# DecodeGenetics/Ratatosk

Hardware: AMD Instinct MI355X
Metric: corrected long-read bases/sec (higher is better)
Workload: dtype u64

## Files before the change

### include/ratatosk_hip.h

```cpp
#ifndef RATATOSK_HIP_H
#define RATATOSK_HIP_H

#include <stdint.h>

#ifdef __cplusplus
extern "C" {
#endif

#define RTK_OK 0
#define RTK_ERR_IO (-1)
#define RTK_ERR_FORMAT (-2)
#define RTK_ERR_ARG (-3)
#define RTK_ERR_NO_DEVICE (-4)
#define RTK_ERR_DEVICE (-5)
#define RTK_ERR_UNSUPPORTED (-6)

typedef struct rtk_graph rtk_graph;
typedef struct rtk_batch rtk_batch;

typedef struct rtk_opts {
    uint64_t insert_sz;
    uint64_t min_cov_vertices;
    uint64_t max_len_weak_region1;
    uint64_t max_km_cov;
    double weak_region_len_factor;
    double large_k_factor;
    double min_score;
    int32_t max_qual;
    int32_t out_qual;
    double min_confidence_snp_corr;
    int32_t long_read_correct;
    int32_t force_unres_snp_corr;
    uint64_t max_len_weak_region2;
    int32_t a2_exclusive;
    int32_t a3_strand_order;
    int32_t d1_desc;
    uint32_t struct_size;
} rtk_opts;

typedef struct rtk_graph_info {
    uint64_t n_unitigs, n_kmers, n_bases, n_colour_ids, n_global_sets;
    uint64_t table_slots, hbm_bytes;
    uint64_t max_km_cov_top;
    int32_t k, device;
} rtk_graph_info;

typedef struct rtk_stats {
    double ms_total, ms_lookup_exact, ms_mask, ms_lookup_inexact, ms_seeds, ms_regions, ms_correct, ms_stitch;
    uint64_t n_windows, n_probes_exact, n_probes_inexact, n_hits_inexact, n_regions, n_region_items, n_arena_overflow;
    uint64_t n_expand, n_colour_elem, n_path_base, n_align, n_align_cells;
    uint64_t in_bases, out_bases;
    uint64_t cyc_colour, cyc_paths, cyc_consensus, cyc_total, cyc_myers, cyc_sets , cyc_tostring, cyc_pathqual;
    uint64_t n_slots_exact, n_slots_inexact;
    uint64_t cyc_walk, n_moves;
    double ms_lanes;
    uint64_t n_lane_regions, n_lane_handed;
    double ms_phase;
    uint64_t n_phase_skipped;
    uint64_t n_trim_stored, n_trim_column, n_trim_fallback, n_consensus_resumed, n_consensus_swept;
    uint64_t n_fa_linked_run, n_fa_linked_skipped, n_fa_linked_entries;
    uint64_t n_strand2_run, n_strand2_skipped, n_strand2_audit_mismatch;
    uint64_t n_park_walked, n_park_deferred;
    uint64_t n_colours_small, n_colours_wide, n_colours_bits, n_colours_general, n_colours_audit_mismatch;
    uint64_t n_colours_declined_fit;
    uint64_t n_park_resweeps;
} rtk_stats;

int rtk_graph_load(const char* unitig_fasta_gz, const char* rtsk, int k, int n_threads, rtk_graph** out);
#define RTK_LOAD_DEVICE_TABLES 1u
int rtk_graph_load2(const char* unitig_fasta_gz, const char* rtsk, int k, int n_threads, uint32_t flags, rtk_graph** out);

int rtk_graph_upload(rtk_graph* g, int device);

int rtk_graph_shell(int k, rtk_graph** out);
int rtk_graph_n_buffers(const rtk_graph* g);
int rtk_graph_buffer(rtk_graph* g, int idx, void** dev_ptr, uint64_t* bytes);
int rtk_graph_alloc_buffers(rtk_graph* g, int device, const uint64_t* bytes, int n, const rtk_graph_info* info);
int rtk_graph_adopt_device(rtk_graph* g);
int rtk_graph_attach_buffers(rtk_graph* g, int device, void* const* dev_ptrs, const uint64_t* bytes, int n, const rtk_graph_info* info);
int rtk_graph_buffer_bytes(const rtk_graph* g, uint64_t* bytes, int n);
int rtk_graph_move_buffer(rtk_graph* g, int idx, void* dev_ptr, uint64_t bytes);
int rtk_graph_host_buffer(const rtk_graph* g, int idx, const void** p, uint64_t* bytes);
int rtk_graph_download_buffer(const rtk_graph* g, int idx, void* host_dst, uint64_t bytes);

int rtk_n_devices(void);
int rtk_device_memory(int device, uint64_t* free_bytes, uint64_t* total_bytes);
int rtk_graph_clone_to_device(const rtk_graph* src, int device, rtk_graph** out);

int rtk_graph_get_info(const rtk_graph* g, rtk_graph_info* info);
void rtk_graph_free(rtk_graph* g);
long long rtk_graph_strip_annotations(rtk_graph* g);

int rtk_reserve_scratch(int device, uint32_t max_read_len);
int rtk_reserve_second_pass(int device, uint32_t n_tickets, uint64_t phase_bytes, uint64_t region_bytes);
int rtk_graph_reserve_batches(rtk_graph* g, uint32_t n_batches, uint64_t bases_per_batch, uint32_t reads_per_batch, int with_qualities, uint64_t raw_bases_per_batch);

int rtk_opts_default(const rtk_graph* g, rtk_opts* opts);

int rtk_correct_batch(rtk_graph* g, const rtk_opts* opts, uint32_t n, const char* const* seq, const char* const* qual,
                      const uint32_t* len, char** out_seq, char** out_qual, uint32_t* out_len);
int rtk_coalesce_stats(rtk_graph* g, uint64_t* n_groups, uint64_t* n_tickets);

int rtk_batch_create(rtk_graph* g, uint32_t n, const char* const* seq, const char* const* qual, const uint32_t* len, rtk_batch** out);
int rtk_batch_create2(rtk_graph* g, uint32_t n, const char* const* seq, const char* const* qual, const uint32_t* len,
                      const char* const* raw, const uint32_t* raw_len, rtk_batch** out);
int rtk_batch_run(rtk_batch* b, const rtk_opts* opts);
int rtk_batch_run_seeds(rtk_batch* b, const rtk_opts* opts);
int rtk_batch_run_regions(rtk_batch* b, const rtk_opts* opts);
int rtk_batch_fetch(rtk_batch* b, char** out_seq, char** out_qual, uint32_t* out_len);
int rtk_batch_fetch_view(rtk_batch* b, const char** pool, const uint64_t** off, const uint32_t** len);
int rtk_batch_get_stats(const rtk_batch* b, rtk_stats* stats);
void rtk_batch_free(rtk_batch* b);


int rtk_lookup_exact(rtk_graph* g, const char* seq, uint32_t len, int64_t* hits);

int rtk_fix_snps(rtk_graph* g, const char* seq, uint32_t len, char* out);

int rtk_seeds(rtk_graph* g, const rtk_opts* opts, const char* seq, uint32_t len,
              uint64_t* n_solid, int64_t* solid, uint64_t* n_weak, int64_t* weak, uint64_t cap);

int rtk_batch_fetch_seeds(rtk_batch* b, uint32_t read, uint64_t* n_solid, int64_t* solid, uint64_t* n_weak, int64_t* weak, uint64_t cap);

int rtk_myers_batch(uint32_t n, const char* const* query, const uint32_t* qlen, const char* const* target, const uint32_t* tlen,
                    const int32_t* k, const int32_t* mode, int want_path, int use_iupac,
                    int32_t* dist, int32_t* n_loc, int32_t* end_locs, uint32_t cap_locs, char* cigar, uint32_t cap_cigar);

int rtk_myers_batch_waves(uint32_t n, const char* const* query, const uint32_t* qlen, const char* const* target, const uint32_t* tlen,
                          const int32_t* k, const int32_t* mode, int want_path, int use_iupac,
                          int32_t* dist, int32_t* n_loc, int32_t* end_locs, uint32_t cap_locs, char* cigar, uint32_t cap_cigar, int waves);

#define RTK_MYERS_MODE_SHW_BY_COLUMN 3
#define RTK_MYERS_MODE_NW_PREFIX 4
#define RTK_MYERS_MODE_NW_PREFIX_LAST 5
#define RTK_MYERS_MODE_NW_PREFIX_LAST_COLUMN 6
void rtk_myers_column_last_routes(uint64_t* column_route, uint64_t* fallback);

int rtk_myers_batch_lanes(uint32_t n, const char* const* query, const uint32_t* qlen, const char* const* target, const uint32_t* tlen,
                          const int32_t* k, const int32_t* mode, int want_path, int use_iupac,
                          int32_t* dist, int32_t* n_loc, int32_t* end_locs, uint32_t cap_locs, char* cigar, uint32_t cap_cigar);
void rtk_myers_lanes_last_routes(uint64_t* lane_route, uint64_t* wave_route);

int rtk_index_count_kmers(int device, int k, const char* const* files, int n_files, uint32_t min_count, int n_threads, uint64_t** solid, uint64_t* n_solid);
int rtk_index_unitigs(int device, int k, const uint64_t* solid, uint64_t n_solid, char** seq_pool, uint64_t** seq_off, uint64_t** seeds, uint64_t* n_unitigs,
                      uint64_t** left, uint64_t* n_left);

int rtk_index_colour_begin(int device, int k, const char* seq_pool, const uint64_t* seq_off, uint64_t n_unitigs, void** job);
int rtk_index_colour_chunk(void* job, const char* chars, uint64_t n_chars, const uint64_t* starts, const uint32_t* ids, uint32_t n_reads);
int rtk_index_colour_end(void* job, uint64_t** events, uint64_t* n_events, uint64_t** cov);
int rtk_index_colour_chunk_q(void* job, const char* chars, const unsigned char* quals, unsigned char q_min, uint64_t n_chars, const uint64_t* starts, const uint32_t* ids,
                             uint32_t n_reads);
int rtk_index_colour_cov(void* job, uint64_t** cov);
int rtk_index_colour_end_subsampled(void* job, const uint8_t* bin_of_unitig, const uint8_t* forced_candidate, const uint8_t* bin_is_sampled, uint32_t n_bins, uint32_t mcv,
                                    double rate, uint64_t seed, uint64_t** events, uint64_t* n_events, uint64_t* n_events_before, uint64_t* n_ids_before, uint64_t* n_ids_after);
int rtk_index_subsample_events(int device, const uint64_t* events, uint64_t n_events, uint32_t n_unitigs, const uint8_t* bin_of_unitig, const uint8_t* forced_candidate,
                               const uint8_t* bin_is_sampled, uint32_t n_bins, uint32_t mcv, double rate, uint64_t seed, uint64_t* events_out, uint64_t* n_out,
                               uint64_t* n_ids_before, uint64_t* n_ids_after);
int rtk_index_colour_merge(void* job, uint64_t* n_events_before, uint64_t* n_events_after, uint64_t* n_ids_before, uint64_t* n_ids_after);
int rtk_index_colour_merge_classes(void* job, uint64_t* classes_above_one, uint64_t* largest);
int rtk_index_merge_events(int device, const uint64_t* events, uint64_t n_events, uint32_t n_unitigs, uint64_t* events_out, uint64_t* n_out, uint64_t* n_ids_before,
                           uint64_t* n_ids_after);

#define RTK_SNP_FIRST_PER_SITE 1u
int rtk_index_snp_candidates(int device, int k, const char* seq_pool, const uint64_t* seq_off, uint64_t n_unitigs, const uint8_t* searched, uint32_t flags,
                             uint64_t** cand, uint64_t* n_cand);
int rtk_index_snp_plan(int device, int k, const uint64_t* seq_off, uint64_t n_unitigs, const uint8_t* searched, uint64_t room, uint32_t* passes,
                       uint64_t* need_one_pass, uint64_t* need_min);

int rtk_index_cover_begin(int device, int k, const char* seq_pool, const uint64_t* seq_off, uint64_t n_unitigs, const uint8_t* low_bits, void** job);
int rtk_index_cover_chunk(void* job, const char* chars, uint64_t n_chars, const uint64_t* starts, const uint32_t* seq_numbers, const uint64_t* first_positions, uint32_t n_seqs);
int rtk_index_cover_end(void* job, uint64_t** crossings, uint64_t* n);

int rtk_rescue_begin(int device, int k, const uint64_t* lr, uint64_t n_lr, const uint64_t* sr, uint64_t n_sr, uint32_t min_positions, void** job);
int rtk_rescue_chunk(void* job, const char* chars, uint64_t n_chars, const uint64_t* starts, uint32_t n_reads, unsigned char* keep);
int rtk_rescue_end(void* job, uint64_t* n_positions_probed, uint64_t* n_hits);

int rtk_qv_begin(int device, int k, const uint64_t* solid, uint64_t n_solid, void** job);
int rtk_qv_chunk(void* job, const char* chars, uint64_t n_chars, const uint64_t* starts, uint32_t n_pieces, uint32_t* windows, uint32_t* found);
int rtk_qv_end(void* job, uint64_t* n_windows, uint64_t* n_found);
uint32_t rtk_qv_span(void);

#define RTK_SETS_UNION 0
#define RTK_SETS_INTER 1
#define RTK_SETS_DIFF 2
#define RTK_SETS_INTER_COUNT 3
#define RTK_SETS_SORT_PAIRS 4
#define RTK_SETS_RADIX_U32 5
#define RTK_SETS_RADIX_PAIRS_U32 6
#define RTK_SETS_BM_LOWEST 7
#define RTK_SETS_BM8_LOWEST 8
#define RTK_SETS_RADIX_TAGGED 9
#define RTK_SETS_COLOUR_UNIVERSE 10
#define RTK_SETS_OK 0
#define RTK_SETS_NOT_IN_BUILD 1
#define RTK_SETS_DECLINED 2
int rtk_sets_batch(uint32_t n, const uint32_t* op, const uint32_t* const* a, const uint32_t* na, const uint32_t* const* b, const uint32_t* nb, const uint32_t* scalar,
                   uint32_t* out_pool, const uint64_t* out_off, uint32_t* out_n, uint32_t* result, uint32_t* status);

void rtk_free(void* p);
void rtk_free_many(void** p, uint32_t n);
const char* rtk_last_error(void);
const char* rtk_version(void);
#define RTK_API_REVISION 10
int rtk_api_revision(void);

#ifdef __cplusplus
}
#endif

#endif
```

### ratatosk_amd/api.py

```python
import ctypes as C
import os

_HERE = os.path.dirname(os.path.abspath(__file__))
LIB_PATH = os.environ.get("RTK_LIB_OVERRIDE") or os.path.join(_HERE, "libratatosk_hip.so")


class RtkError(RuntimeError):
    pass


class RtkOpts(C.Structure):
    _fields_ = [("insert_sz", C.c_uint64), ("min_cov_vertices", C.c_uint64), ("max_len_weak_region1", C.c_uint64),
                ("max_km_cov", C.c_uint64), ("weak_region_len_factor", C.c_double), ("large_k_factor", C.c_double),
                ("min_score", C.c_double), ("max_qual", C.c_int32), ("out_qual", C.c_int32), ("min_confidence_snp_corr", C.c_double),
                ("long_read_correct", C.c_int32), ("force_unres_snp_corr", C.c_int32), ("max_len_weak_region2", C.c_uint64),
                ("a2_exclusive", C.c_int32), ("a3_strand_order", C.c_int32), ("d1_desc", C.c_int32), ("struct_size", C.c_uint32)]


class RtkGraphInfo(C.Structure):
    _fields_ = [("n_unitigs", C.c_uint64), ("n_kmers", C.c_uint64), ("n_bases", C.c_uint64), ("n_colour_ids", C.c_uint64),
                ("n_global_sets", C.c_uint64), ("table_slots", C.c_uint64), ("hbm_bytes", C.c_uint64), ("max_km_cov_top", C.c_uint64),
                ("k", C.c_int32), ("device", C.c_int32)]


class RtkStats(C.Structure):
    _fields_ = [(n, C.c_double) for n in ("ms_total", "ms_lookup_exact", "ms_mask", "ms_lookup_inexact", "ms_seeds", "ms_regions", "ms_correct", "ms_stitch")] + \
               [(n, C.c_uint64) for n in ("n_windows", "n_probes_exact", "n_probes_inexact", "n_hits_inexact", "n_regions", "n_region_items", "n_arena_overflow",
                                         "n_expand", "n_colour_elem", "n_path_base", "n_align", "n_align_cells", "in_bases", "out_bases",
                                         "cyc_colour", "cyc_paths", "cyc_consensus", "cyc_total", "cyc_myers", "cyc_sets", "cyc_tostring", "cyc_pathqual", "n_slots_exact", "n_slots_inexact", "cyc_walk", "n_moves")] + \
               [("ms_lanes", C.c_double), ("n_lane_regions", C.c_uint64), ("n_lane_handed", C.c_uint64), ("ms_phase", C.c_double), ("n_phase_skipped", C.c_uint64)] + \
               [(n, C.c_uint64) for n in ("n_trim_stored", "n_trim_column", "n_trim_fallback", "n_consensus_resumed", "n_consensus_swept",
                                         "n_fa_linked_run", "n_fa_linked_skipped", "n_fa_linked_entries",
                                         "n_strand2_run", "n_strand2_skipped", "n_strand2_audit_mismatch",
                                         "n_park_walked", "n_park_deferred",
                                         "n_colours_small", "n_colours_wide", "n_colours_bits", "n_colours_general", "n_colours_audit_mismatch", "n_colours_declined_fit",
                                         "n_park_resweeps")]

    def as_dict(self):
        return {n: getattr(self, n) for n, _ in self._fields_}


_libs = {}


os.environ.setdefault("GPU_MAX_HW_QUEUES", "16")


def load_library(path=None):
    path = path or LIB_PATH
    if path in _libs:
        return _libs[path]
    if not os.path.exists(path):
        raise RtkError("%s is missing: build it with `python -c 'import __graft_entry__ as g; g.build()'` (make -C ratatosk_amd/csrc)" % path)
    L = C.CDLL(path)
    L.rtk_last_error.restype = C.c_char_p
    L.rtk_version.restype = C.c_char_p
    L.rtk_graph_load.argtypes = [C.c_char_p, C.c_char_p, C.c_int, C.c_int, C.POINTER(C.c_void_p)]
    L.rtk_graph_load2.argtypes = [C.c_char_p, C.c_char_p, C.c_int, C.c_int, C.c_uint32, C.POINTER(C.c_void_p)]
    L.rtk_graph_move_buffer.argtypes = [C.c_void_p, C.c_int, C.c_void_p, C.c_uint64]
    L.rtk_graph_host_buffer.argtypes = [C.c_void_p, C.c_int, C.POINTER(C.c_void_p), C.POINTER(C.c_uint64)]
    L.rtk_graph_download_buffer.argtypes = [C.c_void_p, C.c_int, C.c_void_p, C.c_uint64]
    L.rtk_graph_upload.argtypes = [C.c_void_p, C.c_int]
    L.rtk_graph_shell.argtypes = [C.c_int, C.POINTER(C.c_void_p)]
    L.rtk_graph_n_buffers.argtypes = [C.c_void_p]
    L.rtk_graph_buffer.argtypes = [C.c_void_p, C.c_int, C.POINTER(C.c_void_p), C.POINTER(C.c_uint64)]
    L.rtk_graph_alloc_buffers.argtypes = [C.c_void_p, C.c_int, C.POINTER(C.c_uint64), C.c_int, C.POINTER(RtkGraphInfo)]
    L.rtk_graph_adopt_device.argtypes = [C.c_void_p]
    L.rtk_graph_buffer_bytes.argtypes = [C.c_void_p, C.POINTER(C.c_uint64), C.c_int]
    L.rtk_graph_get_info.argtypes = [C.c_void_p, C.POINTER(RtkGraphInfo)]
    L.rtk_graph_free.argtypes = [C.c_void_p]
    L.rtk_opts_default.argtypes = [C.c_void_p, C.POINTER(RtkOpts)]
    L.rtk_correct_batch.argtypes = [C.c_void_p, C.POINTER(RtkOpts), C.c_uint32, C.POINTER(C.c_char_p), C.POINTER(C.c_char_p), C.POINTER(C.c_uint32),
                                    C.POINTER(C.c_void_p), C.POINTER(C.c_void_p), C.POINTER(C.c_uint32)]
    L.rtk_batch_create.argtypes = [C.c_void_p, C.c_uint32, C.POINTER(C.c_char_p), C.POINTER(C.c_char_p), C.POINTER(C.c_uint32), C.POINTER(C.c_void_p)]
    L.rtk_batch_create2.argtypes = [C.c_void_p, C.c_uint32, C.POINTER(C.c_char_p), C.POINTER(C.c_char_p), C.POINTER(C.c_uint32),
                                    C.POINTER(C.c_char_p), C.POINTER(C.c_uint32), C.POINTER(C.c_void_p)]
    L.rtk_batch_run.argtypes = [C.c_void_p, C.POINTER(RtkOpts)]
    L.rtk_graph_strip_annotations.restype = C.c_longlong
    L.rtk_graph_strip_annotations.argtypes = [C.c_void_p]
    L.rtk_batch_run_seeds.argtypes = [C.c_void_p, C.POINTER(RtkOpts)]
    L.rtk_batch_run_regions.argtypes = [C.c_void_p, C.POINTER(RtkOpts)]
    L.rtk_batch_fetch.argtypes = [C.c_void_p, C.POINTER(C.c_void_p), C.POINTER(C.c_void_p), C.POINTER(C.c_uint32)]
    L.rtk_batch_fetch_view.argtypes = [C.c_void_p, C.POINTER(C.c_char_p), C.POINTER(C.POINTER(C.c_uint64)), C.POINTER(C.POINTER(C.c_uint32))]
    L.rtk_n_devices.restype = C.c_int
    L.rtk_device_memory.argtypes = [C.c_int, C.POINTER(C.c_uint64), C.POINTER(C.c_uint64)]
    L.rtk_graph_clone_to_device.argtypes = [C.c_void_p, C.c_int, C.POINTER(C.c_void_p)]
    L.rtk_batch_get_stats.argtypes = [C.c_void_p, C.POINTER(RtkStats)]
    L.rtk_batch_free.argtypes = [C.c_void_p]
    L.rtk_lookup_exact.argtypes = [C.c_void_p, C.c_char_p, C.c_uint32, C.POINTER(C.c_int64)]
    L.rtk_fix_snps.argtypes = [C.c_void_p, C.c_char_p, C.c_uint32, C.c_char_p]
    L.rtk_seeds.argtypes = [C.c_void_p, C.POINTER(RtkOpts), C.c_char_p, C.c_uint32, C.POINTER(C.c_uint64), C.POINTER(C.c_int64),
                            C.POINTER(C.c_uint64), C.POINTER(C.c_int64), C.c_uint64]
    L.rtk_myers_batch.argtypes = [C.c_uint32, C.POINTER(C.c_char_p), C.POINTER(C.c_uint32), C.POINTER(C.c_char_p), C.POINTER(C.c_uint32),
                                  C.POINTER(C.c_int32), C.POINTER(C.c_int32), C.c_int, C.c_int,
                                  C.POINTER(C.c_int32), C.POINTER(C.c_int32), C.POINTER(C.c_int32), C.c_uint32, C.c_char_p, C.c_uint32]
    L.rtk_myers_batch_waves.argtypes = L.rtk_myers_batch.argtypes + [C.c_int]
    L.rtk_myers_batch_lanes.argtypes = L.rtk_myers_batch.argtypes
    L.rtk_myers_batch_lanes.restype = C.c_int
    L.rtk_coalesce_stats.argtypes = [C.c_void_p, C.POINTER(C.c_uint64), C.POINTER(C.c_uint64)]
    L.rtk_graph_reserve_batches.argtypes = [C.c_void_p, C.c_uint32, C.c_uint64, C.c_uint32, C.c_int, C.c_uint64]
    L.rtk_free_many.argtypes = [C.POINTER(C.c_void_p), C.c_uint32]; L.rtk_free_many.restype = None
    if L.rtk_api_revision() >= 9:
        L.rtk_rescue_begin.argtypes = [C.c_int, C.c_int, C.POINTER(C.c_uint64), C.c_uint64, C.POINTER(C.c_uint64), C.c_uint64, C.c_uint32, C.POINTER(C.c_void_p)]
        L.rtk_rescue_chunk.argtypes = [C.c_void_p, C.c_char_p, C.c_uint64, C.POINTER(C.c_uint64), C.c_uint32, C.POINTER(C.c_ubyte)]
        L.rtk_rescue_end.argtypes = [C.c_void_p, C.POINTER(C.c_uint64), C.POINTER(C.c_uint64)]
    if L.rtk_api_revision() >= 10:
        L.rtk_sets_batch.argtypes = [C.c_uint32, C.POINTER(C.c_uint32), C.POINTER(C.POINTER(C.c_uint32)), C.POINTER(C.c_uint32), C.POINTER(C.POINTER(C.c_uint32)), C.POINTER(C.c_uint32),
                                     C.POINTER(C.c_uint32), C.POINTER(C.c_uint32), C.POINTER(C.c_uint64), C.POINTER(C.c_uint32), C.POINTER(C.c_uint32), C.POINTER(C.c_uint32)]
    if hasattr(L, "rtk_index_subsample_events"):
        L.rtk_index_colour_cov.argtypes = [C.c_void_p, C.POINTER(C.POINTER(C.c_uint64))]
        L.rtk_index_colour_end_subsampled.argtypes = [C.c_void_p, C.POINTER(C.c_ubyte), C.POINTER(C.c_ubyte), C.POINTER(C.c_ubyte), C.c_uint32, C.c_uint32, C.c_double, C.c_uint64,
                                                      C.POINTER(C.POINTER(C.c_uint64)), C.POINTER(C.c_uint64), C.POINTER(C.c_uint64), C.POINTER(C.c_uint64), C.POINTER(C.c_uint64)]
        L.rtk_index_subsample_events.argtypes = [C.c_int, C.POINTER(C.c_uint64), C.c_uint64, C.c_uint32, C.POINTER(C.c_ubyte), C.POINTER(C.c_ubyte), C.POINTER(C.c_ubyte), C.c_uint32, C.c_uint32,
                                                 C.c_double, C.c_uint64, C.POINTER(C.c_uint64), C.POINTER(C.c_uint64), C.POINTER(C.c_uint64), C.POINTER(C.c_uint64)]
    if hasattr(L, "rtk_index_merge_events"):
        L.rtk_index_colour_merge.argtypes = [C.c_void_p, C.POINTER(C.c_uint64), C.POINTER(C.c_uint64), C.POINTER(C.c_uint64), C.POINTER(C.c_uint64)]
        L.rtk_index_colour_merge_classes.argtypes = [C.c_void_p, C.POINTER(C.c_uint64), C.POINTER(C.c_uint64)]
        L.rtk_index_merge_events.argtypes = [C.c_int, C.POINTER(C.c_uint64), C.c_uint64, C.c_uint32, C.POINTER(C.c_uint64), C.POINTER(C.c_uint64), C.POINTER(C.c_uint64), C.POINTER(C.c_uint64)]
    if hasattr(L, "rtk_index_colour_chunk_q"):
        L.rtk_index_colour_chunk_q.argtypes = [C.c_void_p, C.c_char_p, C.c_char_p, C.c_ubyte, C.c_uint64, C.POINTER(C.c_uint64), C.POINTER(C.c_uint32), C.c_uint32]
    if hasattr(L, "rtk_batch_fetch_seeds"):
        L.rtk_batch_fetch_seeds.argtypes = [C.c_void_p, C.c_uint32, C.POINTER(C.c_uint64), C.POINTER(C.c_int64), C.POINTER(C.c_uint64), C.POINTER(C.c_int64), C.c_uint64]
    if hasattr(L, "rtk_index_snp_candidates"):
        L.rtk_index_snp_candidates.argtypes = [C.c_int, C.c_int, C.c_char_p, C.POINTER(C.c_uint64), C.c_uint64, C.POINTER(C.c_ubyte), C.c_uint32,
                                               C.POINTER(C.POINTER(C.c_uint64)), C.POINTER(C.c_uint64)]
    if hasattr(L, "rtk_index_snp_plan"):
        L.rtk_index_snp_plan.argtypes = [C.c_int, C.c_int, C.POINTER(C.c_uint64), C.c_uint64, C.POINTER(C.c_ubyte), C.c_uint64, C.POINTER(C.c_uint32), C.POINTER(C.c_uint64),
                                         C.POINTER(C.c_uint64)]
    if hasattr(L, "rtk_index_cover_begin"):
        L.rtk_index_cover_begin.argtypes = [C.c_int, C.c_int, C.c_char_p, C.POINTER(C.c_uint64), C.c_uint64, C.POINTER(C.c_ubyte), C.POINTER(C.c_void_p)]
        L.rtk_index_cover_chunk.argtypes = [C.c_void_p, C.c_char_p, C.c_uint64, C.POINTER(C.c_uint64), C.POINTER(C.c_uint32), C.POINTER(C.c_uint64), C.c_uint32]
        L.rtk_index_cover_end.argtypes = [C.c_void_p, C.POINTER(C.POINTER(C.c_uint64)), C.POINTER(C.c_uint64)]
    if hasattr(L, "rtk_qv_begin"):
        L.rtk_qv_begin.argtypes = [C.c_int, C.c_int, C.POINTER(C.c_uint64), C.c_uint64, C.POINTER(C.c_void_p)]
        L.rtk_qv_chunk.argtypes = [C.c_void_p, C.c_char_p, C.c_uint64, C.POINTER(C.c_uint64), C.c_uint32, C.POINTER(C.c_uint32), C.POINTER(C.c_uint32)]
        L.rtk_qv_end.argtypes = [C.c_void_p, C.POINTER(C.c_uint64), C.POINTER(C.c_uint64)]
        L.rtk_qv_span.argtypes = []; L.rtk_qv_span.restype = C.c_uint32
    L.rtk_free.argtypes = [C.c_void_p]
    _libs[path] = L
    return L


RTK_LOAD_DEVICE_TABLES = 1


def _b(s):
    return s.encode() if isinstance(s, str) else s


class Graph:

    def __init__(self, fasta_gz, rtsk, k=31, device=0, lib_path=None, upload=True, n_threads=None, host_tables=None):
        self.L = load_library(lib_path)
        self.h = C.c_void_p()
        if n_threads is None:
            n_threads = max(1, min(32, os.cpu_count() or 1))
        if host_tables is None:
            host_tables = not upload or os.environ.get("RTK_HOST_TABLES") == "1"
        self._check(self.L.rtk_graph_load2(_b(fasta_gz), _b(rtsk), k, n_threads, 0 if host_tables else RTK_LOAD_DEVICE_TABLES, C.byref(self.h)))
        self.k = k
        if upload:
            self._check(self.L.rtk_graph_upload(self.h, device))

    def _check(self, rc):
        if rc != 0:
            raise RtkError("rtk error %d: %s" % (rc, self.L.rtk_last_error().decode()))

    def close(self):
        if getattr(self, "h", None):
            self.L.rtk_graph_free(self.h)
            self.h = None

    def __del__(self):
        try:
            self.close()
        except Exception:
            pass

    def info(self):
        i = RtkGraphInfo()
        self._check(self.L.rtk_graph_get_info(self.h, C.byref(i)))
        return i

    def opts(self, **kw):
        o = RtkOpts()
        self._check(self.L.rtk_opts_default(self.h, C.byref(o)))
        for k_, v in kw.items():
            setattr(o, k_, v)
        return o

    def lookup_exact(self, seq):
        s = _b(seq)
        nw = max(0, len(s) - self.k + 1)
        out = (C.c_int64 * max(1, nw))()
        self._check(self.L.rtk_lookup_exact(self.h, s, len(s), out))
        return [out[i] for i in range(nw)]

    def fix_snps(self, seq):
        s = _b(seq)
        out = C.create_string_buffer(len(s) + 1)
        self._check(self.L.rtk_fix_snps(self.h, s, len(s), out))
        return out.raw[:len(s)]

    def seeds(self, seq, opts=None):
        s = _b(seq)
        o = opts or self.opts()
        cap = 64 * len(s) + 64
        ns, nw = C.c_uint64(), C.c_uint64()
        so, we = (C.c_int64 * (4 * cap))(), (C.c_int64 * (4 * cap))()
        self._check(self.L.rtk_seeds(self.h, C.byref(o), s, len(s), C.byref(ns), so, C.byref(nw), we, cap))
        f = lambda a, n: [(a[4 * i], a[4 * i + 1], a[4 * i + 2], a[4 * i + 3]) for i in range(n)]
        return f(so, ns.value), f(we, nw.value)

    def correct_batch(self, seqs, quals=None, opts=None, raw=None):
        b = Batch(self, seqs, quals, raw)
        try:
            b.run(opts)
            return b.fetch()
        finally:
            b.close()


class Batch:

    def __init__(self, graph, seqs, quals=None, raw=None):
        self.g = graph
        self.L = graph.L
        n = len(seqs)
        bs = [_b(s) for s in seqs]
        seq_arr = (C.c_char_p * n)(*bs)
        qual_arr = None
        if quals is not None:
            bq = [_b(q) for q in quals]
            qual_arr = (C.c_char_p * n)(*bq)
        lens = (C.c_uint32 * n)(*[len(b) for b in bs])
        self.n = n
        self.lens = [len(b) for b in bs]
        self.in_bases = sum(self.lens)
        self.h = C.c_void_p()
        if raw is not None:
            br = [_b(s) for s in raw]
            raw_arr = (C.c_char_p * n)(*br)
            raw_lens = (C.c_uint32 * n)(*[len(b) for b in br])
            graph._check(self.L.rtk_batch_create2(graph.h, n, seq_arr, qual_arr, lens, raw_arr, raw_lens, C.byref(self.h)))
        else:
            graph._check(self.L.rtk_batch_create(graph.h, n, seq_arr, qual_arr, lens, C.byref(self.h)))

    def run(self, opts=None):
        o = opts or self.g.opts()
        self.g._check(self.L.rtk_batch_run(self.h, C.byref(o)))

    def run_seeds(self, opts=None):
        o = opts or self.g.opts()
        self.g._check(self.L.rtk_batch_run_seeds(self.h, C.byref(o)))

    def run_regions(self, opts=None):
        o = opts or self.g.opts()
        self.g._check(self.L.rtk_batch_run_regions(self.h, C.byref(o)))

    def seeds(self, i, cap=None):
        if not hasattr(self.L, "rtk_batch_fetch_seeds"):
            raise RtkError("%s lacks rtk_batch_fetch_seeds (anchors of one read of a batch: appended at interface revision 10)" % self.L._name)
        ns, nw = C.c_uint64(), C.c_uint64()
        if cap is None:
            one = (C.c_int64 * 4)()
            rc = self.L.rtk_batch_fetch_seeds(self.h, i, C.byref(ns), one, C.byref(nw), one, 0)
            if rc != 0 and b"capacity" not in self.L.rtk_last_error():
                self.g._check(rc)
            cap = max(ns.value, nw.value)
        so, we = (C.c_int64 * (4 * max(1, cap)))(), (C.c_int64 * (4 * max(1, cap)))()
        self.g._check(self.L.rtk_batch_fetch_seeds(self.h, i, C.byref(ns), so, C.byref(nw), we, cap))
        f = lambda a, n: [(a[4 * j], a[4 * j + 1], a[4 * j + 2], a[4 * j + 3]) for j in range(n)]
        return f(so, ns.value), f(we, nw.value)

    def fetch(self):
        n = self.n
        os_, oq = (C.c_void_p * n)(), (C.c_void_p * n)()
        ol = (C.c_uint32 * n)()
        self.g._check(self.L.rtk_batch_fetch(self.h, os_, oq, ol))
        out = []
        for i in range(n):
            out.append((C.string_at(os_[i], ol[i]).decode(), C.string_at(oq[i], ol[i]).decode()))
            self.L.rtk_free(os_[i]); self.L.rtk_free(oq[i])
        return out

    def stats(self):
        s = RtkStats()
        self.g._check(self.L.rtk_batch_get_stats(self.h, C.byref(s)))
        return s.as_dict()

    def close(self):
        if getattr(self, "h", None):
            self.L.rtk_batch_free(self.h)
            self.h = None

    def __del__(self):
        try:
            self.close()
        except Exception:
            pass


def myers_batch(queries, targets, ks=None, modes=None, want_path=False, use_iupac=True, lib_path=None, waves=0, lanes=False):
    L = load_library(lib_path)
    n = len(queries)
    bq = [_b(q) for q in queries]; bt = [_b(t) for t in targets]
    ks = ks if ks is not None else [-1] * n
    modes = modes if modes is not None else [0] * n
    qa = (C.c_char_p * n)(*bq); ta = (C.c_char_p * n)(*bt)
    ql = (C.c_uint32 * n)(*[len(x) for x in bq]); tl = (C.c_uint32 * n)(*[len(x) for x in bt])
    ka = (C.c_int32 * n)(*ks); ma = (C.c_int32 * n)(*modes)
    cap_locs = max(len(x) for x in bt) + 2 if n else 2
    cap_cig = 4 * (max((len(x) for x in bq), default=0) + max((len(x) for x in bt), default=0)) + 16
    dist = (C.c_int32 * n)(); nloc = (C.c_int32 * n)(); locs = (C.c_int32 * (n * cap_locs))()
    cig = C.create_string_buffer(n * cap_cig) if want_path else None
    if lanes:
        rc = L.rtk_myers_batch_lanes(n, qa, ql, ta, tl, ka, ma, 1 if want_path else 0, 1 if use_iupac else 0, dist, nloc, locs, cap_locs, cig, cap_cig)
    elif waves > 1:
        rc = L.rtk_myers_batch_waves(n, qa, ql, ta, tl, ka, ma, 1 if want_path else 0, 1 if use_iupac else 0, dist, nloc, locs, cap_locs, cig, cap_cig, waves)
    else:
        rc = L.rtk_myers_batch(n, qa, ql, ta, tl, ka, ma, 1 if want_path else 0, 1 if use_iupac else 0, dist, nloc, locs, cap_locs, cig, cap_cig)
    if rc != 0:
        raise RtkError("rtk error %d: %s" % (rc, L.rtk_last_error().decode()))
    out = []
    for i in range(n):
        el = [locs[i * cap_locs + j] for j in range(min(nloc[i], cap_locs))] if dist[i] >= 0 else []
        c = ""
        if want_path:
            c = cig.raw[i * cap_cig:(i + 1) * cap_cig].split(b"\0", 1)[0].decode()
        out.append((dist[i], el, c))
    return out


def _u64_array(a):
    if hasattr(a, "ctypes"):
        import numpy as np
        arr = np.ascontiguousarray(a, dtype=np.uint64)
        return arr, arr.ctypes.data_as(C.POINTER(C.c_uint64)), int(arr.size)
    arr = (C.c_uint64 * max(1, len(a)))(*[int(x) for x in a])
    return arr, arr, len(a)


def rescue_reads(lr_kmers, sr_kmers, seqs, k=31, min_positions=31, device=0, stats=None, lib_path=None):
    L = load_library(lib_path)
    if L.rtk_api_revision() < 9:
        raise RtkError("%s is of interface revision %d: the rescue entries came with revision 9" % (L._name, L.rtk_api_revision()))
    keep_lr, p_lr, n_lr = _u64_array(lr_kmers)
    keep_sr, p_sr, n_sr = _u64_array(sr_kmers)
    job = C.c_void_p()

    def check(rc):
        if rc != 0:
            raise RtkError("rtk error %d: %s" % (rc, L.rtk_last_error().decode()))

    check(L.rtk_rescue_begin(device, k, p_lr, n_lr, p_sr, n_sr, min_positions, C.byref(job)))
    out = []
    try:
        bs = [_b(s) for s in seqs]
        i = 0
        while i < len(bs):
            j, size = i, 0
            while j < len(bs) and (j == i or (size + len(bs[j]) + 1 <= (48 << 20) and j - i < (2 << 20))):
                size += len(bs[j]) + 1; j += 1
            starts, at = (C.c_uint64 * (j - i))(), 0
            for r in range(i, j):
                starts[r - i] = at; at += len(bs[r]) + 1
            chars = b"\n".join(bs[i:j]) + b"\n"
            keep = (C.c_ubyte * (j - i))()
            check(L.rtk_rescue_chunk(job, chars, len(chars), starts, j - i, keep))
            out.extend(bool(x) for x in keep)
            i = j
    except Exception:
        L.rtk_rescue_end(job, None, None)
        raise
    probed, hits = C.c_uint64(), C.c_uint64()
    check(L.rtk_rescue_end(job, C.byref(probed), C.byref(hits)))
    if stats is not None:
        stats["n_positions_probed"], stats["n_hits"] = probed.value, hits.value
    return out


QV_CHUNK_CHARS = 48 << 20


def qv_span(lib_path=None):
    L = load_library(lib_path)
    if not hasattr(L, "rtk_qv_begin"):
        raise RtkError("%s has no rtk_qv entries" % L._name)
    return int(L.rtk_qv_span())


def qv_reads(solid_kmers, seqs, k=31, device=0, max_piece=None, lib_path=None, threads=1, stats=None):
    L = load_library(lib_path)
    if not hasattr(L, "rtk_qv_begin"):
        raise RtkError("%s has no rtk_qv entries" % L._name)
    if max_piece is None:
        max_piece = QV_CHUNK_CHARS - 1
    if max_piece < k or max_piece > QV_CHUNK_CHARS - 1:
        raise ValueError("max_piece must lie in k .. %d" % (QV_CHUNK_CHARS - 1))
    keep_solid, p_solid, n_solid = _u64_array(solid_kmers)
    bs = [_b(s) for s in seqs]
    pieces = []
    for r, s in enumerate(bs):
        a = 0
        while True:
            pieces.append((r, s[a:a + max_piece]))
            if a + max_piece >= len(s):
                break
            a += max_piece - (k - 1)
    chunks, i = [], 0
    while i < len(pieces):
        j, size = i, 0
        while j < len(pieces) and size + len(pieces[j][1]) + 1 <= max_piece + 1 and j - i < (2 << 20):
            size += len(pieces[j][1]) + 1; j += 1
        chunks.append((i, j)); i = j
    job = C.c_void_p()

    def check(rc):
        if rc != 0:
            raise RtkError("rtk error %d: %s" % (rc, L.rtk_last_error().decode()))

    check(L.rtk_qv_begin(device, k, p_solid, n_solid, C.byref(job)))
    windows, found = [0] * len(bs), [0] * len(bs)
    results = [None] * len(chunks)

    def run(c):
        i, j = chunks[c]
        starts, at = (C.c_uint64 * (j - i))(), 0
        for p in range(i, j):
            starts[p - i] = at; at += len(pieces[p][1]) + 1
        chars = b"\n".join(t for _, t in pieces[i:j]) + b"\n"
        w, f = (C.c_uint32 * (j - i))(), (C.c_uint32 * (j - i))()
        check(L.rtk_qv_chunk(job, chars, len(chars), starts, j - i, w, f))
        results[c] = (list(w), list(f))

    try:
        if threads <= 1:
            for c in range(len(chunks)):
                run(c)
        else:
            import threading
            errors = []

            def feed(t):
                try:
                    for c in range(t, len(chunks), threads):
                        run(c)
                except Exception as e:
                    errors.append(e)

            th = [threading.Thread(target=feed, args=(t,)) for t in range(threads)]
            for t in th:
                t.start()
            for t in th:
                t.join()
            if errors:
                raise errors[0]
    except Exception:
        L.rtk_qv_end(job, None, None)
        raise
    n_windows, n_found = C.c_uint64(), C.c_uint64()
    check(L.rtk_qv_end(job, C.byref(n_windows), C.byref(n_found)))
    for c, (i, j) in enumerate(chunks):
        w, f = results[c]
        for p in range(i, j):
            windows[pieces[p][0]] += w[p - i]; found[pieces[p][0]] += f[p - i]
    if (sum(windows), sum(found)) != (n_windows.value, n_found.value):
        raise RtkError("rtk_qv: the pieces add up to %d windows / %d found, the device counted %d / %d" % (sum(windows), sum(found), n_windows.value, n_found.value))
    if stats is not None:
        stats["n_chunks"], stats["n_windows"], stats["n_found"] = len(chunks), n_windows.value, n_found.value
    return windows, found


MODE_SHW_BY_COLUMN, MODE_NW_PREFIX, MODE_NW_PREFIX_LAST, MODE_NW_PREFIX_LAST_COLUMN = 3, 4, 5, 6


def myers_column_last_routes(lib_path=None):
    L = load_library(lib_path)
    a, b = C.c_uint64(), C.c_uint64()
    L.rtk_myers_column_last_routes.argtypes = [C.POINTER(C.c_uint64), C.POINTER(C.c_uint64)]; L.rtk_myers_column_last_routes.restype = None
    L.rtk_myers_column_last_routes(C.byref(a), C.byref(b))
    return a.value, b.value


def myers_lanes_last_routes(lib_path=None):
    L = load_library(lib_path)
    a, b = C.c_uint64(), C.c_uint64()
    L.rtk_myers_lanes_last_routes.argtypes = [C.POINTER(C.c_uint64), C.POINTER(C.c_uint64)]; L.rtk_myers_lanes_last_routes.restype = None
    L.rtk_myers_lanes_last_routes(C.byref(a), C.byref(b))
    return a.value, b.value


SETS_UNION, SETS_INTER, SETS_DIFF, SETS_INTER_COUNT, SETS_SORT_PAIRS, SETS_RADIX_U32, SETS_RADIX_PAIRS_U32, SETS_BM_LOWEST, SETS_BM8_LOWEST, SETS_RADIX_TAGGED, SETS_COLOUR_UNIVERSE = range(11)
SETS_OK, SETS_NOT_IN_BUILD, SETS_DECLINED = 0, 1, 2


def sets_batch(problems, lib_path=None):
    import numpy as np
    L = load_library(lib_path)
    if L.rtk_api_revision() < 10:
        raise RtkError("%s is of interface revision %d: rtk_sets_batch came with revision 10" % (L._name, L.rtk_api_revision()))
    n = len(problems)
    keep, off = [], [0]
    ops = (C.c_uint32 * max(1, n))(); na = (C.c_uint32 * max(1, n))(); nb = (C.c_uint32 * max(1, n))(); sc = (C.c_uint32 * max(1, n))()
    pa = (C.POINTER(C.c_uint32) * max(1, n))(); pb = (C.POINTER(C.c_uint32) * max(1, n))()
    for i, (op, a, b, scalar) in enumerate(problems):
        if op == SETS_SORT_PAIRS:
            a = np.ascontiguousarray(a, dtype="<u8"); b = np.ascontiguousarray(b, dtype="<u8")
            count_a, count_b, a, b = int(a.size), int(b.size), a.view("<u4"), b.view("<u4")
        else:
            a = np.ascontiguousarray(a, dtype=np.uint32); b = np.ascontiguousarray(b, dtype=np.uint32)
            count_a, count_b = int(a.size), int(b.size)
        keep.append((a, b))
        ops[i], na[i], nb[i], sc[i] = op, count_a, count_b, scalar
        pa[i] = a.ctypes.data_as(C.POINTER(C.c_uint32)); pb[i] = b.ctypes.data_as(C.POINTER(C.c_uint32))
        need = {SETS_UNION: count_a + count_b, SETS_INTER: count_a, SETS_DIFF: count_a, SETS_INTER_COUNT: 0, SETS_SORT_PAIRS: 4 * count_a, SETS_RADIX_U32: count_a,
                SETS_RADIX_PAIRS_U32: 2 * count_a, SETS_BM_LOWEST: min(scalar, count_b), SETS_BM8_LOWEST: min(scalar, count_b),
                SETS_RADIX_TAGGED: 2 * count_a, SETS_COLOUR_UNIVERSE: 2 + count_a + 2 * count_b * max(1, (count_a + 63) // 64)}.get(op, 0)
        off.append(off[-1] + need)
    out = np.zeros(max(1, off[-1]), dtype=np.uint32)
    offs = (C.c_uint64 * (n + 1))(*off)
    out_n = (C.c_uint32 * max(1, n))(); res = (C.c_uint32 * max(1, n))(); st = (C.c_uint32 * max(1, n))()
    rc = L.rtk_sets_batch(n, ops, pa, na, pb, nb, sc, out.ctypes.data_as(C.POINTER(C.c_uint32)), offs, out_n, res, st)
    if rc != 0:
        raise RtkError("rtk error %d: %s" % (rc, L.rtk_last_error().decode()))
    ret = []
    for i, (op, _, _, _) in enumerate(problems):
        if out_n[i] > off[i + 1] - off[i]:
            raise RtkError("rtk_sets_batch: problem %d reports %d output words for a slice of %d" % (i, out_n[i], off[i + 1] - off[i]))
        w = out[off[i]:off[i] + out_n[i]]
        if op == SETS_SORT_PAIRS and st[i] == SETS_OK:
            h = len(w) // 2
            words = (w[:h].copy().view("<u8").tolist(), w[h:].copy().view("<u8").tolist())
        else:
            words = w.tolist()
        ret.append((words, int(res[i]), int(st[i])))
    return ret


def index_subsample_events(events, n_unitigs, bin_of_unitig, forced_candidate, bin_is_sampled, mcv, rate, seed=1, device=0, lib_path=None):
    import numpy as np
    L = load_library(lib_path)
    missing = [s for s in ("rtk_index_colour_cov", "rtk_index_colour_end_subsampled", "rtk_index_subsample_events") if not hasattr(L, s)]
    if missing:
        raise RtkError("%s lacks %s (colour subsampling: appended at interface revision 10)" % (L._name, ", ".join(missing)))
    ev = np.ascontiguousarray(events, dtype=np.uint64)
    bins = np.ascontiguousarray(bin_of_unitig, dtype=np.uint8); forced = np.ascontiguousarray(forced_candidate, dtype=np.uint8); sampled = np.ascontiguousarray(bin_is_sampled, dtype=np.uint8)
    if bins.size != n_unitigs or forced.size != n_unitigs:
        raise RtkError("index_subsample_events: bin_of_unitig and forced_candidate hold one entry per unitig")
    out = np.zeros(max(1, ev.size), dtype=np.uint64)
    n_out, before, after = C.c_uint64(0), C.c_uint64(0), C.c_uint64(0)
    u8, u64 = C.POINTER(C.c_ubyte), C.POINTER(C.c_uint64)
    rc = L.rtk_index_subsample_events(device, ev.ctypes.data_as(u64), ev.size, n_unitigs, bins.ctypes.data_as(u8), forced.ctypes.data_as(u8), sampled.ctypes.data_as(u8), sampled.size, mcv,
                                      float(rate), seed, out.ctypes.data_as(u64), C.byref(n_out), C.byref(before), C.byref(after))
    if rc != 0:
        raise RtkError("rtk error %d: %s" % (rc, L.rtk_last_error().decode()))
    return out[:n_out.value].copy(), before.value, after.value


def index_merge_events(events, n_unitigs, device=0, lib_path=None):
    import numpy as np
    L = load_library(lib_path)
    missing = [s for s in ("rtk_index_colour_merge", "rtk_index_colour_merge_classes", "rtk_index_merge_events") if not hasattr(L, s)]
    if missing:
        raise RtkError("%s lacks %s (merged ids: appended at interface revision 10)" % (L._name, ", ".join(missing)))
    ev = np.ascontiguousarray(events, dtype=np.uint64)
    out = np.zeros(max(1, ev.size), dtype=np.uint64)
    n_out, before, after = C.c_uint64(0), C.c_uint64(0), C.c_uint64(0)
    u64 = C.POINTER(C.c_uint64)
    rc = L.rtk_index_merge_events(device, ev.ctypes.data_as(u64), ev.size, n_unitigs, out.ctypes.data_as(u64), C.byref(n_out), C.byref(before), C.byref(after))
    if rc != 0:
        raise RtkError("rtk error %d: %s" % (rc, L.rtk_last_error().decode()))
    return out[:n_out.value].copy(), before.value, after.value


def index_colour_reads(unitigs, k, reads, ids=None, quals=None, q_min=0, device=0, lib_path=None, chunks=None):
    import numpy as np
    L = load_library(lib_path)
    u64p, u32p = C.POINTER(C.c_uint64), C.POINTER(C.c_uint32)
    L.rtk_index_colour_begin.argtypes = [C.c_int, C.c_int, C.c_char_p, u64p, C.c_uint64, C.POINTER(C.c_void_p)]
    L.rtk_index_colour_chunk.argtypes = [C.c_void_p, C.c_char_p, C.c_uint64, u64p, u32p, C.c_uint32]
    L.rtk_index_colour_end.argtypes = [C.c_void_p, C.POINTER(u64p), u64p, C.POINTER(u64p)]

    def as_bytes(x):
        return x if isinstance(x, bytes) else x.encode()

    reads = [as_bytes(r) for r in reads]
    ids = list(range(len(reads))) if ids is None else list(ids)
    quals = [None] * len(reads) if quals is None else [None if q is None else as_bytes(q) for q in quals]
    if len(ids) != len(reads) or len(quals) != len(reads):
        raise ValueError("index_colour_reads: ids and quals need one entry per read")
    for r, q in zip(reads, quals):
        if q is not None and len(q) != len(r):
            raise ValueError("index_colour_reads: a quality string is as long as its read")
    cuts = [0] + sorted(chunks or []) + [len(reads)]
    parts = [(a, b) for a, b in zip(cuts[:-1], cuts[1:]) if a < b]
    for a, b in parts:
        n_q = sum(q is not None for q in quals[a:b])
        if n_q not in (0, b - a):
            raise ValueError("index_colour_reads: reads %d .. %d: a chunk holds reads with qualities or reads without, not both" % (a, b))
        if n_q and not hasattr(L, "rtk_index_colour_chunk_q"):
            raise RtkError("%s lacks rtk_index_colour_chunk_q (colouring by base confidence: appended at interface revision 10)" % L._name)

    def ok(rc):
        if rc != 0:
            raise RtkError("rtk error %d: %s" % (rc, L.rtk_last_error().decode()))

    seqs = [as_bytes(u) for u in unitigs]
    off = np.zeros(len(seqs) + 1, dtype=np.uint64)
    off[1:] = np.cumsum([len(u) for u in seqs], dtype=np.uint64)
    job = C.c_void_p()
    ok(L.rtk_index_colour_begin(device, k, b"".join(seqs), off.ctypes.data_as(u64p), len(seqs), C.byref(job)))
    try:
        for a, b in parts:
            chars = b"".join(r + b"\n" for r in reads[a:b])
            starts = np.zeros(b - a, dtype=np.uint64)
            starts[1:] = np.cumsum([len(r) + 1 for r in reads[a:b - 1]], dtype=np.uint64)
            cid = np.ascontiguousarray(ids[a:b], dtype=np.uint32)
            if quals[a] is None:
                ok(L.rtk_index_colour_chunk(job, chars, len(chars), starts.ctypes.data_as(u64p), cid.ctypes.data_as(u32p), b - a))
            else:
                qs = b"".join(q + b"\0" for q in quals[a:b])
                ok(L.rtk_index_colour_chunk_q(job, chars, qs, q_min, len(chars), starts.ctypes.data_as(u64p), cid.ctypes.data_as(u32p), b - a))
    except BaseException:
        L.rtk_index_colour_end(job, None, None, None)
        raise
    ev_p, cov_p, n_ev = u64p(), u64p(), C.c_uint64(0)
    ok(L.rtk_index_colour_end(job, C.byref(ev_p), C.byref(n_ev), C.byref(cov_p)))
    try:
        events = np.ctypeslib.as_array(ev_p, shape=(max(1, n_ev.value),))[:n_ev.value].copy()
        cov = np.ctypeslib.as_array(cov_p, shape=(len(seqs),)).copy()
    finally:
        L.rtk_free(ev_p); L.rtk_free(cov_p)
    return events, cov


SNP_FIRST_PER_SITE = 1


def index_snp_candidates(unitigs, k, searched=None, first_per_site=False, device=0, lib_path=None):
    import numpy as np
    L = load_library(lib_path)
    if not hasattr(L, "rtk_index_snp_candidates"):
        raise RtkError("%s lacks rtk_index_snp_candidates (SNP candidates: appended at interface revision 10)" % L._name)
    seqs = [_b(u) for u in unitigs]
    off = np.zeros(len(seqs) + 1, dtype=np.uint64)
    off[1:] = np.cumsum([len(u) for u in seqs], dtype=np.uint64)
    flags = None
    if searched is not None:
        flags = np.ascontiguousarray([1 if f else 0 for f in searched], dtype=np.uint8)
        if flags.size != len(seqs):
            raise ValueError("index_snp_candidates: searched holds one flag per unitig")
    u64p = C.POINTER(C.c_uint64)
    cand, n = u64p(), C.c_uint64(0)
    rc = L.rtk_index_snp_candidates(device, k, b"".join(seqs), off.ctypes.data_as(u64p), len(seqs), None if flags is None else flags.ctypes.data_as(C.POINTER(C.c_ubyte)),
                                    SNP_FIRST_PER_SITE if first_per_site else 0, C.byref(cand), C.byref(n))
    if rc != 0:
        raise RtkError("rtk error %d: %s" % (rc, L.rtk_last_error().decode()))
    try:
        w = np.ctypeslib.as_array(cand, shape=(max(1, 2 * n.value),))[:2 * n.value].copy() if n.value else np.zeros(0, dtype=np.uint64)
    finally:
        L.rtk_free(cand)
    w0, w1 = w[0::2], w[1::2]
    return list(zip((w0 >> np.uint64(32)).tolist(), (w0 & np.uint64(0xFFFFFFFF)).tolist(), (w1 >> np.uint64(40)).tolist(), ((w1 >> np.uint64(32)) & np.uint64(3)).tolist(), (w1 & np.uint64(0xFFFFFFFF)).tolist()))


def index_snp_plan(unitigs, k, searched=None, room=0, device=0, lib_path=None):
    import numpy as np
    L = load_library(lib_path)
    if not hasattr(L, "rtk_index_snp_plan"):
        raise RtkError("%s lacks rtk_index_snp_plan (SNP candidates in passes: appended at interface revision 10)" % L._name)
    off = np.zeros(len(unitigs) + 1, dtype=np.uint64)
    off[1:] = np.cumsum([len(u) for u in unitigs], dtype=np.uint64)
    flags = None
    if searched is not None:
        flags = np.ascontiguousarray([1 if f else 0 for f in searched], dtype=np.uint8)
        if flags.size != len(unitigs):
            raise ValueError("index_snp_plan: searched holds one flag per unitig")
    passes, one, least = C.c_uint32(0), C.c_uint64(0), C.c_uint64(0)
    rc = L.rtk_index_snp_plan(device, k, off.ctypes.data_as(C.POINTER(C.c_uint64)), len(unitigs), None if flags is None else flags.ctypes.data_as(C.POINTER(C.c_ubyte)), room,
                              C.byref(passes), C.byref(one), C.byref(least))
    if rc != 0:
        raise RtkError("rtk error %d: %s" % (rc, L.rtk_last_error().decode()))
    return passes.value, one.value, least.value


def index_cover_layout(sequences, k, chunks=None):
    import numpy as np
    if chunks is not None and chunks < k + 3:
        raise ValueError("index_cover_crossings: a chunk holds at least k + 2 characters and a separator")
    pieces = []
    for n, s in enumerate(_b(x) for x in sequences):
        if len(s) < k + 1:
            continue
        a, room = 0, len(s) if chunks is None else chunks - 1
        while True:
            e = min(len(s), a + room)
            pieces.append((n, a, s[a:e]))
            if e == len(s):
                break
            a = e - k
    parts, cur, size = [], [], 0
    for pc in pieces:
        if cur and chunks is not None and size + len(pc[2]) + 1 > chunks:
            parts.append(cur); cur, size = [], 0
        cur.append(pc); size += len(pc[2]) + 1
    if cur:
        parts.append(cur)
    out = []
    for part in parts:
        starts = np.zeros(len(part), dtype=np.uint64)
        starts[1:] = np.cumsum([len(c) + 1 for _, _, c in part[:-1]], dtype=np.uint64)
        out.append((b"".join(c + b"\n" for _, _, c in part), starts, np.ascontiguousarray([n for n, _, _ in part], dtype=np.uint32),
                    np.ascontiguousarray([a for _, a, _ in part], dtype=np.uint64)))
    return out


def index_cover_crossings(unitigs, k, low_bits, sequences, device=0, lib_path=None, chunks=None):
    import numpy as np
    L = load_library(lib_path)
    if not hasattr(L, "rtk_index_cover_begin"):
        raise RtkError("%s lacks rtk_index_cover_begin / _chunk / _end (low-coverage edges covered: appended at interface revision 10)" % L._name)
    u64p, u32p = C.POINTER(C.c_uint64), C.POINTER(C.c_uint32)
    seqs = [_b(u) for u in unitigs]
    off = np.zeros(len(seqs) + 1, dtype=np.uint64)
    off[1:] = np.cumsum([len(u) for u in seqs], dtype=np.uint64)
    low = np.ascontiguousarray(low_bits, dtype=np.uint8)
    if low.size != len(seqs):
        raise ValueError("index_cover_crossings: low_bits holds one byte per unitig")
    parts = index_cover_layout(sequences, k, chunks)

    def ok(rc):
        if rc != 0:
            raise RtkError("rtk error %d: %s" % (rc, L.rtk_last_error().decode()))

    job = C.c_void_p()
    ok(L.rtk_index_cover_begin(device, k, b"".join(seqs), off.ctypes.data_as(u64p), len(seqs), low.ctypes.data_as(C.POINTER(C.c_ubyte)), C.byref(job)))
    try:
        for chars, starts, numbers, first in parts:
            ok(L.rtk_index_cover_chunk(job, chars, len(chars), starts.ctypes.data_as(u64p), numbers.ctypes.data_as(u32p), first.ctypes.data_as(u64p), len(numbers)))
    except BaseException:
        L.rtk_index_cover_end(job, None, None)
        raise
    out, n = u64p(), C.c_uint64(0)
    ok(L.rtk_index_cover_end(job, C.byref(out), C.byref(n)))
    try:
        w = np.ctypeslib.as_array(out, shape=(max(1, 2 * n.value),))[:2 * n.value].copy() if n.value else np.zeros(0, dtype=np.uint64)
    finally:
        L.rtk_free(out)
    w0, w1 = w[0::2], w[1::2]
    one = np.uint64(1)
    return list(zip((w0 >> np.uint64(32)).tolist(), (w0 & np.uint64(0xFFFFFFFF)).tolist(), (w1 >> np.uint64(33)).tolist(), ((w1 >> np.uint64(3)) & np.uint64(0x3FFFFFFF)).tolist(),
                    ((w1 >> np.uint64(2)) & one).tolist(), (w1 & np.uint64(3)).tolist()))


def run_pipelined(batches, opts=None):
    import threading
    prev, err = None, []

    def seeds(b):
        try:
            b.run_seeds(opts)
        except Exception as e:
            err.append(e)

    for b in batches:
        t = threading.Thread(target=seeds, args=(b,))
        t.start()
        if prev is not None:
            prev.run_regions(opts)
        t.join()
        if err:
            raise err[0]
        prev = b
    if prev is not None:
        prev.run_regions(opts)
```

### ratatosk_amd/csrc/hip/rtk_knobs.h

```cpp
#ifndef RTK_KNOBS_H
#define RTK_KNOBS_H

#include <stdint.h>
#include <stdlib.h>
#include <string.h>
#include <algorithm>

inline bool rtk_env_set(const char* name) { return getenv(name) != nullptr; }
inline bool rtk_env_is1(const char* name) { const char* e = getenv(name); return e && e[0] == '1'; }
inline int rtk_env_int(const char* name, int dflt) { const char* e = getenv(name); return e ? atoi(e) : dflt; }
inline int rtk_env_pos_int(const char* name, int dflt) { const int v = rtk_env_int(name, 0); return v > 0 ? v : dflt; }
inline uint64_t rtk_env_u64(const char* name, uint64_t dflt) { const char* e = getenv(name); return e ? strtoull(e, nullptr, 10) : dflt; }
inline bool rtk_env_eq(const char* name, const char* value) { const char* e = getenv(name); return e && !strcmp(e, value); }

inline bool rtk_knob_trace() { return rtk_env_set("RTK_TRACE"); }
inline int rtk_knob_trace_class(int dflt) { return rtk_env_int("RTK_TRACE_CLASS", dflt); }
inline bool rtk_knob_lane_cost() { return rtk_env_set("RTK_LANE_COST"); }
inline bool rtk_knob_myers_prof() { return rtk_env_set("RTK_MYERS_PROF"); }
inline bool rtk_knob_myers_time() { return rtk_env_set("RTK_MYERS_TIME"); }
inline bool rtk_knob_index_trace() { return rtk_env_set("RTK_INDEX_TRACE"); }
inline bool rtk_knob_load_trace() { return rtk_env_set("RTK_LOAD_TRACE"); }

inline uint32_t rtk_knob_mask_seg() { return static_cast<uint32_t>(rtk_env_u64("RTK_MASK_SEG", 8192)); }
inline int rtk_knob_seed_waves() { return rtk_env_pos_int("RTK_SEED_WAVES", 4096); }
inline bool rtk_knob_inexact_enum() { return rtk_env_is1("RTK_INEXACT_ENUM"); }
inline bool rtk_knob_test_tiny_scratch() { return rtk_env_set("RTK_TEST_TINY_SCRATCH"); }
inline int rtk_knob_a2_exclusive() { return rtk_env_eq("RTK_A2_XOR", "union") ? 0 : (rtk_env_eq("RTK_A2_XOR", "exclusive-ids") ? 2 : 1); }
inline int rtk_knob_a3_strand_order() { return rtk_env_eq("RTK_A3_ORDER", "strand") ? 1 : 0; }
inline int rtk_knob_d1_desc() { return rtk_env_eq("RTK_D1_ORDER", "desc") ? 1 : 0; }

inline bool rtk_knob_phase_align_all() { return rtk_env_is1("RTK_PHASE_ALIGN_ALL"); }
inline uint32_t rtk_knob_phase_long() { return static_cast<uint32_t>(rtk_env_u64("RTK_PHASE_LONG", 24576)); }
inline int rtk_knob_phase_lwaves() { return std::max(1, std::min(16, rtk_env_int("RTK_PHASE_LWAVES", 4))); }
inline int rtk_knob_phase_pgrid() { return rtk_env_int("RTK_PHASE_PGRID", 1024); }
inline int rtk_knob_phase_lgrid() { return rtk_env_int("RTK_PHASE_LGRID", 192); }
inline int rtk_knob_phase_mgrid() { return rtk_env_int("RTK_PHASE_MGRID", 768); }

inline bool rtk_knob_lane_max_gap_set() { return rtk_env_set("RTK_LANE_MAX_GAP"); }
inline uint32_t rtk_knob_lane_max_gap() { return static_cast<uint32_t>(rtk_env_u64("RTK_LANE_MAX_GAP", 0)); }
inline int rtk_knob_lane_waves() { return rtk_env_pos_int("RTK_LANE_WAVES", 1024); }
inline bool rtk_knob_lane_serial() { return rtk_env_is1("RTK_LANE_SERIAL"); }
inline int rtk_knob_lane_round() { return rtk_env_int("RTK_LANE_ROUND", 64); }
inline bool rtk_knob_compact() { return rtk_env_is1("RTK_COMPACT"); }
inline int rtk_knob_region_waves() { return rtk_env_pos_int("RTK_REGION_WAVES", 4096); }
inline int rtk_knob_p2_rgrid() { return rtk_env_int("RTK_P2_RGRID", 512); }
inline bool rtk_knob_fa_linked_always() { return rtk_env_is1("RTK_FA_LINKED_ALWAYS"); }
inline bool rtk_knob_strand2_always() { return rtk_env_is1("RTK_STRAND2_ALWAYS"); }
inline bool rtk_knob_strand2_audit() { return rtk_env_is1("RTK_STRAND2_AUDIT"); }
inline uint32_t rtk_knob_colours_route() { return rtk_env_eq("RTK_COLOURS_ROUTE", "bits") ? 1u : (rtk_env_eq("RTK_COLOURS_ROUTE", "general") ? 2u : 0u); }
inline uint32_t rtk_knob_colours_audit() { return rtk_env_is1("RTK_COLOURS_AUDIT") ? (rtk_env_is1("RTK_TEST_COLOURS_FAULT") ? 3u : 1u) : 0u; }
inline bool rtk_knob_park_eager() { return rtk_env_is1("RTK_PARK_EAGER"); }
inline bool rtk_knob_trim_store() { return rtk_env_is1("RTK_TRIM_STORE"); }
inline bool rtk_knob_test_coalesce_fail() { return rtk_env_set("RTK_TEST_COALESCE_FAIL"); }

inline uint64_t rtk_knob_lane_auto_bases() { static const uint64_t v = rtk_env_u64("RTK_LANE_AUTO_BASES", 512ull << 20); return v; }
inline uint64_t rtk_knob_half_slab_bases() { static const uint64_t v = rtk_env_u64("RTK_HALF_SLAB_BASES", 8ull << 20); return v; }
inline int rtk_knob_half_waves() { static const int v = std::min(rtk_env_pos_int("RTK_HALF_WAVES", 2048), 2048); return v; }
inline uint64_t rtk_knob_coalesce_bases() { static const uint64_t v = rtk_env_u64("RTK_COALESCE_BASES", 16ull << 20); return v; }
inline long rtk_knob_coalesce_wait_us() { static const long v = [] { const char* e = getenv("RTK_COALESCE_WAIT_US"); return e ? atol(e) : 1500L; }(); return v; }
inline uint32_t rtk_knob_coalesce_split() { static const uint32_t v = static_cast<uint32_t>(rtk_env_pos_int("RTK_COALESCE_SPLIT", 2)); return v; }

inline uint64_t rtk_knob_index_cap(uint64_t dflt) { return rtk_env_u64("RTK_INDEX_CAP", dflt); }
inline uint64_t rtk_knob_index_chunk(uint64_t dflt) { const uint64_t v = rtk_env_u64("RTK_INDEX_CHUNK", 0); return v >= 1024 ? v : dflt; }
inline int rtk_knob_index_keep_text() { return rtk_env_int("RTK_INDEX_KEEP_TEXT", -1); }
inline uint64_t rtk_knob_index_events(uint64_t dflt) { return rtk_env_u64("RTK_INDEX_EVENTS", dflt); }
inline uint64_t rtk_knob_index_cover_cap(uint64_t dflt) { return rtk_env_u64("RTK_INDEX_COVER_CAP", dflt); }
inline uint64_t rtk_knob_index_snp_mem(uint64_t dflt) { return std::min(dflt, rtk_env_u64("RTK_INDEX_SNP_MEM", dflt)); }
inline uint32_t rtk_knob_index_snp_passes() { return static_cast<uint32_t>(std::min<uint64_t>(rtk_env_u64("RTK_INDEX_SNP_PASSES", 0), 0xFFFFFFFFull)); }
inline uint64_t rtk_knob_hx_part_keys(uint64_t dflt) { return rtk_env_u64("RTK_HX_PART_KEYS", dflt); }

inline int rtk_knob_sim_devices() { return std::max(1, rtk_env_int("RTK_SIM_DEVICES", 1)); }


#endif
```

### ratatosk_amd/csrc/hip/rtk_pipeline_run.inc

```

RTK_GLOBAL void k_enum(const LaunchCtx* L, BatchView bv, int grid) {
#ifdef RTK_SIM
    unsigned char comp_tab[256];
#else
    __shared__ unsigned char comp_tab[256];
#endif
    for (uint32_t c = static_cast<uint32_t>(rtk_lane()); c < 256u; c += RTK_WAVE) comp_tab[c] = static_cast<unsigned char>(rtk_comp(static_cast<char>(c)));
    rtk_sync();
    for (uint32_t ri = static_cast<uint32_t>(RTK_BLOCK_ID); ri < bv.n_reads; ri += static_cast<uint32_t>(grid)) rtk_enum_regions(L->g, L->bv, L->rb, bv.order[ri], comp_tab);
}

RTK_DEV bool rtk_region_is_heavy(const BatchView& bv, const RegionDesc& rd) {
    if (rd.kind == RTK_RG_GAP) { const uint32_t* sp = bv.s_pos + bv.roff[rd.read]; return (sp[rd.i_solid + 1] - sp[rd.i_solid]) >= 160u; }
    return rd.kind == RTK_RG_HEAD || rd.kind == RTK_RG_TAIL;
}
RTK_DEV bool rtk_gap_is_easy(const GraphView& g, const OptsView& o, const BatchView& bv, const RegionDesc& rd, bool* shortcut, UMap* ua_out, uint32_t* len_unitig_km_out, uint32_t* min_pos_out) {
    const uint64_t base = bv.roff[rd.read]; const uint32_t* sp = bv.s_pos + base; const uint32_t k = static_cast<uint32_t>(g.k);
    const uint32_t pa = sp[rd.i_solid], pb = sp[rd.i_solid + 1];
    const UMap ua = rtk_unpack_hit(bv.hits[base + pa]), ub = rtk_unpack_hit(bv.hits[base + pb]);
    *shortcut = false;
    bool same = (ua.unitig == ub.unitig) && (ua.strand == ub.strand);
    if (same && !(g.flags[ua.unitig] & RTK_F_SHORT_CYCLE)) {
        const uint32_t min_pos = ua.dist < ub.dist ? ua.dist : ub.dist, max_pos = ua.dist < ub.dist ? ub.dist : ua.dist;
        const uint32_t len_query_km = pb - pa, len_unitig_km = max_pos - min_pos;
        uint64_t mn, mx; rtk_min_max_len(len_unitig_km, o.weak_region_len_factor, &mn, &mx);
        same = same && ((ua.strand && (ua.dist < ub.dist)) || (!ua.strand && (ua.dist > ub.dist)));
        same = same && (len_query_km >= mn) && (len_query_km <= mx);
        *shortcut = same; *ua_out = ua; *len_unitig_km_out = len_unitig_km; *min_pos_out = min_pos;
        return true;
    }
    return pb < pa + k;
}
#define RTK_OQ 4
RTK_GLOBAL void k_region_order(const LaunchCtx* L, uint64_t n_regions, int grid) {
    const BatchView& bv = L->bv; const RegionBatch& rb = L->rb;
    const bool first_pass = L->o.long_read_correct == 0;
    const uint32_t lane_max_gap = rb.lane_max_gap;
    for (uint64_t i0 = static_cast<uint64_t>(RTK_BLOCK_ID) * RTK_OQ * RTK_WAVE; i0 < n_regions; i0 += static_cast<uint64_t>(grid) * RTK_OQ * RTK_WAVE) {
        uint64_t mh[RTK_OQ], ml[RTK_OQ], me[RTK_OQ], mn[RTK_OQ][4]; uint32_t th = 0, tl = 0, te = 0, tn[4] = {0, 0, 0, 0};
#pragma unroll
        for (int q = 0; q < RTK_OQ; ++q) {
            const uint64_t i = i0 + static_cast<uint64_t>(q) * RTK_WAVE + static_cast<uint64_t>(rtk_lane());
            const bool in = i < n_regions;
            bool easy = false, heavy = false, lane_cls = false; uint32_t lane_sub = 0;
            if (in) {
                const RegionDesc rd = rb.regions[i];
                if (first_pass) {
                    if (rd.kind == RTK_RG_GAP) { bool sc_; UMap ua_; uint32_t a_, b_; easy = rtk_gap_is_easy(L->g, L->o, bv, rd, &sc_, &ua_, &a_, &b_); }
                    else easy = rd.kind == RTK_RG_WHOLE_MAX || rd.kind == RTK_RG_WHOLE_MIN || rd.kind == RTK_RG_TAIL_COPY;
                }
                if (first_pass && !easy && lane_max_gap != 0 && rd.kind == RTK_RG_GAP) { const uint32_t* sp = bv.s_pos + bv.roff[rd.read]; const uint32_t gl = sp[rd.i_solid + 1] - sp[rd.i_solid]; lane_cls = gl < lane_max_gap; lane_sub = lane_cls ? (4u * gl) / lane_max_gap : 0u; }
                heavy = !easy && !lane_cls && rtk_region_is_heavy(bv, rd);
            }
            mh[q] = rtk_ballot(heavy); ml[q] = rtk_ballot(in && !heavy && !easy && !lane_cls); me[q] = rtk_ballot(easy);
            for (uint32_t sb = 0; sb < 4; ++sb) { mn[q][sb] = rtk_ballot(lane_cls && lane_sub == sb); tn[sb] += static_cast<uint32_t>(rtk_popc(mn[q][sb])); }
            th += static_cast<uint32_t>(rtk_popc(mh[q])); tl += static_cast<uint32_t>(rtk_popc(ml[q])); te += static_cast<uint32_t>(rtk_popc(me[q]));
        }
        unsigned long long bh = 0, bl = 0, be = 0, bn[4] = {0, 0, 0, 0};
        if (rtk_lane() == 0) {
            if (th) bh = rtk_atomic_add(rb.n_heavy.get(), static_cast<unsigned long long>(th));
            if (tl) bl = rtk_atomic_add(rb.n_heavy.get() + 1, static_cast<unsigned long long>(tl));
            if (te) be = rtk_atomic_add(rb.n_heavy.get() + 2, static_cast<unsigned long long>(te));
            for (uint32_t sb = 0; sb < 4; ++sb) if (tn[sb]) bn[sb] = rtk_atomic_add(rb.n_heavy.get() + 8 + sb, static_cast<unsigned long long>(tn[sb]));
        }
        bh = rtk_shfl(bh, 0); bl = rtk_shfl(bl, 0); be = rtk_shfl(be, 0); for (uint32_t sb = 0; sb < 4; ++sb) bn[sb] = rtk_shfl(bn[sb], 0);
        const uint64_t below = (1ull << rtk_lane()) - 1ull;
#pragma unroll
        for (int q = 0; q < RTK_OQ; ++q) {
            const uint64_t i = i0 + static_cast<uint64_t>(q) * RTK_WAVE + static_cast<uint64_t>(rtk_lane());
            const uint64_t mine = 1ull << rtk_lane();
            if (mh[q] & mine) rb.rorder[bh + static_cast<unsigned long long>(rtk_popc(mh[q] & below))] = static_cast<uint32_t>(i);
            else if (me[q] & mine) rb.eorder[be + static_cast<unsigned long long>(rtk_popc(me[q] & below))] = static_cast<uint32_t>(i);
            else if (ml[q] & mine) rb.rorder[n_regions - 1ull - (bl + static_cast<unsigned long long>(rtk_popc(ml[q] & below)))] = static_cast<uint32_t>(i);
            else for (uint32_t sb = 0; sb < 4; ++sb) if (mn[q][sb] & mine) rb.lorder[sb * rb.regions_cap + bn[sb] + static_cast<unsigned long long>(rtk_popc(mn[q][sb] & below))] = static_cast<uint32_t>(i);
            bh += static_cast<unsigned long long>(rtk_popc(mh[q])); bl += static_cast<unsigned long long>(rtk_popc(ml[q])); be += static_cast<unsigned long long>(rtk_popc(me[q])); for (uint32_t sb = 0; sb < 4; ++sb) bn[sb] += static_cast<unsigned long long>(rtk_popc(mn[q][sb]));
        }
    }
}

struct RtkEasy { uint64_t src; uint64_t b0; uint32_t len_a, len_b, n_max, n_min, n_dec, strand; };
RTK_GLOBAL void k_regions_easy(const LaunchCtx* L, int grid) {
    const GraphView& g = L->g; const OptsView& o = L->o; const BatchView& bv = L->bv; const RegionBatch& rb = L->rb;
    const unsigned long long n_easy = rtk_u(rb.n_heavy[2]);
    const uint32_t k = static_cast<uint32_t>(g.k);
    const char q_min = rtk_get_qual(0.0, 0, static_cast<uint64_t>(o.max_qual)), q_max = rtk_get_qual(1.0, 0, static_cast<uint64_t>(o.max_qual));
    const char* const seq = bv.seq.get(); const uint64_t* const useq = g.useq.get(); char* const pool = rb.seg_pool.get();
    unsigned long long npb = 0;
    for (unsigned long long i0 = static_cast<unsigned long long>(RTK_BLOCK_ID) * RTK_WAVE; i0 < n_easy; i0 += static_cast<unsigned long long>(grid) * RTK_WAVE) {
        const unsigned long long i = i0 + static_cast<unsigned long long>(rtk_lane());
        const bool in = i < n_easy;
        RtkEasy e; e.src = 0; e.b0 = 0; e.len_a = 0; e.len_b = 0; e.n_max = 0; e.n_min = 0; e.n_dec = 0; e.strand = 1;
        RegionDesc* rd = nullptr;
        if (in) {
            rd = rb.regions.get() + rb.eorder[i];
            const uint32_t r = rd->read, kind = rd->kind;
            const uint64_t base = bv.roff[r]; const uint32_t Lr = static_cast<uint32_t>(bv.roff[r + 1] - base);
            if (kind == RTK_RG_WHOLE_MAX || kind == RTK_RG_WHOLE_MIN) { e.src = base; e.len_a = Lr; if (kind == RTK_RG_WHOLE_MAX) e.n_max = Lr; else e.n_min = Lr; }
            else if (kind == RTK_RG_TAIL_COPY) { const uint32_t prev_pos = rd->prev_pos, pa = bv.s_pos[base + rd->i_solid]; e.src = base + prev_pos; e.len_a = Lr - prev_pos; e.n_max = pa - prev_pos + k; e.n_min = Lr - pa - k; }
            else {
                const uint32_t prev_pos = rd->prev_pos, pa = bv.s_pos[base + rd->i_solid], pb = bv.s_pos[base + rd->i_solid + 1];
                bool shortcut = false; UMap ua = rtk_um_empty(); uint32_t len_unitig_km = 0, min_pos = 0;
                (void)rtk_gap_is_easy(g, o, bv, *rd, &shortcut, &ua, &len_unitig_km, &min_pos);
                e.src = base + prev_pos;
                if (shortcut) {
                    e.len_a = pa - prev_pos; e.len_b = len_unitig_km; e.n_dec = len_unitig_km + k; e.n_max = e.len_a + e.len_b;
                    e.b0 = g.uoff[ua.unitig] + min_pos; e.strand = ua.strand;
                } else {
                    e.len_a = pb - prev_pos;
                    if (pb < pa + k) e.n_max = (pa - prev_pos) + (pb - pa); else { e.n_max = (pa - prev_pos) + k; e.n_min = pb - pa - k; }
                }
            }
        }
        const uint32_t sl = e.len_a + e.len_b, ql = e.n_max + e.n_min;
        int total = 0; const int mine = rtk_wave_excl_scan(static_cast<int>(in ? sl + ql : 0u), &total);
        unsigned long long off0 = 0;
        if (rtk_lane() == 0 && total) off0 = rtk_atomic_add(rb.seg_top, static_cast<unsigned long long>(total));
        off0 = rtk_u(rtk_shfl(off0, 0));
        const unsigned long long off = off0 + static_cast<unsigned long long>(mine);
        if (in) { rd->seg_off = off; rd->seq_len = sl; rd->qual_len = ql; rd->status = 0; }
        if (off0 + static_cast<unsigned long long>(rtk_u(total)) > rb.seg_cap) continue;
        const int cnt = static_cast<int>((n_easy - i0) < static_cast<unsigned long long>(RTK_WAVE) ? (n_easy - i0) : static_cast<unsigned long long>(RTK_WAVE));
        for (int j = 0; j < cnt; ++j) {
            const uint64_t src = rtk_u(rtk_shfl(e.src, j)), b0 = rtk_u(rtk_shfl(e.b0, j)); const unsigned long long o_j = rtk_u(rtk_shfl(off, j));
            const uint32_t len_a = rtk_u(rtk_shfl(e.len_a, j)), len_b = rtk_u(rtk_shfl(e.len_b, j)), n_max = rtk_u(rtk_shfl(e.n_max, j)), n_min = rtk_u(rtk_shfl(e.n_min, j)), n_dec = rtk_u(rtk_shfl(e.n_dec, j)), strand = rtk_u(rtk_shfl(e.strand, j));
            char* out = pool + o_j;
            for (uint32_t x = static_cast<uint32_t>(rtk_lane()); x < len_a; x += RTK_WAVE) out[x] = seq[src + x];
            for (uint32_t x = static_cast<uint32_t>(rtk_lane()); x < len_b; x += RTK_WAVE) {
                const uint64_t pos = strand ? (b0 + x) : (b0 + (n_dec - 1 - x));
                const uint32_t bb = static_cast<uint32_t>((useq[pos >> 5] >> (2 * (pos & 31))) & 3ull);
                out[len_a + x] = static_cast<char>((0x54474341u >> (8 * (strand ? bb : (3u - bb)))) & 0xFFu);
            }
            const uint32_t sl_j = len_a + len_b, ql_j = n_max + n_min;
            for (uint32_t x = static_cast<uint32_t>(rtk_lane()); x < ql_j; x += RTK_WAVE) out[sl_j + x] = x < n_max ? q_max : q_min;
            npb += n_dec;
        }
    }
    if (rtk_lane() == 0 && npb) rtk_atomic_add(L->bv.counters + RTK_CNT_PATHBASE, npb);
}

struct RlLimits { uint32_t str, um, list, arena0, arena1, arena2, tb; };
RTK_GLOBAL void k_regions_lanes(const LaunchCtx* L, uint32_t* area, uint64_t* table, uint64_t n_regions, RlLimits lim, int grid, int round_lanes) {
    const RegionBatch& rb = L->rb; const BatchView& bv = L->bv;
    (void)grid;
    const uint32_t lane = static_cast<uint32_t>(rtk_lane());
#ifndef RTK_SIM
    __builtin_amdgcn_s_setprio(3);
    const unsigned long long round = static_cast<unsigned long long>(round_lanes < 1 ? 1 : (round_lanes > RTK_WAVE ? RTK_WAVE : round_lanes));
#else
    const unsigned long long round = RTK_WAVE; (void)round_lanes;
#endif
    if (lane == 0) {
        RlEnv e;
        e.g = &L->g; e.o = &L->o; e.bv = &L->bv; e.rb = &L->rb;
        e.m = area + static_cast<uint64_t>(RTK_BLOCK_ID) * (static_cast<uint64_t>(RL_WORDS) * RL_STRIDE);
        e.tb = table + static_cast<uint64_t>(RTK_BLOCK_ID) * (static_cast<uint64_t>(RL_TB_WORDCOLS) * 2ull * RL_STRIDE);
        e.k = static_cast<uint32_t>(static_cast<int32_t>(L->g.k));
        e.lim_str = lim.str; e.lim_um = lim.um; e.lim_list = lim.list; e.lim_arena[0] = lim.arena0; e.lim_arena[1] = lim.arena1; e.lim_arena[2] = lim.arena2; e.lim_tb = lim.tb;
        rl_env = e;
    }
    rtk_sync();
    RlCtx c;
    c.c_expand = 0; c.c_colour = 0; c.c_pathbase = 0; c.c_align = 0; c.c_cells = 0;
    unsigned long long n_handed = 0, n_done = 0;
#ifdef RTK_LANE_PROF
    for (int x = 0; x < RL_NPROF; ++x) { c.prof[x] = 0; c.prof2[x] = 0; } c.prof_t = rtk_clock(); c.prof_cur = RL_P_DRIVER;
#endif
    for (int sub = 3; sub >= 0; --sub) {
    const unsigned long long n_lane = rtk_u(rb.n_heavy[8 + sub]);
    const uint32_t* const lorder = rb.lorder.get() + static_cast<uint64_t>(sub) * rb.regions_cap;
    while (true) {
        unsigned long long i0 = 0;
        if (lane == 0) i0 = rtk_atomic_add(rb.next_lane.get() + sub, round);
        i0 = rtk_u(rtk_shfl(i0, 0));
        if (i0 >= n_lane) break;
        const unsigned long long idx = i0 + lane;
        const bool in = idx < n_lane && lane < round;
        uint32_t osl = 0, oql = 0; RegionDesc* rd = nullptr;
        c.fail() = 0;
        if (in) {
            rd = rb.regions.get() + lorder[idx];
            c.top(0) = 0; c.top(1) = 0; c.top(2) = 0; c.memo_n() = 0; c.n_all() = 0; c.sv_valid = 0;
            const uint32_t e0 = c.c_expand, e1 = c.c_colour, e2 = c.c_pathbase, e3 = c.c_align; const unsigned long long e4 = c.c_cells;
#if defined(RTK_SIM) && defined(RTK_LANE_PROF)
            const unsigned long long tr0_ = rtk_clock();
#endif
            rl_region_program(c, rd, &osl, &oql);
#if defined(RTK_SIM) && defined(RTK_LANE_PROF)
            if (rtk_knob_lane_cost()) { const uint32_t* sp_ = bv.s_pos + bv.roff[rd->read]; fprintf(stderr, "LANECOST gap %u cycles %llu expand %u align %u cells %llu fail %u\n", sp_[rd->i_solid + 1] - sp_[rd->i_solid], rtk_clock() - tr0_, c.c_expand - e0, c.c_align - e3, c.c_cells - e4, c.fail()); }
#endif
            if (c.fail()) { osl = 0; oql = 0; c.c_expand = e0; c.c_colour = e1; c.c_pathbase = e2; c.c_align = e3; c.c_cells = e4; }
        }
        RL_LAP(c, RL_P_DRIVER);
        int total = 0; const int mine = rtk_wave_excl_scan(static_cast<int>(osl + oql), &total);
        RL_LAP(c, RL_P_IDLE);
        unsigned long long off0 = 0;
        if (lane == 0 && total) off0 = rtk_atomic_add(rb.seg_top, static_cast<unsigned long long>(total));
        off0 = rtk_u(rtk_shfl(off0, 0));
        if (in) {
            if (c.fail()) {
                rd->status = c.fail(); ++n_handed;
                const unsigned long long at = rtk_atomic_add(rb.n_heavy.get() + 4, 1ull);
                rb.horder[at] = lorder[idx];
            } else {
                const unsigned long long off = off0 + static_cast<unsigned long long>(mine);
                rd->seg_off = off; rd->seq_len = osl; rd->qual_len = oql; rd->status = 0; ++n_done;
                if (off + osl + oql <= rb.seg_cap) {
                    char* out = rb.seg_pool.get() + off;
                    for (uint32_t x = 0; x < osl; ++x) out[x] = static_cast<char>(rl_ldb(c, rl_sb(RL_SB_OUTS) + x));
                    for (uint32_t x = 0; x < oql; ++x) out[osl + x] = static_cast<char>(rl_ldb(c, rl_sb(RL_SB_OUTQ) + x));
                }
            }
        }
        RL_LAP(c, RL_P_EMIT);
    }
    }
#ifdef RTK_LANE_PROF
    { for (int x = 0; x < RL_NPROF; ++x) { unsigned long long v_ = c.prof[x], w_ = c.prof2[x];
#ifndef RTK_SIM
      for (int o = 32; o > 0; o >>= 1) { v_ += __shfl_xor(v_, o, 64); w_ += __shfl_xor(w_, o, 64); }
#endif
      if (lane == 0 && v_) { rtk_atomic_add(bv.counters + RTK_CNT_LANE_PROF + x, v_); rtk_atomic_add(bv.counters + RTK_CNT_LANE_PROF2 + x, w_); } } }
#endif
    {
    unsigned long long v[7] = { c.c_expand, c.c_colour, c.c_pathbase, c.c_align, c.c_cells, n_handed, n_done };
#ifndef RTK_SIM
    for (int x = 0; x < 7; ++x) for (int o = 32; o > 0; o >>= 1) v[x] += __shfl_xor(v[x], o, 64);
#endif
    if (lane == 0) {
        if (v[0]) rtk_atomic_add(bv.counters + RTK_CNT_EXPAND, v[0]); if (v[1]) rtk_atomic_add(bv.counters + RTK_CNT_COLOUR, v[1]); if (v[2]) rtk_atomic_add(bv.counters + RTK_CNT_PATHBASE, v[2]);
        if (v[3]) rtk_atomic_add(bv.counters + RTK_CNT_ALIGN, v[3]); if (v[4]) rtk_atomic_add(bv.counters + RTK_CNT_CELLS, v[4]);
        if (v[5]) rtk_atomic_add(bv.counters + RTK_CNT_LANE_HANDED, v[5]); if (v[6]) rtk_atomic_add(bv.counters + RTK_CNT_LANE_DONE, v[6]);
    }
    }
}

#if defined(RTK_REGION_WPE) && !defined(RTK_SIM)
__attribute__((amdgpu_waves_per_eu(RTK_REGION_WPE, RTK_REGION_WPE)))
#endif
RTK_GLOBAL void k_regions(const LaunchCtx* L, GraphView g, OptsView o, BatchView bv, RegionBatch rb, char* scratch, uint64_t stride, RegionScratchCfg cfg, uint64_t n_regions, int only_flagged, int trace_class, int which) {
#ifdef RTK_SIM
    RegionScratch hdr;
#else
    __shared__ RegionScratch hdr;
#endif
    RegionScratch* sc = region_scratch_carve(scratch + static_cast<uint64_t>(RTK_BLOCK_ID) * stride, cfg, &hdr);
    rtk_sync();
    (void)o;
    RCtx c = {L->g, L->o, L->bv, L->rb, {rtk_opaque(sc)}, {g.k}};
    const unsigned long long n_hv = (which & 1) ? rtk_u(rb.n_heavy[0]) : 0ull, n_lt = (which & 1) ? rtk_u(rb.n_heavy[1]) : 0ull;
    const unsigned long long n_ho = (which & 2) ? rtk_u(rb.n_heavy[4]) : 0ull;
    unsigned long long nxt = 0;
    if (rtk_lane() == 0) nxt = rtk_atomic_add(rb.next_region, 1ull);
#if !defined(RTK_SIM)
    const unsigned long long wall0 = trace_class >= -1 ? 0ull : wall_clock64(); unsigned long long dt_max = 0, n_mine = 0, idx_of_max = 0;
#endif
    int steal_sub = 0;
    while (true) {
        const unsigned long long idx = rtk_u(rtk_shfl(nxt, 0));
        uint32_t ri; bool stolen = false;
        if (idx < n_hv + n_lt + n_ho) {
            ri = rtk_u(idx < n_hv + n_lt ? rb.rorder[idx < n_hv ? idx : (n_regions - n_lt) + (idx - n_hv)] : rb.horder[idx - n_hv - n_lt]);
            if (rtk_lane() == 0) nxt = rtk_atomic_add(rb.next_region, 1ull);
        } else if ((which & 4) && steal_sub < 4) {
            ri = RTK_NONE32;
            while (steal_sub < 4) {
                unsigned long long at = 0;
                if (rtk_lane() == 0) at = rtk_atomic_add(rb.next_lane.get() + steal_sub, 1ull);
                at = rtk_u(rtk_shfl(at, 0));
                if (at < rtk_u(rb.n_heavy[8 + steal_sub])) { ri = rtk_u(rb.lorder[static_cast<uint64_t>(steal_sub) * rb.regions_cap + at]); stolen = true; break; }
                ++steal_sub;
            }
            if (ri == RTK_NONE32) break;
        } else break;
        RegionDesc* rd = rb.regions + ri;
        if (only_flagged && rd->status == 0) continue;
        if (trace_class >= 0) {
            int hb = RTK_GAP_CLASS_HEAD_TAIL;
            if (rd->kind == RTK_RG_GAP) { const uint32_t* sp = bv.s_pos + bv.roff[rd->read]; const uint32_t gl = sp[rd->i_solid + 1] - sp[rd->i_solid]; hb = rtk_gap_class(gl); }
            if (hb != trace_class) continue;
        }
        *sc->overflow = 0; sc->top[RTK_ARENA_REGION] = 0; sc->top[RTK_ARENA_BFS] = 0; sc->top[RTK_ARENA_DFS] = 0; sc->memo_n = 0;
        RTK_PAIR_REGION();
#ifdef RTK_PROF
        {
            const uint64_t* ht = reinterpret_cast<const uint64_t*>(g.ht.get()); const uint64_t nsl = g.ht_slots ? g.ht_slots : 1;
            uint64_t x = (idx * 0x9E3779B97F4A7C15ull) ^ (static_cast<uint64_t>(RTK_BLOCK_ID) << 20);
            unsigned long long t0_ = rtk_clock();
            for (int q = 0; q < 4; ++q) { x = rtk_u(ht[2ull * ((x >> 7) % nsl)]) + x * 0x9E3779B97F4A7C15ull + q; }
            unsigned long long t1_ = rtk_clock();
            uint64_t y = x & 7ull;
            for (int q = 0; q < 4; ++q) { y = (rtk_u(g.uoff[y & 63ull]) + y) & 63ull; }
            unsigned long long t2_ = rtk_clock();
            volatile uint64_t* slab = reinterpret_cast<volatile uint64_t*>(sc->str[RTK_STR_PROBE].get());
            slab[rtk_lane()] = y + x; const uint64_t z = slab[(rtk_lane() + 1) & 63];
            unsigned long long t3_ = rtk_clock() + (z & 1ull);
            sc->prof[RTK_LAP_PROBE_COLD] += t1_ - t0_; sc->prof[RTK_LAP_PROBE_WARM] += t2_ - t1_; sc->prof[RTK_LAP_PROBE_SLAB] += t3_ - t2_; sc->prof[RTK_LAP_PROBE_SAMPLES] += 1; sc->prof_t = rtk_clock();
        }
#endif
        const unsigned long long t0 = rtk_clock();
        const unsigned long long exp0 = RTK_HIST_GET(*sc, RTK_H_DFS_RUNNING);
        rtk_region_program(c, rd);
        { const unsigned long long dt = rtk_clock() - t0; sc->cnt[RTK_RC_CYC_TOTAL] += dt;
#if !defined(RTK_SIM)
          if (trace_class < -1) { ++n_mine; if (dt > dt_max) { dt_max = dt; idx_of_max = idx; } }
#endif
          int hb = RTK_GAP_CLASS_HEAD_TAIL;
          if (rd->kind == RTK_RG_GAP) { const uint32_t* sp = bv.s_pos + bv.roff[rd->read]; const uint32_t gl = sp[rd->i_solid + 1] - sp[rd->i_solid]; hb = rtk_gap_class(gl); }
          else if (rd->kind != RTK_RG_HEAD && rd->kind != RTK_RG_TAIL) hb = -1;
          if (hb >= 0) { RTK_HIST_ADD(*sc, RTK_H_CYCLES + hb, dt); RTK_HIST_ADD(*sc, RTK_H_REGIONS + hb, 1); RTK_HIST_ADD(*sc, RTK_H_DFS + hb, RTK_HIST_GET(*sc, RTK_H_DFS_RUNNING) - exp0); } }
        rd->status = *sc->overflow;
        if (*sc->overflow && rtk_lane() == 0) {
            rtk_atomic_add(rb.n_overflow, 1ull);
            if (stolen) { const unsigned long long at = rtk_atomic_add(rb.n_heavy.get() + 4, 1ull); rb.horder[at] = ri; }
        }
    }
#if !defined(RTK_SIM)
    if (trace_class < -1 && rtk_lane() == 0) {
        const unsigned long long wall1 = wall_clock64();
        atomicMax(reinterpret_cast<unsigned long long*>(bv.counters + RTK_CNT_WAVE_TRACE + 0), dt_max); atomicMax(reinterpret_cast<unsigned long long*>(bv.counters + RTK_CNT_WAVE_TRACE + 1), ~wall0); atomicMax(reinterpret_cast<unsigned long long*>(bv.counters + RTK_CNT_WAVE_TRACE + 2), wall1);
        rtk_atomic_add(bv.counters + RTK_CNT_WAVE_TRACE + 3, wall1 - wall0); rtk_atomic_add(bv.counters + RTK_CNT_WAVE_TRACE + 4, 1ull);
        if (dt_max > 0 && atomicMax(reinterpret_cast<unsigned long long*>(bv.counters + RTK_CNT_WAVE_TRACE + 5), dt_max) < dt_max) bv.counters[RTK_CNT_WAVE_TRACE + 6] = idx_of_max;
        atomicMax(reinterpret_cast<unsigned long long*>(bv.counters + RTK_CNT_WAVE_TRACE + 7), n_mine);
    }
#endif
    if (rtk_lane() == 0) {
        rtk_atomic_add(bv.counters + RTK_CNT_EXPAND, sc->cnt[RTK_RC_EXPAND]); rtk_atomic_add(bv.counters + RTK_CNT_COLOUR, sc->cnt[RTK_RC_COLOUR]); rtk_atomic_add(bv.counters + RTK_CNT_PATHBASE, sc->cnt[RTK_RC_PATHBASE]);
        rtk_atomic_add(bv.counters + RTK_CNT_ALIGN, sc->cnt[RTK_RC_ALIGN]); rtk_atomic_add(bv.counters + RTK_CNT_CELLS, sc->cnt[RTK_RC_CELLS]);
        for (int i = 0; i < 6; ++i) rtk_atomic_add(bv.counters + RTK_CNT_CYC + i, sc->cnt[RTK_RC_CYC_COLOUR + i]);
        rtk_atomic_add(bv.counters + RTK_CNT_CYC_SETS, sc->cnt[RTK_RC_CYC_PATHREC]); rtk_atomic_add(bv.counters + RTK_CNT_CYC_TOSTRING, sc->cnt[RTK_RC_CYC_TOSTRING]); rtk_atomic_add(bv.counters + RTK_CNT_CYC_PATHQUAL, sc->cnt[RTK_RC_CYC_PATHQUAL]); rtk_atomic_add(bv.counters + RTK_CNT_WALK_CYCLES, sc->my.walk_cycles); rtk_atomic_add(bv.counters + RTK_CNT_WALK_MOVES, sc->my.walk_moves); rtk_atomic_add(bv.counters + RTK_CNT_WALK_RELOADS, sc->my.walk_reloads); rtk_atomic_add(bv.counters + RTK_CNT_WALK_SCALAR, sc->my.walk_scalar); rtk_atomic_add(bv.counters + RTK_CNT_WALK_CALLS, sc->my.walk_calls); rtk_atomic_add(bv.counters + RTK_CNT_WALK_TAIL, sc->my.walk_tail_cycles); rtk_atomic_add(bv.counters + RTK_CNT_CYC_DFS, sc->cnt[RTK_RC_CYC_DFS]); rtk_atomic_add(bv.counters + RTK_CNT_CYC_COLOUR_OK, sc->cnt[RTK_RC_CYC_COLOUR_OK]);
        for (int i = 0; i < RTK_FINE_N; ++i) rtk_atomic_add(bv.counters + RTK_CNT_FINE + i, sc->fine[i]);
        for (int i = RTK_RC_TRIM_STORED; i < RTK_RC_FA_LINKED_RUN; ++i) rtk_atomic_add(bv.counters + RTK_CNT_ROUTES + (i - RTK_RC_TRIM_STORED), sc->cnt[i]);
        for (int i = RTK_RC_FA_LINKED_RUN; i < RTK_RC_STRAND2_RUN; ++i) rtk_atomic_add(bv.counters + RTK_CNT_FA_LINKED + (i - RTK_RC_FA_LINKED_RUN), sc->cnt[i]);
        for (int i = RTK_RC_STRAND2_RUN; i < RTK_RC_PARK_WALKED; ++i) rtk_atomic_add(bv.counters + RTK_CNT_STRAND2 + (i - RTK_RC_STRAND2_RUN), sc->cnt[i]);
        for (int i = RTK_RC_PARK_WALKED; i < RTK_RC_COLOURS_SMALL; ++i) rtk_atomic_add(bv.counters + RTK_CNT_PARK + (i - RTK_RC_PARK_WALKED), sc->cnt[i]);
        for (int i = RTK_RC_COLOURS_SMALL; i < RTK_RC_PARK_RESWEEPS; ++i) rtk_atomic_add(bv.counters + RTK_CNT_COLOURS + (i - RTK_RC_COLOURS_SMALL), sc->cnt[i]);
        rtk_atomic_add(bv.counters + RTK_CNT_PARK_RESWEEPS, sc->cnt[RTK_RC_PARK_RESWEEPS]);
        for (int i = 0; i < RTK_H_N; ++i) rtk_atomic_add(bv.counters + RTK_CNT_HIST + i, static_cast<unsigned long long>(RTK_HIST_GET(*sc, i)));
#ifdef RTK_PROF
        for (int i = 0; i < RTK_LAP_N; ++i) rtk_atomic_add(bv.counters + RTK_CNT_PROF + i, static_cast<unsigned long long>(sc->prof[i]));
#endif
    }
}

RTK_GLOBAL void k_stitch(const LaunchCtx* L, BatchView bv, int grid) {
    for (uint32_t ri = static_cast<uint32_t>(RTK_BLOCK_ID); ri < bv.n_reads; ri += static_cast<uint32_t>(grid)) rtk_stitch_offsets(L->bv, L->rb, bv.order[ri]);
}
RTK_GLOBAL void k_stitch_copy(const LaunchCtx* L, uint64_t n_regions, int grid) {
    for (uint64_t c0 = static_cast<uint64_t>(RTK_BLOCK_ID) * RTK_WAVE; c0 < n_regions; c0 += static_cast<uint64_t>(grid) * RTK_WAVE) rtk_stitch_copy(L->rb, c0, n_regions);
}

static bool region_compact() { return rtk_knob_compact(); }
static int region_waves_that_fit(uint64_t stride, uint64_t held, bool trace) {
    int w = rtk_knob_region_waves();
#ifndef RTK_SIM
    size_t fr = 0, tot = 0;
    if (hipMemGetInfo(&fr, &tot) == hipSuccess && stride) {
        const uint64_t room = (static_cast<uint64_t>(fr) + held) / 10 * 7;
        if (trace) fprintf(stderr, "[rtk trace] region work areas: %.1f GB free + %.1f GB held of %.1f GB, %d waves x %.1f MB wanted\n", fr / 1073741824.0, held / 1073741824.0, tot / 1073741824.0, w, stride / 1048576.0);
        if (static_cast<uint64_t>(w) * stride > room) { uint64_t f = room / stride / 256 * 256; if (f < 512) f = 512; if (f < static_cast<uint64_t>(w)) w = static_cast<int>(f); }
    }
#else
    (void)stride; (void)held; (void)trace;
#endif
    return w;
}

static RegionScratchCfg region_cfg(uint32_t max_len_exact, int attempt) {
    RegionScratchCfg c;
    uint32_t max_len = 131072u; while (max_len < max_len_exact) max_len <<= 1;
    if (attempt == 0 && rtk_knob_test_tiny_scratch()) {
        c.str_cap = 2048; c.my.w_cap = c.str_cap / 64 + 2; c.my.t_cap = c.str_cap; c.my.r_cap = c.str_cap; c.my.mv_cap = 2 * c.str_cap;
        c.my.tb_cap_words = 4ull * 52429 + 64; c.set_cap = 64; c.um_cap = 8; c.list_cap = 64; c.memo_cap = 16; c.bm_words = max_len / 64 + 8; c.arena_cap = 8192;
        return c;
    }
    if (region_compact()) {
        if (attempt == 0) {
            c.str_cap = 65536; c.my.w_cap = c.str_cap / 64 + 2; c.my.t_cap = c.str_cap; c.my.r_cap = c.str_cap; c.my.mv_cap = 2 * c.str_cap;
            c.my.tb_cap_words = 4ull * 8192 + 64; c.set_cap = 4096; c.um_cap = 512; c.list_cap = 1024; c.memo_cap = 512; c.bm_words = c.str_cap / 64 + 8; c.arena_cap = 128u << 10;
            return c;
        }
        attempt -= 1;
    }
    const uint32_t scale = 1u << (3 * attempt);
    c.str_cap = std::max<uint32_t>(65536u, (5u * max_len) / 2u + 1024u) * scale;
    c.my.w_cap = c.str_cap / 64 + 2; c.my.t_cap = c.str_cap; c.my.r_cap = c.str_cap; c.my.mv_cap = 2 * c.str_cap;
    c.my.tb_cap_words = std::max<uint64_t>(4ull * 52429 + 64, 4ull * c.my.w_cap + 64);
    c.set_cap = 16384u * scale; c.um_cap = 2048u * scale; c.list_cap = 4096u * scale; c.memo_cap = 2048u * scale;
    c.bm_words = max_len / 64 + 8; c.arena_cap = (1ull << 20) * scale;
    return c;
}

static int batch_precheck(rtk_batch* b, const rtk_opts* opts, const char* who) {
    if (!b || !opts) return rtk_fail(RTK_ERR_ARG, std::string(who) + ": null argument");
    if (!opts_ok(opts)) return rtk_fail(RTK_ERR_ARG, std::string(who) + ": rtk_opts was not filled by this library's rtk_opts_default (struct_size does not match: older header, or a zero-filled struct)");
    if (!b->g->on_device) return rtk_fail(RTK_ERR_NO_DEVICE, std::string(who) + ": graph is not resident on a device");
    return RTK_OK;
}

extern "C" int rtk_batch_run_seeds(rtk_batch* b, const rtk_opts* opts) {
    int rc = batch_precheck(b, opts, "rtk_batch_run_seeds");
    if (rc) return rc;
    if (b->g->info.k > 31 && !opts->long_read_correct) return rtk_fail(RTK_ERR_ARG, "rtk_batch_run_seeds: graphs with k > 31 serve the second pass only (long_read_correct = 1): the 1-edit anchor search of the first pass is built for one-word k-mers");
    try {
        rtk_set_device(b->g->device);
        b->seeded = false; b->ran = false;
        b->t_all.start(b->stream);
        if (opts->long_read_correct && opts->force_unres_snp_corr && !b->snps_fixed) fix_snps_step(b);
        if (opts->long_read_correct && b->has_raw && !b->phased) { rc = phase_step(b, opts_view(opts)); if (rc) return rc; }
        rc = seed_stage_checked(b, opts_view(opts));
        if (rc == RTK_OK) b->seeded = true;
    } catch (const std::exception& e) { return rtk_fail(RTK_ERR_DEVICE, e.what()); }
    return rc;
}

struct SlabHold {
    rtk_graph* g; int what;
    void take(bool half_ok) { what = g->region_slab_take(half_ok); }
    void release() { if (what >= 0) { g->region_slab_give(what); what = -1; } }
    ~SlabHold() { release(); }
};
struct OwnSlab {
    rtk_graph* g; void* p; uint64_t n;
    char* at_least(uint64_t bytes) { if (n < bytes) { if (p) { g->phase_give(p, n); p = nullptr; n = 0; } p = g->phase_take(bytes, &n); } return static_cast<char*>(p); }
    ~OwnSlab() { if (p) g->phase_give(p, n); }
};
struct RegionRun {
    rtk_batch* b; rtk_graph* g; OptsView ov; rtk_stream_t sm;
    bool trace;
    bool own_slab;
    std::chrono::steady_clock::time_point w0;
    int grid; uint32_t max_len; unsigned long long n_regions, n_ovf_total, out_top;
    bool lane_auto, lanes_on, lanes_beside; int lane_waves_used;
    RtkTimer t_enum, t_easy, t_lanes, t_reg, t_st; double ms_reg;
    SlabHold hold; OwnSlab slab;
    const LaunchCtx* ctx() const { return static_cast<const LaunchCtx*>(b->ctx()); }
    void set_ctx() { rtk_launch(k_set_ctx, 1, sm, b->ctx(), g->dview, ov, b->bv, b->rb); }
    void lap(const char* what) const {
        if (trace) fprintf(stderr, "[rtk trace] regions %-10s +%.2f ms\n", what, std::chrono::duration<double, std::milli>(std::chrono::steady_clock::now() - w0).count());
    }
};

static void region_alloc_lists(rtk_batch* b, uint64_t cap) {
    RegionBatch& rb = b->rb;
    rb.regions_cap = cap;
    rb.regions = b->alloc<RegionDesc>(cap); rb.rorder = b->alloc<uint32_t>(cap); rb.eorder = b->alloc<uint32_t>(cap);
    rb.lorder = b->alloc<uint32_t>(4 * cap); rb.horder = b->alloc<uint32_t>(cap); rb.st_off = b->alloc<uint64_t>(cap);
}

static void region_alloc(RegionRun& R) {
    rtk_batch* b = R.b; RegionBatch& rb = b->rb;
    if (rb.seq_rc) return;
    rb.seq_rc = b->alloc<char>(b->n_bases + 64);
    rb.qual_rev = b->bv.qual.get() ? b->alloc<char>(b->n_bases + 64) : nullptr;
    rb.r_first = b->alloc<uint64_t>(b->n); rb.r_count = b->alloc<uint32_t>(b->n);
    rb.n_regions = b->alloc<unsigned long long>(1); rb.n_heavy = b->alloc<unsigned long long>(16); rb.seg_top = b->alloc<unsigned long long>(1);
    rb.next_region = b->alloc<unsigned long long>(1); rb.n_overflow = b->alloc<unsigned long long>(1); rb.out_top = b->alloc<unsigned long long>(1);
    rb.out_off = b->alloc<uint64_t>(b->n); rb.out_seq_len = b->alloc<uint32_t>(b->n); rb.out_qual_len = b->alloc<uint32_t>(b->n);
    region_alloc_lists(b, std::max<uint64_t>(1024, b->n_bases / 8 + 4ull * b->n));
    rb.next_lane = b->alloc<unsigned long long>(4);
    rb.seg_cap = 6 * b->n_bases + (1ull << 20); rb.seg_pool = b->alloc<char>(rb.seg_cap);
    rb.out_cap = 6 * b->n_bases + (1ull << 20); rb.out_pool = b->alloc<char>(rb.out_cap);
}

static void region_lane_class(RegionRun& R) {
    const uint64_t auto_bases = rtk_knob_lane_auto_bases();
    R.lane_auto = !R.own_slab && !rtk_knob_lane_max_gap_set() && auto_bases != 0 && R.b->n_bases >= auto_bases;
    R.b->rb.lane_max_gap = R.own_slab ? 0u : (R.lane_auto ? 128u : rtk_knob_lane_max_gap());
}

static void region_enumerate(RegionRun& R) {
    rtk_batch* b = R.b; RegionBatch& rb = b->rb; const rtk_stream_t sm = R.sm;
    const int eg = std::min<int>(R.grid, static_cast<int>(b->n) > 0 ? static_cast<int>(b->n) : 1);
    for (int tries = 0; tries < 2; ++tries) {
        rtk_dzero_s(rb.n_regions, 8, sm);
        R.set_ctx();
        R.t_enum.start(sm);
        rtk_launch(k_enum, eg, sm, R.ctx(), b->bv, eg);
        R.t_enum.stop(sm);
        rtk_ssync(sm);
        rtk_d2h_s(&R.n_regions, rb.n_regions, 8, sm);
        if (R.n_regions <= rb.regions_cap) break;
        region_alloc_lists(b, R.n_regions + 1024);
    }
    if (R.n_regions) {
        rtk_dzero_s(rb.n_heavy, 128, sm);
        R.set_ctx();
        const unsigned long long per_wave = RTK_OQ * RTK_WAVE;
        const int og = static_cast<int>(std::min<unsigned long long>(static_cast<unsigned long long>(R.grid), (R.n_regions + per_wave - 1ull) / per_wave));
        rtk_launch(k_region_order, og, sm, R.ctx(), static_cast<uint64_t>(R.n_regions), og);
    }
}

static void region_easy(RegionRun& R) {
    rtk_dzero_s(R.b->rb.seg_top, 8, R.sm); rtk_dzero_s(R.b->rb.out_top, 8, R.sm);
    if (!R.n_regions) return;
    const int eg = static_cast<int>(std::min<unsigned long long>(static_cast<unsigned long long>(2 * R.grid), R.n_regions));
    R.t_easy.start(R.sm);
    rtk_launch(k_regions_easy, eg, R.sm, R.ctx(), eg);
    R.t_easy.stop(R.sm);
}

static void region_lanes(RegionRun& R) {
    rtk_batch* b = R.b; RegionBatch& rb = b->rb; const rtk_stream_t sm = R.sm;
    R.lane_waves_used = 0;
    R.lanes_on = R.n_regions && rb.lane_max_gap;
    R.lanes_beside = R.lanes_on && !R.lane_auto && !rtk_knob_lane_serial();
    if (!R.lanes_on) return;
    R.hold.take(false);
#ifdef RTK_SIM
    const int lgrid = 16;
#else
    const int lgrid = R.lane_auto ? 4096 : rtk_knob_lane_waves();
#endif
    R.lane_waves_used = lgrid;
    const uint64_t a_bytes = rl_area_bytes(), t_bytes = rl_table_bytes();
    char* ls = graph_scratch(R.g, 2, (a_bytes + t_bytes) * static_cast<uint64_t>(lgrid));
    RlLimits lim;
    lim.str = RL_STR_BYTES; lim.um = RL_UM_CAP; lim.list = RL_LIST_CAP; lim.arena0 = RL_A0_W; lim.arena1 = RL_A1_W; lim.arena2 = RL_A2_W; lim.tb = RL_TB_WORDCOLS;
    if (rtk_knob_test_tiny_scratch()) { lim.str = 200; lim.um = 6; lim.list = 3; lim.arena0 = 160; lim.arena1 = 400; lim.arena2 = 400; lim.tb = 400; }
    rtk_dzero_s(rb.next_lane, 32, sm);
    rtk_stream_t sl = sm;
    if (R.lanes_beside) { sl = b->lane_stream(); rtk_event_record(b->ev[0], sm); rtk_stream_wait(sl, b->ev[0]); }
    R.t_lanes.start(sl);
    rtk_launch(k_regions_lanes, lgrid, sl, R.ctx(), reinterpret_cast<uint32_t*>(ls), reinterpret_cast<uint64_t*>(ls + a_bytes * static_cast<uint64_t>(lgrid)),
               static_cast<uint64_t>(R.n_regions), lim, lgrid, rtk_knob_lane_round());
    R.t_lanes.stop(sl);
    if (R.lanes_beside) rtk_event_record(b->ev[1], sl);
}

static void region_take_areas(RegionRun& R) {
    rtk_batch* b = R.b; rtk_graph* g = R.g;
    if (!R.own_slab && R.hold.what < 0) {
        const uint64_t half_max_bases = rtk_knob_half_slab_bases();
        R.hold.take(half_max_bases != 0 && b->n_bases <= half_max_bases && !region_compact());
        if (R.hold.what != 2) {
            const uint64_t st0 = region_scratch_bytes(region_cfg(R.max_len, 0)), half_bytes = (g->scratch_bytes_[1] / 2) & ~255ull;
            if (!g->scratch[1] || half_bytes / st0 < 512) { R.hold.release(); R.hold.take(false); }
        }
    }
    if (b->on_region_slab) { b->on_region_slab(b->on_region_slab_arg); b->on_region_slab = nullptr; }
}

struct RegionGridIn {
    int attempt; bool compact;
    int waves_that_fit;
    bool own_slab; int p2_cap;
    bool lanes_beside; int lane_waves;
    bool on_half; int half_waves; uint64_t half_fit;
    unsigned long long n_regions;
};
static int region_grid(const RegionGridIn& in) {
#ifdef RTK_SIM
    int rgrid = 16;
#else
    const int big = in.attempt - (in.compact ? 1 : 0);
    int rgrid = in.attempt == 0 ? in.waves_that_fit : (big == 0 ? 1024 : (big == 1 ? 256 : 8));
#endif
    if (in.own_slab && in.attempt == 0)
        rgrid = static_cast<int>(std::min<unsigned long long>(static_cast<unsigned long long>(in.p2_cap), std::max<unsigned long long>(128ull, in.n_regions / 4ull)));
    if (in.attempt == 0 && in.lanes_beside) rgrid = std::max(1024, rgrid - in.lane_waves);
    rgrid = static_cast<int>(std::min<unsigned long long>(static_cast<unsigned long long>(rgrid), in.n_regions ? in.n_regions : 1ull));
    if (in.on_half) rgrid = static_cast<int>(std::min<uint64_t>(static_cast<uint64_t>(std::min(rgrid, in.half_waves)), in.half_fit));
    return rgrid;
}

static void region_attempt_trace(RegionRun& R, int attempt, int rgrid, uint64_t stride) {
    const BatchView& bv = R.b->bv; const rtk_stream_t sm = R.sm;
    std::vector<RegionDesc> rds(R.n_regions); rtk_d2h_s(rds.data(), R.b->rb.regions, sizeof(RegionDesc) * R.n_regions, sm);
    unsigned long long hist[16] = {0}; for (size_t i = 0; i < rds.size(); ++i) hist[rds[i].status & 15u]++;
    fprintf(stderr, "[rtk trace] k_regions attempt %d: %.2f ms, %d waves, stride %.2f MB; status codes:", attempt, R.t_reg.elapsed(), rgrid, stride / 1048576.0);
    for (int i = 1; i < 16; ++i) if (hist[i]) fprintf(stderr, " %d:%llu", i, hist[i]);
    fprintf(stderr, "\n");
    unsigned long long tc[RTK_CNT_WAVE_TRACE_END - RTK_CNT_WAVE_TRACE] = {0}; rtk_d2h_s(tc, bv.counters + RTK_CNT_WAVE_TRACE, sizeof(tc), sm);
    const double span = static_cast<double>(tc[2] - ~tc[1]) / 100e6 * 1e3, avg_life = tc[4] ? static_cast<double>(tc[3]) / static_cast<double>(tc[4]) / 100e6 * 1e3 : 0.0;
    fprintf(stderr, "[rtk trace] k_regions waves: first start to last end %.2f ms, average lifetime of a wave %.2f ms (%.0f %% of it), longest single region %.3g cycles "
                    "(taken off the queue at place %llu of %llu), most regions on one wave %llu\n",
            span, avg_life, span > 0 ? 100.0 * avg_life / span : 0.0, static_cast<double>(tc[0]), tc[6], static_cast<unsigned long long>(R.n_regions), tc[7]);
}

static int region_attempts(RegionRun& R) {
    rtk_batch* b = R.b; rtk_graph* g = R.g; RegionBatch& rb = b->rb; const rtk_stream_t sm = R.sm;
    const int n_attempts = region_compact() ? 4 : 3;
    R.ms_reg = 0; R.n_ovf_total = 0;
    for (int attempt = 0; attempt < n_attempts; ++attempt) {
        if (attempt != 0 && !R.own_slab && R.hold.what != 2) { R.hold.release(); R.hold.take(false); }
        const RegionScratchCfg cfg = region_cfg(R.max_len, attempt);
        const uint64_t stride = region_scratch_bytes(cfg);
        if (R.trace) fprintf(stderr, "[rtk trace] region work area: %llu bytes per wave\n", static_cast<unsigned long long>(stride));
        const bool on_half = !R.own_slab && R.hold.what != 2;
        const uint64_t half_bytes = (g->scratch_bytes_[1] / 2) & ~255ull;
        RegionGridIn gi;
        gi.attempt = attempt; gi.compact = region_compact(); gi.n_regions = R.n_regions;
#ifdef RTK_SIM
        gi.waves_that_fit = 0;
#else
        gi.waves_that_fit = attempt == 0 ? region_waves_that_fit(stride, R.own_slab ? 0 : g->scratch_bytes_[1], R.trace) : 0;
#endif
        gi.own_slab = R.own_slab; gi.p2_cap = rtk_knob_p2_rgrid();
        gi.lanes_beside = R.lanes_beside; gi.lane_waves = R.lane_waves_used;
        gi.on_half = on_half; gi.half_waves = on_half ? rtk_knob_half_waves() : 0; gi.half_fit = on_half ? half_bytes / stride : 0;
        const int rgrid = region_grid(gi);
        char* scratch;
        if (R.own_slab) scratch = R.slab.at_least(stride * rgrid);
        else if (!on_half) scratch = graph_scratch(g, 1, stride * rgrid);
        else scratch = static_cast<char*>(g->scratch[1]) + static_cast<uint64_t>(R.hold.what) * half_bytes;
        rtk_dzero_s(rb.next_region, 8, sm); rtk_dzero_s(rb.n_overflow, 8, sm);
        if (attempt != 0) R.set_ctx();
        const int tcls = rtk_knob_trace_class(R.trace ? -2 : -1);
        R.t_reg.start(sm);
        rtk_launch(k_regions, rgrid, sm, R.ctx(), g->dview, R.ov, b->bv, rb, scratch, stride, cfg, static_cast<uint64_t>(R.n_regions), attempt == 0 ? 0 : 1, tcls,
                   attempt == 0 ? (R.lanes_beside ? 5 : 1) : 3);
        if (attempt == 0 && R.lanes_on) {
            if (R.lanes_beside) rtk_stream_wait(sm, b->ev[1]);
            rtk_dzero_s(rb.next_region, 8, sm);
            rtk_launch(k_regions, std::min(rgrid, 1024), sm, R.ctx(), g->dview, R.ov, b->bv, rb, scratch, stride, cfg, static_cast<uint64_t>(R.n_regions), 0, tcls, 2);
        }
        R.t_reg.stop(sm);
        rtk_ssync(sm);
        R.ms_reg += R.t_reg.elapsed();
        if (R.trace) region_attempt_trace(R, attempt, rgrid, stride);
        unsigned long long n_ovf = 0; rtk_d2h_s(&n_ovf, rb.n_overflow, 8, sm);
        if (attempt == 0) R.n_ovf_total = n_ovf;
        unsigned long long seg_top = 0; rtk_d2h_s(&seg_top, rb.seg_top, 8, sm);
        if (seg_top > rb.seg_cap) return rtk_fail(RTK_ERR_DEVICE, "region stage: segment pool exhausted");
        if (n_ovf == 0) return RTK_OK;
    }
    return rtk_fail(RTK_ERR_DEVICE, "region stage: scratch capacity exceeded after " + std::to_string(n_attempts) + " attempts");
}

static int region_stitch(RegionRun& R) {
    rtk_batch* b = R.b; const rtk_stream_t sm = R.sm;
    R.t_st.start(sm);
    const int sg = std::min<int>(R.grid, static_cast<int>(b->n) > 0 ? static_cast<int>(b->n) : 1);
    rtk_launch(k_stitch, sg, sm, R.ctx(), b->bv, sg);
    if (R.n_regions) {
        const int cg = static_cast<int>(std::min<unsigned long long>(static_cast<unsigned long long>(2 * R.grid), (R.n_regions + RTK_WAVE - 1ull) / RTK_WAVE));
        rtk_launch(k_stitch_copy, cg, sm, R.ctx(), static_cast<uint64_t>(R.n_regions), cg);
    }
    R.t_st.stop(sm);
    b->t_all.stop(sm);
    rtk_ssync(sm);
    R.out_top = 0; rtk_d2h_s(&R.out_top, b->rb.out_top, 8, sm);
    if (R.out_top > b->rb.out_cap) return rtk_fail(RTK_ERR_DEVICE, "stitch: output pool exhausted");
    return RTK_OK;
}

static void region_trace_report(const unsigned long long* cnt) {
    const double total = double(cnt[RTK_CNT_CYC_TOTAL] ? cnt[RTK_CNT_CYC_TOTAL] : 1);
    auto share = [&](int slot) { return double(cnt[slot]) / total; };
#ifdef RTK_PROF
    {
        static const char* const pn[RTK_LAP_N] = {
            "driver: dispatch + anchors", "driver: same-unitig shortcut", "region: prologue", "region: side lists", "region: chooseColors",
            "semiweak: glue", "paths: prologue", "explore: prefix", "dfs: pop + adj", "dfs: nkm + colour_ok", "dfs T: load/extend",
            "dfs T: to_string", "dfs T: NW sweep", "dfs T: commit", "dfs NT: load/extend", "dfs NT: commit/rest", "dfs post: nt scoring",
            "dfs post: load + to_string", "dfs post: path qual", "dfs post: commit", "paths: after explore", "paths: final select",
            "semiweak: merge", "region: restart/select", "region: assemble", "region: fixAmbiguity", "region: corrected? + trim",
            "driver: between fw/bw", "consensus: rc + card", "consensus: fw NW path", "consensus: bw path / checks", "consensus: merge",
            "consensus: final", "driver: emit prep", "dequeue", "emit", 0, 0, 0, 0, "probe: 4 dependent cold loads", "probe: 4 dependent warm loads",
            "probe: slab store + load", 0};
        const unsigned long long* pr = cnt + RTK_CNT_PROF; const int n = RTK_LAP_N;
        if (pr[RTK_LAP_PROBE_SAMPLES]) fprintf(stderr, "[rtk trace] in-situ probes: cold load %.0f cycles, warm load %.0f cycles, slab store + load %.0f cycles "
                                    "(per round trip, %llu samples)\n",
                            double(pr[RTK_LAP_PROBE_COLD]) / 4.0 / double(pr[RTK_LAP_PROBE_SAMPLES]), double(pr[RTK_LAP_PROBE_WARM]) / 4.0 / double(pr[RTK_LAP_PROBE_SAMPLES]), double(pr[RTK_LAP_PROBE_SLAB]) / double(pr[RTK_LAP_PROBE_SAMPLES]), pr[RTK_LAP_PROBE_SAMPLES]);
        unsigned long long tot = 0; for (int i = 0; i < n; ++i) tot += pr[i];
        fprintf(stderr, "[rtk trace] k_regions lap profile (%.3g cycles):", double(tot));
        for (int i = 0; i < n; ++i) if (pr[i] && pn[i]) fprintf(stderr, " [%d %s %.4f]", i, pn[i], double(pr[i]) / double(tot ? tot : 1));
        fprintf(stderr, "\n");
    }
#endif
    {
        static const char* const hn[RTK_GAP_CLASSES] = {"gap<40", "gap<64", "gap<128", "gap<256", "gap<512", "gap<1024", "gap>=1024", "head/tail"};
        const unsigned long long* h = cnt + RTK_CNT_HIST;
        fprintf(stderr, "[rtk trace] k_regions by size class (share of region time, regions, avg kcycles, second-strand share, DFS calls per region):");
        for (int i = 0; i < RTK_GAP_CLASSES; ++i) {
            const unsigned long long cyc = h[RTK_H_CYCLES + i], n = h[RTK_H_REGIONS + i];
            if (n) fprintf(stderr, " [%s %.3f n=%llu %.0fk bw=%.2f dfs=%.1f]", hn[i], double(cyc) / total, n, 1e-3 * double(cyc) / double(n), double(h[RTK_H_STRAND2 + i]) / double(n),
                           double(h[RTK_H_DFS + i]) / double(n));
        }
        fprintf(stderr, "\n");
    }
    {
        static const char* const fine_names[RTK_FINE_N] = {
            "colour: class unions", "fixAmbiguity: path alignment", "fixAmbiguity: walk of the moves",
            "fixAmbiguity: linked alleles (k-mer lookups)", "fixAmbiguity: apply", "colour small: bit vectors (or array: shared_with(all))",
            "colour small: classes + selection (or array: set ops)", "region: side lists", "region: trim alignment", "region: fixAmbiguity",
            "consensus: merge logic", "paths: explore_paths outside DFS", "colour: small path (cycles)", "colour: 4096-bit path (cycles)",
            "colour: small path calls / total cycles", "colour: 4096-bit path calls / total cycles"};
        const unsigned long long* f = cnt + RTK_CNT_FINE;
        fprintf(stderr, "[rtk trace] chooseColors calls: small path %llu, 4096-bit path %llu; fixAmbiguity calls %llu, of which left by the all-confident way out %llu\n",
                f[RTK_FINE_COL_S_CALLS], f[RTK_FINE_COL_B_CALLS], f[RTK_FINE_FA_CALLS], f[RTK_FINE_FA_ALL_CONFIDENT]);
        fprintf(stderr, "[rtk trace] k_regions fine shares:");
        for (int i = 0; i < RTK_FINE_N; ++i) if (f[i]) fprintf(stderr, " [%s %.3f]", fine_names[i], double(f[i]) / total);
        fprintf(stderr, "\n");
    }
#ifdef RTK_LANE_PROF
    {
        static const char* const ln[RL_NPROF] = {
            "driver", "side lists", "chooseColors", "search glue", "dfs walk", "colour_ok", "to_string", "peq build", "sweep", "walk",
            "path records", "path qual", "select", "amb collect", "fixAmbiguity", "assemble", "trim", "revcomp", "consensus", "emit",
            "idle at round end", "colours: universe", "colours: rows", 0};
        static_assert(RL_NPROF == RTK_CNT_LANE_PROF2 - RTK_CNT_LANE_PROF, "counter map: the lane profile has RL_NPROF slots");
        const unsigned long long* p1 = cnt + RTK_CNT_LANE_PROF; const unsigned long long* p2 = cnt + RTK_CNT_LANE_PROF2;
        unsigned long long tot = 0; for (int i = 0; i < RL_NPROF; ++i) tot += p1[i];
        fprintf(stderr, "[rtk trace] k_regions_lanes lap profile (%.3g lane cycles):", double(tot));
        for (int i = 0; i < RL_NPROF; ++i) if (p1[i] && ln[i]) fprintf(stderr, " [%s %.4f]", ln[i], double(p1[i]) / double(tot ? tot : 1));
        fprintf(stderr, "\n");
        unsigned long long tw = 0; for (int i = 0; i < RL_NPROF; ++i) tw += p2[i];
        fprintf(stderr, "[rtk trace] k_regions_lanes wave-time estimate by slot (share of %.3g, lanes together):", double(tw) / 64.0);
        for (int i = 0; i < RL_NPROF; ++i)
            if (p2[i] && ln[i]) fprintf(stderr, " [%s %.4f x%.1f]", ln[i], double(p2[i]) / double(tw ? tw : 1), 64.0 * double(p1[i]) / double(p2[i]));
        fprintf(stderr, "\n");
    }
#endif
    fprintf(stderr, "[rtk trace] k_regions shares of %.3g wave cycles: colour %.3f paths %.3f consensus %.3f myers %.3f sets %.3f tostring %.3f pathqual %.3f "
                    "walk %.3f\n",
            double(cnt[RTK_CNT_CYC_TOTAL]), share(RTK_CNT_CYC_COLOUR), share(RTK_CNT_CYC_PATHS), share(RTK_CNT_CYC_CONSENSUS), share(RTK_CNT_CYC_MYERS),
            share(RTK_CNT_CYC_SETS),
            share(RTK_CNT_CYC_TOSTRING), share(RTK_CNT_CYC_PATHQUAL), share(RTK_CNT_WALK_CYCLES));
    fprintf(stderr, "[rtk trace] k_regions cycle shares: DFS bookkeeping %.3f (of which colour checks %.3f)\n", share(RTK_CNT_CYC_DFS), share(RTK_CNT_CYC_COLOUR_OK));
    fprintf(stderr, "[rtk trace] trims: by column %llu (of which stored %llu), by the distance call %llu, cycles %.3g; consensus calls: forward alignment resumed %llu, swept %llu\n",
            cnt[RTK_CNT_ROUTES + 0] + cnt[RTK_CNT_ROUTES + 1], cnt[RTK_CNT_ROUTES + 0], cnt[RTK_CNT_ROUTES + 2], double(cnt[RTK_CNT_FINE + RTK_FINE_TRIM]), cnt[RTK_CNT_ROUTES + 3], cnt[RTK_CNT_ROUTES + 4]);
    fprintf(stderr, "[rtk trace] fixAmbiguity linked-allele searches: run %llu, skipped %llu, entries produced %llu, cycles %.3g\n", cnt[RTK_CNT_FA_LINKED + 0], cnt[RTK_CNT_FA_LINKED + 1],
            cnt[RTK_CNT_FA_LINKED + 2], double(cnt[RTK_CNT_FINE + RTK_FINE_FA_LINKED]));
    fprintf(stderr, "[rtk trace] second strand of gap regions: run %llu, skipped %llu (the forward result decides), audit mismatches %llu\n", cnt[RTK_CNT_STRAND2 + 0], cnt[RTK_CNT_STRAND2 + 1], cnt[RTK_CNT_STRAND2 + 2]);
    fprintf(stderr, "[rtk trace] stored sweeps of the forward trims: walked for a consensus %llu (from a second sweep %llu), never walked %llu\n", cnt[RTK_CNT_PARK + 0], cnt[RTK_CNT_PARK_RESWEEPS], cnt[RTK_CNT_PARK + 1]);
    fprintf(stderr, "[rtk trace] colour selections answered by: small %llu, wide %llu, bits %llu, general %llu; audit mismatches %llu; handed on by the register program for room %llu\n", cnt[RTK_CNT_COLOURS + 0], cnt[RTK_CNT_COLOURS + 1], cnt[RTK_CNT_COLOURS + 2],
            cnt[RTK_CNT_COLOURS + 3], cnt[RTK_CNT_COLOURS + 4], cnt[RTK_CNT_COLOURS + 5]);
    fprintf(stderr, "[rtk trace] walks %llu moves %llu reloads %llu scalar steps %llu cycles %.3g tail cycles %.3g\n", cnt[RTK_CNT_WALK_CALLS], cnt[RTK_CNT_WALK_MOVES],
            cnt[RTK_CNT_WALK_RELOADS], cnt[RTK_CNT_WALK_SCALAR], double(cnt[RTK_CNT_WALK_CYCLES]), double(cnt[RTK_CNT_WALK_TAIL]));
}

static void region_stats(RegionRun& R, const unsigned long long* cnt) {
    rtk_batch* b = R.b; rtk_stats& st = b->stats;
    st.cyc_colour = cnt[RTK_CNT_CYC_COLOUR]; st.cyc_paths = cnt[RTK_CNT_CYC_PATHS]; st.cyc_consensus = cnt[RTK_CNT_CYC_CONSENSUS]; st.cyc_total = cnt[RTK_CNT_CYC_TOTAL];
    st.cyc_myers = cnt[RTK_CNT_CYC_MYERS]; st.cyc_sets = cnt[RTK_CNT_CYC_SETS]; st.cyc_tostring = cnt[RTK_CNT_CYC_TOSTRING]; st.cyc_pathqual = cnt[RTK_CNT_CYC_PATHQUAL];
    st.cyc_walk = cnt[RTK_CNT_WALK_CYCLES]; st.n_moves = cnt[RTK_CNT_WALK_MOVES];
    st.n_slots_exact = cnt[RTK_CNT_SLOTS_EXACT]; st.n_slots_inexact = cnt[RTK_CNT_SLOTS_INEXACT];
    st.ms_regions = R.t_enum.elapsed() + (R.n_regions ? R.t_easy.elapsed() : 0.0);
    st.ms_lanes = R.lanes_on ? R.t_lanes.elapsed() : 0.0;
    st.ms_correct = R.ms_reg + ((R.lanes_on && !R.lanes_beside) ? st.ms_lanes : 0.0);
    st.n_lane_handed = cnt[RTK_CNT_LANE_HANDED]; st.n_lane_regions = cnt[RTK_CNT_LANE_HANDED] + cnt[RTK_CNT_LANE_DONE];
    st.n_trim_stored = cnt[RTK_CNT_ROUTES + 0]; st.n_trim_column = cnt[RTK_CNT_ROUTES + 1]; st.n_trim_fallback = cnt[RTK_CNT_ROUTES + 2];
    st.n_consensus_resumed = cnt[RTK_CNT_ROUTES + 3]; st.n_consensus_swept = cnt[RTK_CNT_ROUTES + 4];
    st.n_fa_linked_run = cnt[RTK_CNT_FA_LINKED + 0]; st.n_fa_linked_skipped = cnt[RTK_CNT_FA_LINKED + 1]; st.n_fa_linked_entries = cnt[RTK_CNT_FA_LINKED + 2];
    st.n_strand2_run = cnt[RTK_CNT_STRAND2 + 0]; st.n_strand2_skipped = cnt[RTK_CNT_STRAND2 + 1]; st.n_strand2_audit_mismatch = cnt[RTK_CNT_STRAND2 + 2];
    st.n_park_walked = cnt[RTK_CNT_PARK + 0]; st.n_park_deferred = cnt[RTK_CNT_PARK + 1]; st.n_park_resweeps = cnt[RTK_CNT_PARK_RESWEEPS];
    st.n_colours_small = cnt[RTK_CNT_COLOURS + 0]; st.n_colours_wide = cnt[RTK_CNT_COLOURS + 1]; st.n_colours_bits = cnt[RTK_CNT_COLOURS + 2]; st.n_colours_general = cnt[RTK_CNT_COLOURS + 3];
    st.n_colours_audit_mismatch = cnt[RTK_CNT_COLOURS + 4]; st.n_colours_declined_fit = cnt[RTK_CNT_COLOURS + 5];
    st.ms_stitch = R.t_st.elapsed(); st.ms_total = b->t_all.elapsed();
    st.n_windows = b->n_bases;
    st.n_probes_exact = cnt[RTK_CNT_PROBES_EXACT]; st.n_probes_inexact = cnt[RTK_CNT_PROBES_INEXACT]; st.n_hits_inexact = cnt[RTK_CNT_HITS_INEXACT];
    st.n_regions = R.n_regions; st.n_region_items = R.n_regions; st.n_arena_overflow = R.n_ovf_total;
    st.n_expand = cnt[RTK_CNT_EXPAND]; st.n_colour_elem = cnt[RTK_CNT_COLOUR]; st.n_path_base = cnt[RTK_CNT_PATHBASE];
    st.n_align = cnt[RTK_CNT_ALIGN]; st.n_align_cells = cnt[RTK_CNT_CELLS];
    st.in_bases = b->n_bases; st.out_bases = R.out_top / 2;
}

extern "C" int rtk_batch_run_regions(rtk_batch* b, const rtk_opts* opts) {
    int rc = batch_precheck(b, opts, "rtk_batch_run_regions");
    if (rc) return rc;
    if (!b->seeded) return rtk_fail(RTK_ERR_ARG, "rtk_batch_run_regions: rtk_batch_run_seeds has not completed for this batch");
    if (opts->long_read_correct && !b->bv.qual.get())
        return rtk_fail(RTK_ERR_ARG, "rtk_batch_run_regions: the second pass (long_read_correct) needs a batch created with quality strings");
    rtk_graph* g = b->g;
    try {
        rtk_set_device(g->device);
        RegionRun R = {};
        R.b = b; R.g = g; R.ov = opts_view(opts); R.sm = b->stream; R.own_slab = opts->long_read_correct != 0;
        R.hold.g = g; R.hold.what = -1; R.slab.g = g;
        R.trace = rtk_knob_trace(); R.w0 = std::chrono::steady_clock::now();
        for (uint32_t i = 0; i < b->n; ++i) R.max_len = std::max<uint32_t>(R.max_len, static_cast<uint32_t>(b->roff[i + 1] - b->roff[i]));
        R.grid = default_grid();
        region_alloc(R);
        region_lane_class(R);
        R.lap("alloc");
        region_enumerate(R);
        R.lap("enum");
        region_easy(R);
        region_lanes(R);
        region_take_areas(R);
        rc = region_attempts(R);
        if (rc) return rc;
        R.hold.release();
        R.lap("regions");
        rc = region_stitch(R);
        if (rc) return rc;
        unsigned long long cnt[RTK_CNT_TOTAL]; rtk_d2h_s(cnt, b->bv.counters, sizeof(cnt), R.sm);
        if (R.trace) region_trace_report(cnt);
        region_stats(R, cnt);
        R.lap("done");
        if (b->h_out) { g->stage_give(b->h_out, b->h_out_bytes); b->h_out = nullptr; }
        b->ran = true; b->seeded = false;
    } catch (const std::exception& e) { return rtk_fail(RTK_ERR_DEVICE, e.what()); }
    return RTK_OK;
}

extern "C" int rtk_batch_run(rtk_batch* b, const rtk_opts* opts) {
    const int rc = rtk_batch_run_seeds(b, opts);
    return rc ? rc : rtk_batch_run_regions(b, opts);
}

static int batch_fetch_host(rtk_batch* b) {
    if (b->h_out) return RTK_OK;
    rtk_set_device(b->g->device);
    const auto tf0 = std::chrono::steady_clock::now();
    unsigned long long out_top = 0; rtk_d2h_s(&out_top, b->rb.out_top, 8, b->stream);
    const auto tf1 = std::chrono::steady_clock::now();
    b->h_out = b->g->stage_take(out_top + 8, &b->h_out_bytes);
    const auto tf2 = std::chrono::steady_clock::now();
    b->h_off.resize(b->n); b->h_sl.resize(b->n); b->h_ql.resize(b->n);
    if (out_top) rtk_check_async_d2h(b->h_out, b->rb.out_pool, out_top, b->stream);
    rtk_d2h_s(b->h_off.data(), b->rb.out_off, 8ull * b->n, b->stream); rtk_d2h_s(b->h_sl.data(), b->rb.out_seq_len, 4ull * b->n, b->stream); rtk_d2h_s(b->h_ql.data(), b->rb.out_qual_len, 4ull * b->n, b->stream);
    if (rtk_knob_trace()) { auto ms = [](std::chrono::steady_clock::time_point a, std::chrono::steady_clock::time_point b_) { return std::chrono::duration<double, std::milli>(b_ - a).count(); }; fprintf(stderr, "[rtk trace] fetch: wait for the stream %.2f ms, staging buffer %.2f ms, %.1f MB to the host %.2f ms\n", ms(tf0, tf1), ms(tf1, tf2), out_top / 1048576.0, ms(tf2, std::chrono::steady_clock::now())); }
    for (uint32_t i = 0; i < b->n; ++i) {
        const char* bad = nullptr;
        if (b->h_sl[i] != b->h_ql[i]) bad = "rtk_batch_fetch: sequence and quality lengths differ for a read";
        else if (b->h_off[i] + 2ull * b->h_sl[i] > out_top) bad = "rtk_batch_fetch: record outside the output pool";
        if (bad) { rtk_ssync(b->stream); b->g->stage_give(b->h_out, b->h_out_bytes); b->h_out = nullptr; return rtk_fail(RTK_ERR_DEVICE, bad); }
    }
    return RTK_OK;
}

extern "C" int rtk_batch_fetch_view(rtk_batch* b, const char** pool, const uint64_t** off, const uint32_t** len) {
    if (!b || !pool || !off || !len) return rtk_fail(RTK_ERR_ARG, "rtk_batch_fetch_view: null argument");
    if (!b->ran) return rtk_fail(RTK_ERR_ARG, "rtk_batch_fetch_view: rtk_batch_run has not completed");
    try { const int rc = batch_fetch_host(b); if (rc) return rc; }
    catch (const std::exception& e) { return rtk_fail(RTK_ERR_DEVICE, e.what()); }
    *pool = static_cast<const char*>(b->h_out); *off = b->h_off.data(); *len = b->h_sl.data();
    return RTK_OK;
}

extern "C" int rtk_batch_fetch(rtk_batch* b, char** out_seq, char** out_qual, uint32_t* out_len) {
    if (!b || !out_seq || !out_qual || !out_len) return rtk_fail(RTK_ERR_ARG, "rtk_batch_fetch: null argument");
    if (!b->ran) return rtk_fail(RTK_ERR_ARG, "rtk_batch_fetch: rtk_batch_run has not completed");
    try {
        const int rc = batch_fetch_host(b); if (rc) return rc;
        const char* pool = static_cast<const char*>(b->h_out);
        for (uint32_t i = 0; i < b->n; ++i) { out_seq[i] = nullptr; out_qual[i] = nullptr; }
        std::atomic<bool> oom(false);
        auto copy_range = [&](uint32_t lo, uint32_t hi) {
            for (uint32_t i = lo; i < hi && !oom.load(std::memory_order_relaxed); ++i) {
                const uint32_t sl = b->h_sl[i];
                out_seq[i] = static_cast<char*>(malloc(sl + 1)); out_qual[i] = static_cast<char*>(malloc(sl + 1));
                if (!out_seq[i] || !out_qual[i]) { oom.store(true); return; }
                memcpy(out_seq[i], pool + b->h_off[i], sl); out_seq[i][sl] = 0;
                memcpy(out_qual[i], pool + b->h_off[i] + sl, sl); out_qual[i][sl] = 0;
                out_len[i] = sl;
            }
        };
        {
            const uint32_t n_thr = (b->n_bases >= (4u << 20) && b->n >= 8) ? 4u : 1u;
            std::vector<uint32_t> cut(n_thr + 1, b->n); cut[0] = 0;
            for (uint32_t t = 1, i = 0; t < n_thr; ++t) { const uint64_t want = b->n_bases / n_thr * t; while (i < b->n && b->roff[i] < want) ++i; cut[t] = i; }
            std::vector<std::thread> thr;
            for (uint32_t t = 1; t < n_thr; ++t) thr.emplace_back(copy_range, cut[t], cut[t + 1]);
            copy_range(cut[0], cut[1]);
            for (size_t t = 0; t < thr.size(); ++t) thr[t].join();
        }
        if (oom.load()) { for (uint32_t j = 0; j < b->n; ++j) { free(out_seq[j]); free(out_qual[j]); out_seq[j] = nullptr; out_qual[j] = nullptr; } return rtk_fail(RTK_ERR_DEVICE, "rtk_batch_fetch: out of host memory"); }
    } catch (const std::exception& e) { return rtk_fail(RTK_ERR_DEVICE, e.what()); }
    return RTK_OK;
}

extern "C" int rtk_batch_get_stats(const rtk_batch* b, rtk_stats* stats) { if (!b || !stats) return rtk_fail(RTK_ERR_ARG, "rtk_batch_get_stats: null"); *stats = b->stats; return RTK_OK; }

struct CoGroup { rtk_batch* b = nullptr; const char* pool = nullptr; const uint64_t* off = nullptr; const uint32_t* len = nullptr; std::atomic<int> left{0}; };
struct CoTicket {
    const rtk_opts* opts; uint32_t n; const char* const* seq; const char* const* qual; const uint32_t* len; uint64_t bases;
    bool taken = false, done = false, alone_after_all = false; int rc = 0; std::string err; CoGroup* grp = nullptr; uint32_t first = 0;
};
static bool co_compatible(const CoTicket& a, const CoTicket& b) { return (a.qual == nullptr) == (b.qual == nullptr) && memcmp(a.opts, b.opts, sizeof(rtk_opts)) == 0; }

extern "C" int rtk_coalesce_stats(rtk_graph* g, uint64_t* n_groups, uint64_t* n_tickets) {
    if (!g || !n_groups || !n_tickets) return rtk_fail(RTK_ERR_ARG, "rtk_coalesce_stats: null argument");
    std::lock_guard<std::mutex> lk(g->co_m); *n_groups = g->co_groups; *n_tickets = g->co_tickets; return RTK_OK;
}

static int correct_batch_alone(rtk_graph* g, const rtk_opts* opts, uint32_t n, const char* const* seq, const char* const* qual, const uint32_t* len, char** out_seq, char** out_qual, uint32_t* out_len) {
    rtk_batch* b = nullptr;
    const bool trace = rtk_knob_trace();
    const auto t0 = std::chrono::steady_clock::now();
    auto ms = [&](std::chrono::steady_clock::time_point a) { return std::chrono::duration<double, std::milli>(std::chrono::steady_clock::now() - a).count(); };
    int rc = rtk_batch_create(g, n, seq, qual, len, &b);
    if (rc) return rc;
    const double t_create = ms(t0); const auto t1 = std::chrono::steady_clock::now();
    rc = rtk_batch_run(b, opts);
    const double t_run = ms(t1); const auto t2 = std::chrono::steady_clock::now();
    if (rc == RTK_OK) rc = rtk_batch_fetch(b, out_seq, out_qual, out_len);
    const double t_fetch = ms(t2); const auto t3 = std::chrono::steady_clock::now();
    rtk_batch_free(b);
    if (trace) fprintf(stderr, "[rtk trace] correct_batch: create %.1f ms, run %.1f ms, fetch %.1f ms, free %.1f ms\n", t_create, t_run, t_fetch, ms(t3));
    return rc;
}

extern "C" int rtk_correct_batch(rtk_graph* g, const rtk_opts* opts, uint32_t n, const char* const* seq, const char* const* qual, const uint32_t* len,
                                 char** out_seq, char** out_qual, uint32_t* out_len) {
    if (!g || !opts || (n && (!seq || !len || !out_seq || !out_qual || !out_len))) return rtk_fail(RTK_ERR_ARG, "rtk_correct_batch: null argument");
    if (!opts_ok(opts)) return rtk_fail(RTK_ERR_ARG, "rtk_correct_batch: rtk_opts was not filled by this library's rtk_opts_default (struct_size does not match: older header, or a zero-filled struct)");
    if (!g->on_device) return rtk_fail(RTK_ERR_NO_DEVICE, "rtk_correct_batch: graph is not resident on a device (call rtk_graph_upload); there is no CPU fallback");
    if (n == 0) return RTK_OK;
    uint64_t bases = 0; for (uint32_t i = 0; i < n; ++i) bases += len[i];
    const uint64_t cap = rtk_knob_coalesce_bases();
    if (cap == 0 || bases >= cap || opts->long_read_correct) return correct_batch_alone(g, opts, n, seq, qual, len, out_seq, out_qual, out_len);

    CoTicket me; me.opts = opts; me.n = n; me.seq = seq; me.qual = qual; me.len = len; me.bases = bases;
    std::unique_lock<std::mutex> lk(g->co_m);
    g->co_q.push_back(&me);
    g->co_cv.notify_all();
    while (!me.done) {
        if (me.taken || g->co_gathering) { g->co_cv.wait(lk); continue; }
        g->co_gathering = true;
        const bool alone = g->co_q.size() == 1 && g->co_running == 0 && g->co_last_group <= 1;
        const auto deadline = std::chrono::steady_clock::now() + std::chrono::microseconds(alone ? 0L : rtk_knob_coalesce_wait_us());
        const bool cold = g->co_running == 0;
        while (true) {
            uint64_t sum = 0; for (size_t i = 0; i < g->co_q.size(); ++i) if (co_compatible(*g->co_q[i], me)) sum += g->co_q[i]->bases;
            if (sum >= cap) break;
            const bool late = std::chrono::steady_clock::now() >= deadline;
            if (late && (g->co_running == 0 || (g->co_pre_region == 0 && g->co_running < 3))) break;
            if (late) g->co_cv.wait(lk); else g->co_cv.wait_until(lk, deadline);
        }
        uint64_t take_cap = cap; uint32_t take_n = 0xFFFFFFFFu;
        { uint32_t nw = 0; for (size_t i = 0; i < g->co_q.size(); ++i) if (co_compatible(*g->co_q[i], me)) ++nw;
          const uint32_t split = rtk_knob_coalesce_split();
          const uint32_t around = nw + g->co_inflight_tickets; if (around >= 2 * split) take_n = (around + split - 1) / split; }
        (void)cold;
        std::vector<CoTicket*> grp; uint64_t sum = 0;
        for (size_t i = 0; i < g->co_q.size();) {
            CoTicket* t = g->co_q[i];
            if (((sum < take_cap && grp.size() < take_n) || t == &me) && co_compatible(*t, me)) { t->taken = true; sum += t->bases; grp.push_back(t); g->co_q.erase(g->co_q.begin() + static_cast<long>(i)); } else ++i;
        }
        g->co_gathering = false; g->co_running += 1; g->co_pre_region += 1; g->co_last_group = static_cast<uint32_t>(grp.size()); g->co_inflight_tickets += static_cast<uint32_t>(grp.size()); g->co_groups += 1; g->co_tickets += grp.size();
        g->co_cv.notify_all();
        lk.unlock();
        int rc = RTK_OK; std::string err; CoGroup* cg = new CoGroup();
        struct Pace { rtk_graph* g; bool in_regions; } pace = {g, false};
        auto enter_regions_fn = [](void* p_) { Pace* p = static_cast<Pace*>(p_); if (!p->in_regions) { p->in_regions = true; std::lock_guard<std::mutex> l2(p->g->co_m); p->g->co_pre_region -= 1; p->g->co_cv.notify_all(); } };
        auto enter_regions = [&]() { enter_regions_fn(&pace); };
        if (grp.size() == 1) {
            delete cg; cg = nullptr;
            rtk_batch* b1 = nullptr;
            rc = rtk_batch_create(g, n, seq, qual, len, &b1);
            if (rc == RTK_OK) { b1->on_region_slab = enter_regions_fn; b1->on_region_slab_arg = &pace; rc = rtk_batch_run_seeds(b1, opts); }
            if (rc == RTK_OK) rc = rtk_batch_run_regions(b1, opts);
            enter_regions();
            if (rc == RTK_OK) rc = rtk_batch_fetch(b1, out_seq, out_qual, out_len);
            if (rc) err = rtk_last_error();
            if (b1) rtk_batch_free(b1);
        } else {
            uint32_t tot = 0; for (size_t i = 0; i < grp.size(); ++i) { grp[i]->first = tot; tot += grp[i]->n; }
            std::vector<const char*> sa(tot), qa(qual ? tot : 0); std::vector<uint32_t> la(tot);
            for (size_t i = 0; i < grp.size(); ++i) for (uint32_t j = 0; j < grp[i]->n; ++j) { sa[grp[i]->first + j] = grp[i]->seq[j]; la[grp[i]->first + j] = grp[i]->len[j]; if (qual) qa[grp[i]->first + j] = grp[i]->qual[j]; }
            const bool tr_ = rtk_knob_trace(); static const auto t_epoch = std::chrono::steady_clock::now();
            auto now_ms = [&]() { return std::chrono::duration<double, std::milli>(std::chrono::steady_clock::now() - t_epoch).count(); };
            const double tq0 = now_ms();
            rc = rtk_batch_create(g, tot, sa.data(), qual ? qa.data() : nullptr, la.data(), &cg->b);
            const double tq1 = now_ms();
            if (rc == RTK_OK) { cg->b->on_region_slab = enter_regions_fn; cg->b->on_region_slab_arg = &pace; rc = rtk_batch_run_seeds(cg->b, opts); }
            const double tq2 = now_ms();
            if (rc == RTK_OK) rc = rtk_batch_run_regions(cg->b, opts);
            enter_regions();
            const double tq3 = now_ms();
            if (rc == RTK_OK) rc = rtk_batch_fetch_view(cg->b, &cg->pool, &cg->off, &cg->len);
            if (tr_) fprintf(stderr, "[rtk trace] correct_batch group at %.1f ms: %zu tickets, %u reads, %.2f Mb; create %.2f seeds %.2f (kernels %.2f) regions %.2f (k_regions %.2f) fetch %.2f ms (rc %d)\n", tq0, grp.size(), tot, sum / 1e6, tq1 - tq0, tq2 - tq1,
                            cg->b ? cg->b->stats.ms_lookup_exact + cg->b->stats.ms_mask + cg->b->stats.ms_lookup_inexact + cg->b->stats.ms_seeds : 0.0, tq3 - tq2, cg->b ? cg->b->stats.ms_correct : 0.0, now_ms() - tq3, rc);
            if (rc == RTK_OK && rtk_knob_test_coalesce_fail()) rc = rtk_fail(RTK_ERR_DEVICE, "test hook: the merged batch is reported as failed");
            if (rc) { err = rtk_last_error(); if (cg->b) rtk_batch_free(cg->b); delete cg; cg = nullptr; }
            else cg->left.store(static_cast<int>(grp.size()));
        }
        enter_regions();
        lk.lock();
        g->co_running -= 1; g->co_inflight_tickets -= static_cast<uint32_t>(grp.size());
        const bool redo = rc != RTK_OK && grp.size() > 1;
        for (size_t i = 0; i < grp.size(); ++i) { grp[i]->rc = redo ? RTK_OK : rc; grp[i]->err = err; grp[i]->grp = cg; grp[i]->alone_after_all = redo; grp[i]->done = true; }
        g->co_cv.notify_all();
    }
    lk.unlock();
    if (me.rc) return rtk_fail(me.rc, me.err);
    if (me.alone_after_all) return correct_batch_alone(g, opts, n, seq, qual, len, out_seq, out_qual, out_len);
    if (!me.grp) return RTK_OK;
    CoGroup* cg = me.grp; int rc = RTK_OK;
    for (uint32_t i = 0; i < n; ++i) { out_seq[i] = nullptr; out_qual[i] = nullptr; }
    for (uint32_t i = 0; i < n && rc == RTK_OK; ++i) {
        const uint32_t r = me.first + i, sl = cg->len[r];
        out_seq[i] = static_cast<char*>(malloc(sl + 1)); out_qual[i] = static_cast<char*>(malloc(sl + 1));
        if (!out_seq[i] || !out_qual[i]) { for (uint32_t j = 0; j <= i; ++j) { free(out_seq[j]); free(out_qual[j]); out_seq[j] = nullptr; out_qual[j] = nullptr; } rc = rtk_fail(RTK_ERR_DEVICE, "rtk_correct_batch: out of host memory"); break; }
        memcpy(out_seq[i], cg->pool + cg->off[r], sl); out_seq[i][sl] = 0;
        memcpy(out_qual[i], cg->pool + cg->off[r] + sl, sl); out_qual[i][sl] = 0;
        out_len[i] = sl;
    }
    if (cg->left.fetch_sub(1) == 1) { rtk_batch_free(cg->b); delete cg; }
    return rc;
}

extern "C" int rtk_reserve_second_pass(int device, uint32_t n_tickets, uint64_t phase_bytes, uint64_t region_bytes) {
#ifdef RTK_SIM
    (void)device; (void)n_tickets; (void)phase_bytes; (void)region_bytes; return RTK_OK;
#endif
    try {
        rtk_set_device(device);
        {
            static std::vector<int> seeded; bool first = false;
            { std::lock_guard<std::mutex> lk(g_reserved_lock); if (std::find(seeded.begin(), seeded.end(), device) == seeded.end()) { seeded.push_back(device); first = true; } }
            if (first) {
                SeedScratchCfg sc; sc.set_cap = 32768u; sc.v_cap = 32768u; sc.s_cap = 131072u + 64;
                ReservedSlab r; r.device = device; r.bytes = seed_scratch_bytes(sc) * static_cast<uint64_t>(seed_waves()); r.p = rtk_dmalloc(r.bytes);
                std::lock_guard<std::mutex> lk(g_reserved_lock); g_reserved.push_back(r);
            }
        }
        for (uint32_t t = 0; t < n_tickets; ++t) for (int i = 0; i < 2; ++i) {
            const uint64_t want = i == 0 ? phase_bytes : region_bytes;
            if (!want) continue;
#ifndef RTK_SIM
            size_t fr = 0, tot = 0; if (hipMemGetInfo(&fr, &tot) != hipSuccess) break;
            if (static_cast<uint64_t>(fr) < want + (static_cast<uint64_t>(tot) / 4)) return rtk_fail(RTK_ERR_DEVICE, "rtk_reserve_second_pass: not reserved (less than a quarter of the device memory would stay free)");
#endif
            ReservedSlab r; r.device = device; r.bytes = want; r.p = rtk_dmalloc(want);
            std::lock_guard<std::mutex> lk(g_reserved_lock); g_reserved.push_back(r);
        }
    } catch (const std::exception& e) { return rtk_fail(RTK_ERR_DEVICE, std::string("rtk_reserve_second_pass: ") + e.what()); }
    return RTK_OK;
}

extern "C" int rtk_reserve_scratch(int device, uint32_t max_read_len) {
    try {
        rtk_set_device(device);
        SeedScratchCfg sc; sc.set_cap = 32768u; sc.v_cap = 32768u; { uint32_t q = 131072u; while (q < max_read_len) q <<= 1; sc.s_cap = q + 64; }
#ifdef RTK_SIM
        const uint64_t n_seed_waves = 16, reg_waves = 16;
#else
        const uint64_t n_seed_waves = static_cast<uint64_t>(seed_waves()), reg_waves = static_cast<uint64_t>(rtk_knob_region_waves());
#endif
#ifdef RTK_SIM
        uint64_t reg_bytes = region_scratch_bytes(region_cfg(max_read_len, 0)) * reg_waves;
#else
        (void)reg_waves;
        uint64_t reg_bytes = region_scratch_bytes(region_cfg(max_read_len, 0)) * static_cast<uint64_t>(region_waves_that_fit(region_scratch_bytes(region_cfg(max_read_len, 0)), 0, rtk_knob_trace()));
#endif
#ifndef RTK_SIM
        if (region_compact()) reg_bytes = std::max<uint64_t>(reg_bytes, region_scratch_bytes(region_cfg(max_read_len, 1)) * 1024ull);
#endif
        const uint64_t want[2] = { seed_scratch_bytes(sc) * n_seed_waves, reg_bytes };
        for (int i = 0; i < 2; ++i) {
            ReservedSlab r; r.device = device; r.bytes = want[i]; r.p = rtk_dmalloc(want[i]);
            std::lock_guard<std::mutex> lk(g_reserved_lock);
            g_reserved.push_back(r);
        }
    } catch (const std::exception& e) { return rtk_fail(RTK_ERR_DEVICE, std::string("rtk_reserve_scratch: ") + e.what()); }
    return RTK_OK;
}
```

### ratatosk_amd/csrc/hip/rtk_region_types.h

```cpp
#ifndef RTK_REGION_TYPES_H
#define RTK_REGION_TYPES_H

#include "rtk_myers.h"
#include "rtk_seeds.h"
#include "rtk_types.h"
#include "rtk_wave.h"

struct RegionDesc {
    uint32_t read;
    uint32_t kind;
    uint32_t i_solid;
    uint32_t prev_pos;
    uint64_t seg_off;
    uint32_t seq_len, qual_len;
    uint32_t status;
    uint32_t pad;
};
#define RTK_RG_WHOLE_MAX 0
#define RTK_RG_WHOLE_MIN 1
#define RTK_RG_HEAD 2
#define RTK_RG_GAP 3
#define RTK_RG_TAIL 4
#define RTK_RG_TAIL_COPY 5

struct RegionBatch {
    U<RegionDesc*> regions; U<uint64_t> regions_cap; U<unsigned long long*> n_regions;
    U<uint64_t*> r_first; U<uint32_t*> r_count;
    U<char*> seq_rc;
    U<char*> qual_rev;
    U<char*> seg_pool; U<uint64_t> seg_cap; U<unsigned long long*> seg_top;
    U<unsigned long long*> next_region;
    U<uint32_t*> eorder;
    U<uint32_t*> rorder; U<unsigned long long*> n_heavy;
    U<unsigned long long*> n_overflow;
    U<uint32_t*> horder;
    U<uint32_t*> lorder; U<unsigned long long*> next_lane; U<uint32_t> lane_max_gap;
    U<char*> out_pool; U<uint64_t> out_cap; U<unsigned long long*> out_top;
    U<uint64_t*> out_off; U<uint32_t*> out_seq_len; U<uint32_t*> out_qual_len;
    U<uint64_t*> st_off;
};

enum RtkRbuf { RTK_RB_FW_SEQ = 0, RTK_RB_FW_QUAL = 1, RTK_RB_BW_SEQ = 2, RTK_RB_BW_QUAL = 3, RTK_RB_OUT_SEQ = 4, RTK_RB_OUT_QUAL = 5,
               RTK_RB_RC_TMP = 6, RTK_RB_CONS_SEQ = 6, RTK_RB_PARK_MOVES = 7, RTK_RB_CONS_QUAL = 7, RTK_RB_N = 8,
               RTK_RB_PHASE_SEQ = 0, RTK_RB_PHASE_QUAL = 1 };
enum RtkStr { RTK_STR_CAND = 0, RTK_STR_AMB_QUERY = 0, RTK_STR_PATH = 1, RTK_STR_AMB_SUB = 1, RTK_STR_QUAL = 2, RTK_STR_SWEEP_STASH = 3,
              RTK_STR_CONS_MOVES_FW = 3, RTK_STR_CONS_MOVES_BW = 4, RTK_STR_PROBE = 4, RTK_STR_N = 5 };
enum RtkBm { RTK_BM_FW = 0, RTK_BM_BW = 1, RTK_BM_RC_TMP = 2, RTK_BM_N = 3,
             RTK_BM_PHASE_RM = 0, RTK_BM_PHASE_NEW = 1, RTK_BM_PHASE_COV = 2 };
enum RtkList { RTK_L_SIDE_LEFT = 0, RTK_L_SIDE_RIGHT = 1, RTK_L_SIDE_MIDDLE = 2,
               RTK_L_BFS_PATHS = 0, RTK_L_BFS_NEW = 1, RTK_L_DFS_T = 2, RTK_L_DFS_NT = 3, RTK_L_DFS_STACK = 4, RTK_L_PARTIAL = 5,
               RTK_L_COL_VALS = 3, RTK_L_COL_KEYS = 4, RTK_L_COL_SLOT_OF = 5,
               RTK_L_AMB = 6, RTK_L_AMB_SAFE = 7, RTK_L_AMB_ALL = 8, RTK_L_AMB_UNITIG = 9, RTK_L_AMB_LINKED = 10, RTK_L_N = 11,
               RTK_L_PHASE_RUN_POS = 0, RTK_L_PHASE_RUN_UNITIG = 1, RTK_L_PHASE_NBITS = 2, RTK_L_PHASE_STATE = 3 };
enum RtkSet { RTK_SET_ALL_PIDS = 0, RTK_SET_UNION_A = 1, RTK_SET_UNION_B = 2, RTK_SET_ALL_PIDS_ALT = 3, RTK_SET_PICKED = 4,
              RTK_SET_CUR_A = 7, RTK_SET_CUR_B = 8, RTK_SET_UNION_TMP = 9, RTK_SET_N = 10,
              RTK_SET_CS_SORT = 1, RTK_SET_CS_TAGS = 2, RTK_SET_CB_IDS = 1, RTK_SET_CB_STORE = 2 };
enum RtkWp { RTK_WP_REGION = 0, RTK_WP_BFS = 1, RTK_WP_DFS = 2, RTK_WP_REPEATS_PATH = 1, RTK_WP_REPEATS_TRIAL = 2, RTK_WP_REPEATS_CYCLE = 3, RTK_WP_N = 4 };
enum RtkArena { RTK_ARENA_REGION = 0, RTK_ARENA_BFS = 1, RTK_ARENA_DFS = 2, RTK_ARENA_N = 3,
                RTK_ARENA_COL_AUDIT = 0, RTK_ARENA_COL_SETS = 2, RTK_ARENA_PHASE_FILTERS = 0 };
enum RtkLocLen { RTK_LEN_OUT_SEQ = 0, RTK_LEN_OUT_QUAL = 1, RTK_LEN_CONS_SEQ = 2, RTK_LEN_CONS_QUAL = 3, RTK_LEN_CORR_SEQ = 4, RTK_LEN_CORR_QUAL = 5, RTK_LEN_N = 6 };
enum RtkLocBest { RTK_BEST_ID = 0, RTK_BEST_END = 1, RTK_BEST_N = 2 };
enum RtkLocAnchors { RTK_AN_SOLID = 0, RTK_AN_WEAK = 1, RTK_AN_SOLID_RC = 2, RTK_AN_WEAK_RC = 3, RTK_AN_N = 4 };
enum RtkLocRes { RTK_RES_FW = 0, RTK_RES_BW = 1, RTK_RES_N = 2 };
enum RtkLocSide { RTK_SIDE_LEFT = 0, RTK_SIDE_RIGHT = 1, RTK_SIDE_MIDDLE = 2, RTK_SIDE_N = 3 };

enum RtkOvf {
    RTK_OVF_NONE = 0,
    RTK_OVF_ALIGN_CAP = 1,
    RTK_OVF_ALIGN_OPTIMUM = 2,
    RTK_OVF_ARENA = 3,
    RTK_OVF_PATH_LOAD = 4,
    RTK_OVF_PATH_UNITIGS = 5,
    RTK_OVF_PATH_QUAL = 6,
    RTK_OVF_STRING = 7,
    RTK_OVF_LIST = 8,
    RTK_OVF_SET = 9,
    RTK_OVF_BITMAP = 10,
    RTK_OVF_AMB = 11,
    RTK_OVF_CONS_STALL = 11,
    RTK_OVF_SEG_POOL = 12,
    RTK_OVF_REPEAT_QUAL = 14
};

enum RtkLap {
    RTK_LAP_DRIVER_DISPATCH = 0, RTK_LAP_DRIVER_SAME_UNITIG = 1, RTK_LAP_REGION_PROLOGUE = 2, RTK_LAP_REGION_SIDE_LISTS = 3, RTK_LAP_REGION_COLOURS = 4,
    RTK_LAP_SEMIWEAK_GLUE = 5, RTK_LAP_PATHS_PROLOGUE = 6, RTK_LAP_EXPLORE_PREFIX = 7, RTK_LAP_DFS_POP = 8, RTK_LAP_DFS_COLOUR_OK = 9,
    RTK_LAP_DFS_T_EXTEND = 10, RTK_LAP_DFS_T_STRING = 11, RTK_LAP_DFS_T_SWEEP = 12, RTK_LAP_DFS_T_COMMIT = 13, RTK_LAP_DFS_NT_EXTEND = 14,
    RTK_LAP_DFS_NT_REST = 15, RTK_LAP_DFS_POST_SCORE = 16, RTK_LAP_DFS_POST_STRING = 17, RTK_LAP_DFS_POST_QUAL = 18, RTK_LAP_DFS_POST_COMMIT = 19,
    RTK_LAP_PATHS_AFTER_EXPLORE = 20, RTK_LAP_PATHS_SELECT = 21, RTK_LAP_SEMIWEAK_MERGE = 22, RTK_LAP_REGION_RESTART = 23, RTK_LAP_REGION_ASSEMBLE = 24,
    RTK_LAP_REGION_FIX_AMBIGUITY = 25, RTK_LAP_REGION_TRIM = 26, RTK_LAP_DRIVER_STRAND2 = 27, RTK_LAP_CONS_ENTRY = 28, RTK_LAP_CONS_FW_PATH = 29,
    RTK_LAP_CONS_BW_PATH = 30, RTK_LAP_CONS_MERGE = 31, RTK_LAP_CONS_FINAL = 32, RTK_LAP_DRIVER_EMIT_PREP = 33, RTK_LAP_DEQUEUE = 34, RTK_LAP_EMIT = 35,
    RTK_LAP_PROBE_COLD = 40, RTK_LAP_PROBE_WARM = 41, RTK_LAP_PROBE_SLAB = 42, RTK_LAP_PROBE_SAMPLES = 43,
    RTK_LAP_N = 48
};
static_assert(RTK_LAP_N == RTK_CNT_PROF_END - RTK_CNT_PROF, "lap slots: the counter map holds one word per slot");

enum RtkSite {
    RTK_SITE_NONE = 0,
    RTK_SITE_SCORE_TERMINAL = 1,
    RTK_SITE_SCORE_REF_IN_PATH = 2,
    RTK_SITE_SCORE_PATH_IN_REF = 3,
    RTK_SITE_PATH_QUAL = 4,
    RTK_SITE_EXPLORE_PREFIX = 5,
    RTK_SITE_SELECT_NT = 6,
    RTK_SITE_RESIZE_BEST = 7,
    RTK_SITE_REPEATS_PATH = 8,
    RTK_SITE_REPEATS_TURN = 9,
    RTK_SITE_SELECT_BFS = 10,
    RTK_SITE_SELECT_PARTIAL_RETRY = 11,
    RTK_SITE_SELECT_PARTIAL = 12,
    RTK_SITE_TRIM_FALLBACK = 13,
    RTK_SITE_CONS_FW = 14, RTK_SITE_CONS_BW = 15, RTK_SITE_CONS_FINAL = 16,
    RTK_SITE_FIX_AMBIGUITY = 17,
    RTK_SITE_TRIM_STORED = 18, RTK_SITE_TRIM_COLUMN = 19
};

enum RtkHist { RTK_H_CYCLES = 0, RTK_H_REGIONS = 8, RTK_H_STRAND2 = 16, RTK_H_DFS = 24, RTK_H_DFS_RUNNING = 31, RTK_H_N = 32 };
enum { RTK_GAP_CLASS_HEAD_TAIL = 7, RTK_GAP_CLASSES = 8 };
static_assert(RTK_H_N == RTK_CNT_HIST_END - RTK_CNT_HIST, "size-class table: the counter map holds one word per slot");
#define rtk_gap_class(gap_len) ((gap_len) < 40 ? 0 : (gap_len) < 64 ? 1 : (gap_len) < 128 ? 2 : (gap_len) < 256 ? 3 : (gap_len) < 512 ? 4 : (gap_len) < 1024 ? 5 : 6)

struct RegionScratchCfg { ScratchCfg my; uint32_t set_cap, um_cap, str_cap, list_cap, memo_cap, bm_words; uint64_t arena_cap; };

struct WPath { U<UMap*> ums; U<char*> qual; U<uint32_t> n, l, qlen; };

struct Anchors { U<const uint32_t*> pos; U<const uint64_t*> hit; U<const uint64_t*> hits_by_pos; U<uint32_t> n, L; U<int> rev; U<int> k; };
struct SideList { uint32_t* u; uint8_t* nb; uint32_t n, cap; };
struct ResCorr { char* seq; char* qual; uint32_t seq_len, qual_len; uint64_t* bm; uint32_t old_len; bool is_corrected; uint32_t n_all; int all_set; };
struct RegionCall { const char* s_read; const char* q_read; uint64_t complete; UMap um1, um2; uint32_t s_len, p1, p2, first_pos, len_weak_region, lw_lo, lw_hi, n_all, n_partial, n_amb, has_end_pt, found_first, lrc; };
struct TrimPark { uint32_t nm, len; int32_t dist; uint32_t n, last_move, pending, gen; };
enum { RTK_PARK_TABLE = 1u, RTK_PARK_NO_TABLE = 2u };
struct DriverLocals { Anchors an[RTK_AN_N]; ResCorr rc[RTK_RES_N]; SideList side[RTK_SIDE_N]; uint32_t len[RTK_LEN_N]; int best[RTK_BEST_N]; MyersSaved saved; RegionCall call; TrimPark park; MyersResult trim; };

struct RegionScratch {
    MyersScratch my;
    U<uint32_t*> set[RTK_SET_N]; U<uint32_t> set_cap;
    U<char*> arena[RTK_ARENA_N]; U<uint64_t> arena_cap; U<uint64_t> top[RTK_ARENA_N];
    WPath wp[RTK_WP_N]; U<uint32_t> um_cap;
    U<char*> str[RTK_STR_N]; U<uint32_t> str_cap;
    U<char*> rbuf[RTK_RB_N];
    U<uint64_t*> list[RTK_L_N]; U<uint32_t> list_cap;
    U<uint32_t*> memo_u; U<uint8_t*> memo_v; U<uint32_t> memo_cap; U<uint32_t> memo_n;
    U<uint64_t*> bm[RTK_BM_N]; U<uint32_t> bm_words;
    UL<uint32_t*> overflow; U<uint32_t> ovf_word;
    DriverLocals loc;
    U<unsigned long long> cnt[RTK_RC_N];
    U<unsigned long long> fine[RTK_FINE_N];
#ifdef RTK_PROF
    U<unsigned long long> prof[RTK_LAP_N]; U<unsigned long long> prof_t;
#endif
#ifndef RTK_SLIM_HDR
    U<unsigned long long> hist[RTK_H_N];
#endif
};
#ifdef RTK_SLIM_HDR
#define RTK_HIST_ADD(sc, i, v) ((void)0)
#define RTK_HIST_GET(sc, i) 0ull
#else
#define RTK_HIST_ADD(sc, i, v) ((sc).hist[i] += (v))
#define RTK_HIST_GET(sc, i) ((sc).hist[i])
#endif
#ifdef RTK_PROF
#define RTK_PL(sc, i) do { const unsigned long long t_ = rtk_clock(); (sc).prof[i] += t_ - (sc).prof_t; (sc).prof_t = t_; } while (0)
#else
#define RTK_PL(sc, i) ((void)0)
#endif

struct LaunchCtx { GraphView g; OptsView o; BatchView bv; RegionBatch rb; };

struct RCtx {
    const GraphView& g; const OptsView& o; const BatchView& bv; const RegionBatch& rb;
    UL<RegionScratch*> sc;
    U<int> k;
};

RTK_DEV RegionScratch& rtk_hdr(const RCtx& c) { RegionScratch* p = c.sc; RTK_ASSUME_LDS(p); return *p; }

RTK_HD uint64_t region_scratch_bytes(const RegionScratchCfg& c) {
    uint64_t b = scratch_bytes(c.my);
    b += 4ull * RTK_SET_N * c.set_cap + 1ull * RTK_ARENA_N * c.arena_cap + 1ull * RTK_WP_N * (sizeof(UMap) * c.um_cap + c.str_cap) + (1ull * RTK_STR_N + RTK_RB_N) * c.str_cap;
    b += 8ull * RTK_L_N * c.list_cap + 5ull * c.memo_cap + 8ull * RTK_BM_N * c.bm_words + sizeof(RegionScratch) + 1024;
    return (b + 255) / 256 * 256;
}

RTK_DEV RegionScratch* region_scratch_carve(char* base, const RegionScratchCfg& c, RegionScratch* hdr = nullptr) {
    RegionScratch* s = hdr ? hdr : reinterpret_cast<RegionScratch*>(base);
    char* p = base + ((sizeof(RegionScratch) + 255) / 256 * 256);
    RegionScratch t;
    t.my = scratch_carve(p, c.my); p += scratch_bytes(c.my);
    for (int i = 0; i < RTK_ARENA_N; ++i) { t.arena[i] = p; p += c.arena_cap; t.top[i] = 0; }
    t.arena_cap = c.arena_cap;
    for (int i = 0; i < RTK_L_N; ++i) { t.list[i] = reinterpret_cast<uint64_t*>(p); p += 8ull * c.list_cap; }
    t.list_cap = c.list_cap;
    for (int i = 0; i < RTK_BM_N; ++i) { t.bm[i] = reinterpret_cast<uint64_t*>(p); p += 8ull * c.bm_words; }
    t.bm_words = c.bm_words;
    for (int i = 0; i < RTK_WP_N; ++i) { t.wp[i].ums = reinterpret_cast<UMap*>(p); p += sizeof(UMap) * c.um_cap; t.wp[i].n = 0; t.wp[i].l = 0; t.wp[i].qlen = 0; }
    t.um_cap = c.um_cap;
    for (int i = 0; i < RTK_SET_N; ++i) { t.set[i] = reinterpret_cast<uint32_t*>(p); p += 4ull * c.set_cap; }
    t.set_cap = c.set_cap;
    t.memo_u = reinterpret_cast<uint32_t*>(p); p += 4ull * c.memo_cap; t.memo_cap = c.memo_cap; t.memo_n = 0;
    for (int i = 0; i < RTK_WP_N; ++i) { t.wp[i].qual = p; p += c.str_cap; }
    for (int i = 0; i < RTK_STR_N; ++i) { t.str[i] = p; p += c.str_cap; }
    for (int i = 0; i < RTK_RB_N; ++i) { t.rbuf[i] = p; p += c.str_cap; }
    t.str_cap = c.str_cap;
    t.memo_v = reinterpret_cast<uint8_t*>(p); p += c.memo_cap;
    t.ovf_word = 0; t.overflow = reinterpret_cast<uint32_t*>(&s->ovf_word); t.my.overflow = t.overflow;
    for (int i = 0; i < RTK_RC_N; ++i) t.cnt[i] = 0;
    for (int i = 0; i < RTK_FINE_N; ++i) t.fine[i] = 0;
#ifdef RTK_PROF
    for (int i = 0; i < RTK_LAP_N; ++i) t.prof[i] = 0;
    t.prof_t = rtk_clock();
#endif
#ifndef RTK_SLIM_HDR
    for (int i = 0; i < RTK_H_N; ++i) t.hist[i] = 0;
#endif
    *s = t;
    return s;
}

#endif
```

Baseline: 2.304 billion.

## Order hard regions into eight gap-size classes scheduled largest-first

Region ordering previously split non-easy regions into just heavy and light lists. It now buckets them into eight size classes by gap length, with heads and tails in their own class, and serves them in a fixed class order through the work-stealing counter. Counters are spread 128 bytes apart, one slot per list. The aim is a longest-job-first schedule that cuts tail imbalance across waves. In exchange the kernel does more ballots, the rorder buffer grows eightfold, each fetch walks the class counts, and per-class statistics are copied back to the host.

```diff
diff --git a/include/ratatosk_hip.h b/include/ratatosk_hip.h
--- a/include/ratatosk_hip.h
+++ b/include/ratatosk_hip.h
@@ -64,6 +64,8 @@
     uint64_t n_colours_small, n_colours_wide, n_colours_bits, n_colours_general, n_colours_audit_mismatch;
     uint64_t n_colours_declined_fit;
     uint64_t n_park_resweeps;
+    uint64_t n_regions_easy;
+    uint64_t n_regions_class[8];
 } rtk_stats;
 
 int rtk_graph_load(const char* unitig_fasta_gz, const char* rtsk, int k, int n_threads, rtk_graph** out);
diff --git a/ratatosk_amd/api.py b/ratatosk_amd/api.py
--- a/ratatosk_amd/api.py
+++ b/ratatosk_amd/api.py
@@ -34,7 +34,8 @@
                                          "n_strand2_run", "n_strand2_skipped", "n_strand2_audit_mismatch",
                                          "n_park_walked", "n_park_deferred",
                                          "n_colours_small", "n_colours_wide", "n_colours_bits", "n_colours_general", "n_colours_audit_mismatch", "n_colours_declined_fit",
-                                         "n_park_resweeps")]
+                                         "n_park_resweeps", "n_regions_easy")] + \
+               [("n_regions_class%d" % c, C.c_uint64) for c in range(8)]
 
     def as_dict(self):
         return {n: getattr(self, n) for n, _ in self._fields_}
diff --git a/ratatosk_amd/csrc/hip/rtk_knobs.h b/ratatosk_amd/csrc/hip/rtk_knobs.h
--- a/ratatosk_amd/csrc/hip/rtk_knobs.h
+++ b/ratatosk_amd/csrc/hip/rtk_knobs.h
@@ -43,6 +43,7 @@
 inline int rtk_knob_lane_round() { return rtk_env_int("RTK_LANE_ROUND", 64); }
 inline bool rtk_knob_compact() { return rtk_env_is1("RTK_COMPACT"); }
 inline int rtk_knob_region_waves() { return rtk_env_pos_int("RTK_REGION_WAVES", 4096); }
+inline bool rtk_knob_region_order_two() { return rtk_env_eq("RTK_REGION_ORDER", "two"); }
 inline int rtk_knob_p2_rgrid() { return rtk_env_int("RTK_P2_RGRID", 512); }
 inline bool rtk_knob_fa_linked_always() { return rtk_env_is1("RTK_FA_LINKED_ALWAYS"); }
 inline bool rtk_knob_strand2_always() { return rtk_env_is1("RTK_STRAND2_ALWAYS"); }
diff --git a/ratatosk_amd/csrc/hip/rtk_pipeline_run.inc b/ratatosk_amd/csrc/hip/rtk_pipeline_run.inc
--- a/ratatosk_amd/csrc/hip/rtk_pipeline_run.inc
+++ b/ratatosk_amd/csrc/hip/rtk_pipeline_run.inc
@@ -32,48 +32,55 @@
     return pb < pa + k;
 }
 #define RTK_OQ 4
-RTK_GLOBAL void k_region_order(const LaunchCtx* L, uint64_t n_regions, int grid) {
+RTK_GLOBAL void k_region_order(const LaunchCtx* L, uint64_t n_regions, int two_classes, int grid) {
     const BatchView& bv = L->bv; const RegionBatch& rb = L->rb;
     const bool first_pass = L->o.long_read_correct == 0;
     const uint32_t lane_max_gap = rb.lane_max_gap;
+    const uint32_t NONE = RTK_NQ_SLOTS;
     for (uint64_t i0 = static_cast<uint64_t>(RTK_BLOCK_ID) * RTK_OQ * RTK_WAVE; i0 < n_regions; i0 += static_cast<uint64_t>(grid) * RTK_OQ * RTK_WAVE) {
-        uint64_t mh[RTK_OQ], ml[RTK_OQ], me[RTK_OQ], mn[RTK_OQ][4]; uint32_t th = 0, tl = 0, te = 0, tn[4] = {0, 0, 0, 0};
+        uint32_t slot[RTK_OQ], rank[RTK_OQ], tot[RTK_NQ_HANDED];
+        for (uint32_t s = 0; s < RTK_NQ_HANDED; ++s) tot[s] = 0;
+        const uint64_t below = (1ull << rtk_lane()) - 1ull;
 #pragma unroll
         for (int q = 0; q < RTK_OQ; ++q) {
             const uint64_t i = i0 + static_cast<uint64_t>(q) * RTK_WAVE + static_cast<uint64_t>(rtk_lane());
-            const bool in = i < n_regions;
-            bool easy = false, heavy = false, lane_cls = false; uint32_t lane_sub = 0;
-            if (in) {
+            slot[q] = NONE; rank[q] = 0;
+            if (i < n_regions) {
                 const RegionDesc rd = rb.regions[i];
+                bool easy = false; uint32_t gl = 0;
+                if (rd.kind == RTK_RG_GAP) { const uint32_t* sp = bv.s_pos + bv.roff[rd.read]; gl = sp[rd.i_solid + 1] - sp[rd.i_solid]; }
                 if (first_pass) {
                     if (rd.kind == RTK_RG_GAP) { bool sc_; UMap ua_; uint32_t a_, b_; easy = rtk_gap_is_easy(L->g, L->o, bv, rd, &sc_, &ua_, &a_, &b_); }
                     else easy = rd.kind == RTK_RG_WHOLE_MAX || rd.kind == RTK_RG_WHOLE_MIN || rd.kind == RTK_RG_TAIL_COPY;
                 }
-                if (first_pass && !easy && lane_max_gap != 0 && rd.kind == RTK_RG_GAP) { const uint32_t* sp = bv.s_pos + bv.roff[rd.read]; const uint32_t gl = sp[rd.i_solid + 1] - sp[rd.i_solid]; lane_cls = gl < lane_max_gap; lane_sub = lane_cls ? (4u * gl) / lane_max_gap : 0u; }
-                heavy = !easy && !lane_cls && rtk_region_is_heavy(bv, rd);
+                if (easy) slot[q] = RTK_NQ_EASY;
+                else if (first_pass && lane_max_gap != 0 && rd.kind == RTK_RG_GAP && gl < lane_max_gap) slot[q] = RTK_NQ_LANE + (4u * gl) / lane_max_gap;
+                else if (two_classes) slot[q] = RTK_NQ_CLASS + rtk_class_at(rtk_region_is_heavy(bv, rd) ? 0 : RTK_GAP_CLASSES - 1);
+                else if (rd.kind == RTK_RG_GAP) { const uint32_t c = static_cast<uint32_t>(rtk_gap_class(gl)); slot[q] = RTK_NQ_CLASS + c; }
+                else slot[q] = RTK_NQ_CLASS + ((rd.kind == RTK_RG_HEAD || rd.kind == RTK_RG_TAIL) ? RTK_GAP_CLASS_HEAD_TAIL : 0);
             }
-            mh[q] = rtk_ballot(heavy); ml[q] = rtk_ballot(in && !heavy && !easy && !lane_cls); me[q] = rtk_ballot(easy);
-            for (uint32_t sb = 0; sb < 4; ++sb) { mn[q][sb] = rtk_ballot(lane_cls && lane_sub == sb); tn[sb] += static_cast<uint32_t>(rtk_popc(mn[q][sb])); }
-            th += static_cast<uint32_t>(rtk_popc(mh[q])); tl += static_cast<uint32_t>(rtk_popc(ml[q])); te += static_cast<uint32_t>(rtk_popc(me[q]));
-        }
-        unsigned long long bh = 0, bl = 0, be = 0, bn[4] = {0, 0, 0, 0};
-        if (rtk_lane() == 0) {
-            if (th) bh = rtk_atomic_add(rb.n_heavy.get(), static_cast<unsigned long long>(th));
-            if (tl) bl = rtk_atomic_add(rb.n_heavy.get() + 1, static_cast<unsigned long long>(tl));
-            if (te) be = rtk_atomic_add(rb.n_heavy.get() + 2, static_cast<unsigned long long>(te));
-            for (uint32_t sb = 0; sb < 4; ++sb) if (tn[sb]) bn[sb] = rtk_atomic_add(rb.n_heavy.get() + 8 + sb, static_cast<unsigned long long>(tn[sb]));
-        }
-        bh = rtk_shfl(bh, 0); bl = rtk_shfl(bl, 0); be = rtk_shfl(be, 0); for (uint32_t sb = 0; sb < 4; ++sb) bn[sb] = rtk_shfl(bn[sb], 0);
-        const uint64_t below = (1ull << rtk_lane()) - 1ull;
+            for (uint32_t s = 0; s < RTK_NQ_HANDED; ++s) {
+                const uint64_t m = rtk_ballot(slot[q] == s);
+                if (slot[q] == s) rank[q] = tot[s] + static_cast<uint32_t>(rtk_popc(m & below));
+                tot[s] += static_cast<uint32_t>(rtk_popc(m));
+            }
+        }
+        unsigned long long base[RTK_NQ_HANDED];
+        for (uint32_t s = 0; s < RTK_NQ_HANDED; ++s) {
+            base[s] = 0;
+            if (rtk_lane() == 0 && tot[s]) base[s] = rtk_atomic_add(rb.n_heavy.get() + RTK_NQ(s), static_cast<unsigned long long>(tot[s]));
+        }
+        for (uint32_t s = 0; s < RTK_NQ_HANDED; ++s) base[s] = rtk_shfl(base[s], 0);
 #pragma unroll
         for (int q = 0; q < RTK_OQ; ++q) {
             const uint64_t i = i0 + static_cast<uint64_t>(q) * RTK_WAVE + static_cast<uint64_t>(rtk_lane());
-            const uint64_t mine = 1ull << rtk_lane();
-            if (mh[q] & mine) rb.rorder[bh + static_cast<unsigned long long>(rtk_popc(mh[q] & below))] = static_cast<uint32_t>(i);
-            else if (me[q] & mine) rb.eorder[be + static_cast<unsigned long long>(rtk_popc(me[q] & below))] = static_cast<uint32_t>(i);
-            else if (ml[q] & mine) rb.rorder[n_regions - 1ull - (bl + static_cast<unsigned long long>(rtk_popc(ml[q] & below)))] = static_cast<uint32_t>(i);
-            else for (uint32_t sb = 0; sb < 4; ++sb) if (mn[q][sb] & mine) rb.lorder[sb * rb.regions_cap + bn[sb] + static_cast<unsigned long long>(rtk_popc(mn[q][sb] & below))] = static_cast<uint32_t>(i);
-            bh += static_cast<unsigned long long>(rtk_popc(mh[q])); bl += static_cast<unsigned long long>(rtk_popc(ml[q])); be += static_cast<unsigned long long>(rtk_popc(me[q])); for (uint32_t sb = 0; sb < 4; ++sb) bn[sb] += static_cast<unsigned long long>(rtk_popc(mn[q][sb]));
+            if (slot[q] == NONE) continue;
+            unsigned long long at = 0;
+            for (uint32_t s = 0; s < RTK_NQ_HANDED; ++s) if (slot[q] == s) at = base[s];
+            at += rank[q];
+            uint32_t* const list = slot[q] == RTK_NQ_EASY ? rb.eorder.get() : (slot[q] >= RTK_NQ_LANE ? rb.lorder.get() + static_cast<uint64_t>(slot[q] - RTK_NQ_LANE) * rb.regions_cap
+                                                                                                       : rb.rorder.get() + static_cast<uint64_t>(slot[q] - RTK_NQ_CLASS) * rb.regions_cap);
+            list[at] = static_cast<uint32_t>(i);
         }
     }
 }
@@ -81,7 +88,7 @@
 struct RtkEasy { uint64_t src; uint64_t b0; uint32_t len_a, len_b, n_max, n_min, n_dec, strand; };
 RTK_GLOBAL void k_regions_easy(const LaunchCtx* L, int grid) {
     const GraphView& g = L->g; const OptsView& o = L->o; const BatchView& bv = L->bv; const RegionBatch& rb = L->rb;
-    const unsigned long long n_easy = rtk_u(rb.n_heavy[2]);
+    const unsigned long long n_easy = rtk_u(rb.n_heavy[RTK_NQ(RTK_NQ_EASY)]);
     const uint32_t k = static_cast<uint32_t>(g.k);
     const char q_min = rtk_get_qual(0.0, 0, static_cast<uint64_t>(o.max_qual)), q_max = rtk_get_qual(1.0, 0, static_cast<uint64_t>(o.max_qual));
     const char* const seq = bv.seq.get(); const uint64_t* const useq = g.useq.get(); char* const pool = rb.seg_pool.get();
@@ -166,7 +173,7 @@
     for (int x = 0; x < RL_NPROF; ++x) { c.prof[x] = 0; c.prof2[x] = 0; } c.prof_t = rtk_clock(); c.prof_cur = RL_P_DRIVER;
 #endif
     for (int sub = 3; sub >= 0; --sub) {
-    const unsigned long long n_lane = rtk_u(rb.n_heavy[8 + sub]);
+    const unsigned long long n_lane = rtk_u(rb.n_heavy[RTK_NQ(RTK_NQ_LANE + sub)]);
     const uint32_t* const lorder = rb.lorder.get() + static_cast<uint64_t>(sub) * rb.regions_cap;
     while (true) {
         unsigned long long i0 = 0;
@@ -199,7 +206,7 @@
         if (in) {
             if (c.fail()) {
                 rd->status = c.fail(); ++n_handed;
-                const unsigned long long at = rtk_atomic_add(rb.n_heavy.get() + 4, 1ull);
+                const unsigned long long at = rtk_atomic_add(rb.n_heavy.get() + RTK_NQ(RTK_NQ_HANDED), 1ull);
                 rb.horder[at] = lorder[idx];
             } else {
                 const unsigned long long off = off0 + static_cast<unsigned long long>(mine);
@@ -247,8 +254,9 @@
     rtk_sync();
     (void)o;
     RCtx c = {L->g, L->o, L->bv, L->rb, {rtk_opaque(sc)}, {g.k}};
-    const unsigned long long n_hv = (which & 1) ? rtk_u(rb.n_heavy[0]) : 0ull, n_lt = (which & 1) ? rtk_u(rb.n_heavy[1]) : 0ull;
-    const unsigned long long n_ho = (which & 2) ? rtk_u(rb.n_heavy[4]) : 0ull;
+    unsigned long long n_cls = 0;
+    if (which & 1) for (uint32_t p = 0; p < RTK_GAP_CLASSES; ++p) n_cls += rtk_u(rb.n_heavy[RTK_NQ(RTK_NQ_CLASS + p)]);
+    const unsigned long long n_ho = (which & 2) ? rtk_u(rb.n_heavy[RTK_NQ(RTK_NQ_HANDED)]) : 0ull;
     unsigned long long nxt = 0;
     if (rtk_lane() == 0) nxt = rtk_atomic_add(rb.next_region, 1ull);
 #if !defined(RTK_SIM)
@@ -258,8 +266,16 @@
     while (true) {
         const unsigned long long idx = rtk_u(rtk_shfl(nxt, 0));
         uint32_t ri; bool stolen = false;
-        if (idx < n_hv + n_lt + n_ho) {
-            ri = rtk_u(idx < n_hv + n_lt ? rb.rorder[idx < n_hv ? idx : (n_regions - n_lt) + (idx - n_hv)] : rb.horder[idx - n_hv - n_lt]);
+        if (idx < n_cls + n_ho) {
+            if (idx < n_cls) {
+                unsigned long long at = idx; uint32_t cls = rtk_class_at(0);
+                for (uint32_t p = 0; p + 1 < RTK_GAP_CLASSES; ++p) {
+                    const unsigned long long n_p = rtk_u(rb.n_heavy[RTK_NQ(RTK_NQ_CLASS + rtk_class_at(p))]);
+                    if (at < n_p) break;
+                    at -= n_p; cls = rtk_class_at(p + 1);
+                }
+                ri = rtk_u(rb.rorder[static_cast<uint64_t>(cls) * rb.regions_cap + at]);
+            } else ri = rtk_u(rb.horder[idx - n_cls]);
             if (rtk_lane() == 0) nxt = rtk_atomic_add(rb.next_region, 1ull);
         } else if ((which & 4) && steal_sub < 4) {
             ri = RTK_NONE32;
@@ -267,7 +283,7 @@
                 unsigned long long at = 0;
                 if (rtk_lane() == 0) at = rtk_atomic_add(rb.next_lane.get() + steal_sub, 1ull);
                 at = rtk_u(rtk_shfl(at, 0));
-                if (at < rtk_u(rb.n_heavy[8 + steal_sub])) { ri = rtk_u(rb.lorder[static_cast<uint64_t>(steal_sub) * rb.regions_cap + at]); stolen = true; break; }
+                if (at < rtk_u(rb.n_heavy[RTK_NQ(RTK_NQ_LANE + steal_sub)])) { ri = rtk_u(rb.lorder[static_cast<uint64_t>(steal_sub) * rb.regions_cap + at]); stolen = true; break; }
                 ++steal_sub;
             }
             if (ri == RTK_NONE32) break;
@@ -311,7 +327,7 @@
         rd->status = *sc->overflow;
         if (*sc->overflow && rtk_lane() == 0) {
             rtk_atomic_add(rb.n_overflow, 1ull);
-            if (stolen) { const unsigned long long at = rtk_atomic_add(rb.n_heavy.get() + 4, 1ull); rb.horder[at] = ri; }
+            if (stolen) { const unsigned long long at = rtk_atomic_add(rb.n_heavy.get() + RTK_NQ(RTK_NQ_HANDED), 1ull); rb.horder[at] = ri; }
         }
     }
 #if !defined(RTK_SIM)
@@ -430,6 +446,7 @@
     bool own_slab;
     std::chrono::steady_clock::time_point w0;
     int grid; uint32_t max_len; unsigned long long n_regions, n_ovf_total, out_top;
+    unsigned long long n_lists[RTK_NQ_BYTES / 8];
     bool lane_auto, lanes_on, lanes_beside; int lane_waves_used;
     RtkTimer t_enum, t_easy, t_lanes, t_reg, t_st; double ms_reg;
     SlabHold hold; OwnSlab slab;
@@ -443,7 +460,7 @@
 static void region_alloc_lists(rtk_batch* b, uint64_t cap) {
     RegionBatch& rb = b->rb;
     rb.regions_cap = cap;
-    rb.regions = b->alloc<RegionDesc>(cap); rb.rorder = b->alloc<uint32_t>(cap); rb.eorder = b->alloc<uint32_t>(cap);
+    rb.regions = b->alloc<RegionDesc>(cap); rb.rorder = b->alloc<uint32_t>(RTK_GAP_CLASSES * cap); rb.eorder = b->alloc<uint32_t>(cap);
     rb.lorder = b->alloc<uint32_t>(4 * cap); rb.horder = b->alloc<uint32_t>(cap); rb.st_off = b->alloc<uint64_t>(cap);
 }
 
@@ -453,7 +470,7 @@
     rb.seq_rc = b->alloc<char>(b->n_bases + 64);
     rb.qual_rev = b->bv.qual.get() ? b->alloc<char>(b->n_bases + 64) : nullptr;
     rb.r_first = b->alloc<uint64_t>(b->n); rb.r_count = b->alloc<uint32_t>(b->n);
-    rb.n_regions = b->alloc<unsigned long long>(1); rb.n_heavy = b->alloc<unsigned long long>(16); rb.seg_top = b->alloc<unsigned long long>(1);
+    rb.n_regions = b->alloc<unsigned long long>(1); rb.n_heavy = b->alloc<unsigned long long>(RTK_NQ_BYTES / 8); rb.seg_top = b->alloc<unsigned long long>(1);
     rb.next_region = b->alloc<unsigned long long>(1); rb.n_overflow = b->alloc<unsigned long long>(1); rb.out_top = b->alloc<unsigned long long>(1);
     rb.out_off = b->alloc<uint64_t>(b->n); rb.out_seq_len = b->alloc<uint32_t>(b->n); rb.out_qual_len = b->alloc<uint32_t>(b->n);
     region_alloc_lists(b, std::max<uint64_t>(1024, b->n_bases / 8 + 4ull * b->n));
@@ -482,12 +499,12 @@
         if (R.n_regions <= rb.regions_cap) break;
         region_alloc_lists(b, R.n_regions + 1024);
     }
+    rtk_dzero_s(rb.n_heavy, RTK_NQ_BYTES, sm);
     if (R.n_regions) {
-        rtk_dzero_s(rb.n_heavy, 128, sm);
         R.set_ctx();
         const unsigned long long per_wave = RTK_OQ * RTK_WAVE;
         const int og = static_cast<int>(std::min<unsigned long long>(static_cast<unsigned long long>(R.grid), (R.n_regions + per_wave - 1ull) / per_wave));
-        rtk_launch(k_region_order, og, sm, R.ctx(), static_cast<uint64_t>(R.n_regions), og);
+        rtk_launch(k_region_order, og, sm, R.ctx(), static_cast<uint64_t>(R.n_regions), rtk_knob_region_order_two() ? 1 : 0, og);
     }
 }
 
@@ -748,6 +765,8 @@
     st.n_park_walked = cnt[RTK_CNT_PARK + 0]; st.n_park_deferred = cnt[RTK_CNT_PARK + 1]; st.n_park_resweeps = cnt[RTK_CNT_PARK_RESWEEPS];
     st.n_colours_small = cnt[RTK_CNT_COLOURS + 0]; st.n_colours_wide = cnt[RTK_CNT_COLOURS + 1]; st.n_colours_bits = cnt[RTK_CNT_COLOURS + 2]; st.n_colours_general = cnt[RTK_CNT_COLOURS + 3];
     st.n_colours_audit_mismatch = cnt[RTK_CNT_COLOURS + 4]; st.n_colours_declined_fit = cnt[RTK_CNT_COLOURS + 5];
+    st.n_regions_easy = R.n_lists[RTK_NQ(RTK_NQ_EASY)];
+    for (int c = 0; c < RTK_GAP_CLASSES; ++c) st.n_regions_class[c] = R.n_lists[RTK_NQ(RTK_NQ_CLASS + c)];
     st.ms_stitch = R.t_st.elapsed(); st.ms_total = b->t_all.elapsed();
     st.n_windows = b->n_bases;
     st.n_probes_exact = cnt[RTK_CNT_PROBES_EXACT]; st.n_probes_inexact = cnt[RTK_CNT_PROBES_INEXACT]; st.n_hits_inexact = cnt[RTK_CNT_HITS_INEXACT];
@@ -786,7 +805,7 @@
         R.lap("regions");
         rc = region_stitch(R);
         if (rc) return rc;
-        unsigned long long cnt[RTK_CNT_TOTAL]; rtk_d2h_s(cnt, b->bv.counters, sizeof(cnt), R.sm);
+        unsigned long long cnt[RTK_CNT_TOTAL]; rtk_check_async_d2h(R.n_lists, b->rb.n_heavy.get(), sizeof(R.n_lists), R.sm); rtk_d2h_s(cnt, b->bv.counters, sizeof(cnt), R.sm);
         if (R.trace) region_trace_report(cnt);
         region_stats(R, cnt);
         R.lap("done");
diff --git a/ratatosk_amd/csrc/hip/rtk_region_types.h b/ratatosk_amd/csrc/hip/rtk_region_types.h
--- a/ratatosk_amd/csrc/hip/rtk_region_types.h
+++ b/ratatosk_amd/csrc/hip/rtk_region_types.h
@@ -39,6 +39,11 @@
     U<uint64_t*> out_off; U<uint32_t*> out_seq_len; U<uint32_t*> out_qual_len;
     U<uint64_t*> st_off;
 };
+
+enum { RTK_NQ_CLASS = 0 , RTK_NQ_LANE = 8 ,
+       RTK_NQ_EASY = 12, RTK_NQ_HANDED = 13, RTK_NQ_SLOTS = 16 };
+#define RTK_NQ(slot) (static_cast<uint64_t>(slot) * 16ull)
+#define RTK_NQ_BYTES (RTK_NQ_SLOTS * 16 * 8)
 
 enum RtkRbuf { RTK_RB_FW_SEQ = 0, RTK_RB_FW_QUAL = 1, RTK_RB_BW_SEQ = 2, RTK_RB_BW_QUAL = 3, RTK_RB_OUT_SEQ = 4, RTK_RB_OUT_QUAL = 5,
                RTK_RB_RC_TMP = 6, RTK_RB_CONS_SEQ = 6, RTK_RB_PARK_MOVES = 7, RTK_RB_CONS_QUAL = 7, RTK_RB_N = 8,
@@ -119,6 +124,8 @@
 enum { RTK_GAP_CLASS_HEAD_TAIL = 7, RTK_GAP_CLASSES = 8 };
 static_assert(RTK_H_N == RTK_CNT_HIST_END - RTK_CNT_HIST, "size-class table: the counter map holds one word per slot");
 #define rtk_gap_class(gap_len) ((gap_len) < 40 ? 0 : (gap_len) < 64 ? 1 : (gap_len) < 128 ? 2 : (gap_len) < 256 ? 3 : (gap_len) < 512 ? 4 : (gap_len) < 1024 ? 5 : 6)
+#define RTK_CLASS_ORDER 0x70123456u
+#define rtk_class_at(place) ((RTK_CLASS_ORDER >> (4u * static_cast<uint32_t>(place))) & 7u)
 
 struct RegionScratchCfg { ScratchCfg my; uint32_t set_cap, um_cap, str_cap, list_cap, memo_cap, bm_words; uint64_t arena_cap; };
 
```

Measured after the change: 2.237 billion. -2.9%, worse.
